# kongzhecn/OMG

Hardware: AMD Instinct MI355X
Metric: images/sec @ SDXL 1024^2 50-step, 2-concept mask fusion (higher is better)
Workload: dtype fp16 (storage and MFMA operands; fp32 accumulate; = the reference's own torch_dtype, inference_lora.py:153-159).  Measured tolerance per UNet forward at full size vs the fp32 oracle: rms 1.09e-3, max 4.9e-3 of O(1) outputs — the reference's own fp16 eager execution, emulated op by op in the oracle

## Files before the change

### include/omg_hip.h

```cpp
#ifndef OMG_HIP_H
#define OMG_HIP_H

#include <stdint.h>

#ifdef __cplusplus
extern "C" {
#endif

#define OMG_ABI_VERSION 6

enum { OMG_F16 = 0, OMG_BF16 = 1, OMG_F32 = 2  };

enum {
  OMG_OK = 0,
  OMG_EINVAL = -1,
  OMG_EDTYPE = -2,
  OMG_ELAUNCH = -3
};

enum {
  OMG_ACT_NONE = 0,
  OMG_ACT_SILU = 1,
  OMG_ACT_GEGLU = 2
};

int omg_abi_version(void);
const char* omg_last_error(void);

typedef struct {
  int32_t dtype;
  int32_t M, N, K;
  const void* A;  int64_t lda;
  const void* W;  int64_t ldw;
  const void* A2; int64_t lda2;
  const void* W2; int64_t ldw2;
  int32_t K2;
  int32_t a2_col_block;
  int32_t groups;
  int32_t rows_per_group;
  const int32_t* group_adapter;
  int64_t w_adapter_stride;
  int64_t w2_adapter_stride;
  const void* bias;
  const void* group_bias; int64_t ldgb;
  const void* residual; int64_t ldr;
  int32_t act;
  float out_scale;
  void* C; int64_t ldc;
} omg_gemm_args;

int omg_gemm(const omg_gemm_args* a, void* stream);

int omg_quant_mx8(int32_t dtype, const void* x, int64_t ldx, int32_t M, int32_t K,
                  void* q, int64_t ldq, void* scales, int32_t s_ld, void* stream);

typedef struct {
  int32_t dtype;
  int32_t M, N, K;
  const void* A; int64_t lda;
  const void* a_scale; int32_t sa_ld;
  const void* W; int64_t ldw;
  const void* w_scale; int32_t sw_ld;
  int32_t groups, rows_per_group;
  const int32_t* group_adapter;
  int64_t w_adapter_stride;
  int64_t sw_adapter_stride;
  const void* bias;
  const void* residual; int64_t ldr;
  int32_t act;
  float out_scale;
  void* C; int64_t ldc;
  void* c_scale; int32_t sc_ld;
} omg_gemm_mx8_args;

int omg_gemm_mx8(const omg_gemm_mx8_args* a, void* stream);

typedef struct {
  int32_t dtype;
  int32_t B, H, W, Cin, Cout;
  const void* X; const void* x_scale;
  const void* Wq; const void* w_scale;
  int32_t sw_ld, act;
  const void* bias;
  const void* group_bias; int64_t ldgb;
  const void* residual;
  float out_scale;
  void* Y;
} omg_conv2d_mx8_args;
int omg_conv2d_mx8(const omg_conv2d_mx8_args* a, void* stream);

typedef struct {
  int32_t dtype;
  int32_t B, Hin, Win;
  int32_t C1, C2;
  int32_t Hout, Wout, Cout;
  int32_t ksize;
  int32_t stride;
  int32_t upsample;
  const void* X1; const void* X2;
  const void* W;
  const void* bias;
  const void* group_bias; int64_t ldgb;
  const void* residual;
  float out_scale;
  void* Y;
  int32_t act;
} omg_conv2d_args;

int omg_conv2d(const omg_conv2d_args* a, void* stream);

typedef struct {
  int32_t dtype;
  int32_t B, heads, Nq, Nkv;
  const void* Q; int64_t ldq; int64_t q_bstride;
  const void* K; int64_t ldk; int64_t k_bstride;
  const void* Vt;
  int32_t Nkv_pad;
  const int32_t* qk_src;
  float scale;
  int32_t accumulate;
  float out_scale;
  void* O; int64_t ldo; int64_t o_bstride;
  const void* V; int64_t ldv; int64_t v_bstride;
} omg_attn_args;

int omg_attn_fwd(const omg_attn_args* a, void* stream);

int omg_transpose_v(int dtype, const void* V, int64_t ldv, int64_t v_bstride,
                    int B, int heads, int Nkv, int Nkv_pad, void* Vt, int mfma_key_order, void* stream);

int64_t omg_groupnorm_ws_floats(int B, int groups, int HW);
int omg_groupnorm(int dtype, const void* X1, int C1, const void* X2, int C2,
                  int B, int HW, int groups, float eps,
                  const void* gamma, const void* beta, int silu,
                  float* workspace, void* Y, void* stream);
int omg_layernorm(int dtype, const void* X, int64_t ldx, int M, int C, float eps,
                  const void* gamma, const void* beta, void* Y, int64_t ldy, void* stream);
int omg_layernorm_mx8(int dtype, const void* X, int64_t ldx, int M, int C, float eps,
                      const void* gamma, const void* beta, void* Q, int64_t ldq,
                      void* scales, int s_ld, void* stream);

int omg_groupnorm_mx8(int dtype, const void* X1, int C1, const void* X2, int C2,
                      int B, int HW, int groups, float eps,
                      const void* gamma, const void* beta, int silu,
                      float* workspace, void* Q, void* scales, void* stream);

typedef struct {
  int32_t B, Hin, Win, Cin;
  int32_t Hout, Wout, Cout;
  int32_t ksize, upsample;
  const void* X; const void* W; const void* bias; const void* residual;
  void* Y;
} omg_conv2d_f32_args;

int omg_conv2d_f32(const omg_conv2d_f32_args* a, void* stream);

typedef struct {
  int32_t B, Hin, Win, Cin;
  int32_t Hout, Wout, Cout;
  int32_t upsample;
  const void* X; const void* U; const void* bias; const void* residual;
  void* Y;
} omg_conv2d_f32_wino_args;

int64_t omg_conv2d_f32_wino_weight_floats(int Cout, int Cin);
int omg_conv2d_f32_wino(const omg_conv2d_f32_wino_args* a, void* stream);
int omg_cast_f32(int dtype, const void* X, float* Y, int64_t n, void* stream);

int omg_conv_in(int dtype, const void* X_nchw, int x_is_f32, int B, int Cin, int H, int W,
                const void* Wt , const void* bias, int Cout,
                void* workspace ,
                void* Y_nhwc, void* stream);
int omg_conv_out(int dtype, const void* X_nhwc, int B, int H, int W, int Cin,
                 const void* Wt , const void* bias, int Cout,
                 float* Y_nchw, void* stream);

int omg_timestep_embedding(int dtype, const float* t, int n, int dim, void* out, int64_t ldo, void* stream);
int omg_silu(int dtype, const void* x, void* y, int64_t n, void* stream);
int omg_add_inplace(int dtype, void* y, const void* a, int64_t n, void* stream);
int omg_softmax_rows(int dtype, void* X, int64_t rows, int64_t cols, int64_t ld, float scale, void* stream);
int omg_channel_mix(const float* X, const float* Wm, const float* bias, int B, int Cin, int Cout, int64_t HW,
                    float* Y, void* stream);
int omg_copy2d(int dtype, const void* src, int64_t lds, void* dst, int64_t ldd, int64_t rows, int64_t cols, void* stream);

#define OMG_MAX_CONCEPTS 8
typedef struct {
  int32_t C, H, W;
  int32_t Hm, Wm;
  int32_t n_concepts;
  int32_t fuse;
  float guidance_scale;
  const float* noise_pred;
  const float* region_pred[OMG_MAX_CONCEPTS];
  const float* masks[OMG_MAX_CONCEPTS];
  const float* coef;
  int32_t* step_idx;
  int32_t advance;
  float* latents;
  int32_t out_dtype;
  void* model_input_next;
  float* fused_noise_out;
// ... 27 lines not shown
```

### omg_amd/_lib.py

```python
from __future__ import annotations

import ctypes as C
import os

_HERE = os.path.dirname(os.path.abspath(__file__))
LIB_PATH = os.environ.get("OMG_HIP_LIB") or os.path.join(_HERE, "csrc", "libomg_hip.so")

OMG_F16, OMG_BF16, OMG_F32 = 0, 1, 2
ACT_NONE, ACT_SILU, ACT_GEGLU = 0, 1, 2
MAX_CONCEPTS = 8

c_i32, c_i64, c_f32, c_vp = C.c_int32, C.c_int64, C.c_float, C.c_void_p


class GemmArgs(C.Structure):
    _fields_ = [
        ("dtype", c_i32), ("M", c_i32), ("N", c_i32), ("K", c_i32),
        ("A", c_vp), ("lda", c_i64), ("W", c_vp), ("ldw", c_i64),
        ("A2", c_vp), ("lda2", c_i64), ("W2", c_vp), ("ldw2", c_i64),
        ("K2", c_i32), ("a2_col_block", c_i32),
        ("groups", c_i32), ("rows_per_group", c_i32),
        ("group_adapter", c_vp), ("w_adapter_stride", c_i64), ("w2_adapter_stride", c_i64),
        ("bias", c_vp), ("group_bias", c_vp), ("ldgb", c_i64),
        ("residual", c_vp), ("ldr", c_i64),
        ("act", c_i32), ("out_scale", c_f32),
        ("C", c_vp), ("ldc", c_i64),
    ]


class GemmMx8Args(C.Structure):
    _fields_ = [
        ("dtype", c_i32), ("M", c_i32), ("N", c_i32), ("K", c_i32),
        ("A", c_vp), ("lda", c_i64), ("a_scale", c_vp), ("sa_ld", c_i32),
        ("W", c_vp), ("ldw", c_i64), ("w_scale", c_vp), ("sw_ld", c_i32),
        ("groups", c_i32), ("rows_per_group", c_i32), ("group_adapter", c_vp),
        ("w_adapter_stride", c_i64), ("sw_adapter_stride", c_i64),
        ("bias", c_vp), ("residual", c_vp), ("ldr", c_i64),
        ("act", c_i32), ("out_scale", c_f32),
        ("C", c_vp), ("ldc", c_i64),
        ("c_scale", c_vp), ("sc_ld", c_i32),
    ]


class Conv2dMx8Args(C.Structure):
    _fields_ = [
        ("dtype", c_i32), ("B", c_i32), ("H", c_i32), ("W", c_i32), ("Cin", c_i32), ("Cout", c_i32),
        ("X", c_vp), ("x_scale", c_vp), ("Wq", c_vp), ("w_scale", c_vp),
        ("sw_ld", c_i32), ("act", c_i32),
        ("bias", c_vp), ("group_bias", c_vp), ("ldgb", c_i64), ("residual", c_vp),
        ("out_scale", c_f32), ("Y", c_vp),
    ]


class Conv2dArgs(C.Structure):
    _fields_ = [
        ("dtype", c_i32), ("B", c_i32), ("Hin", c_i32), ("Win", c_i32),
        ("C1", c_i32), ("C2", c_i32), ("Hout", c_i32), ("Wout", c_i32), ("Cout", c_i32),
        ("ksize", c_i32), ("stride", c_i32), ("upsample", c_i32),
        ("X1", c_vp), ("X2", c_vp), ("W", c_vp), ("bias", c_vp),
        ("group_bias", c_vp), ("ldgb", c_i64), ("residual", c_vp),
        ("out_scale", c_f32), ("Y", c_vp), ("act", c_i32),
    ]


class Conv2dF32Args(C.Structure):
    _fields_ = [
        ("B", c_i32), ("Hin", c_i32), ("Win", c_i32), ("Cin", c_i32),
        ("Hout", c_i32), ("Wout", c_i32), ("Cout", c_i32), ("ksize", c_i32), ("upsample", c_i32),
        ("X", c_vp), ("W", c_vp), ("bias", c_vp), ("residual", c_vp), ("Y", c_vp),
    ]


class Conv2dF32WinoArgs(C.Structure):
    _fields_ = [
        ("B", c_i32), ("Hin", c_i32), ("Win", c_i32), ("Cin", c_i32),
        ("Hout", c_i32), ("Wout", c_i32), ("Cout", c_i32), ("upsample", c_i32),
        ("X", c_vp), ("U", c_vp), ("bias", c_vp), ("residual", c_vp), ("Y", c_vp),
    ]


class AttnArgs(C.Structure):
    _fields_ = [
        ("dtype", c_i32), ("B", c_i32), ("heads", c_i32), ("Nq", c_i32), ("Nkv", c_i32),
        ("Q", c_vp), ("ldq", c_i64), ("q_bstride", c_i64),
        ("K", c_vp), ("ldk", c_i64), ("k_bstride", c_i64),
        ("Vt", c_vp), ("Nkv_pad", c_i32),
        ("qk_src", c_vp), ("scale", c_f32), ("accumulate", c_i32), ("out_scale", c_f32),
        ("O", c_vp), ("ldo", c_i64), ("o_bstride", c_i64),
        ("V", c_vp), ("ldv", c_i64), ("v_bstride", c_i64),
    ]


class StepArgs(C.Structure):
    _fields_ = [
        ("C", c_i32), ("H", c_i32), ("W", c_i32), ("Hm", c_i32), ("Wm", c_i32),
        ("n_concepts", c_i32), ("fuse", c_i32), ("guidance_scale", c_f32),
        ("noise_pred", c_vp), ("region_pred", c_vp * MAX_CONCEPTS), ("masks", c_vp * MAX_CONCEPTS),
        ("coef", c_vp), ("step_idx", c_vp), ("advance", c_i32),
        ("latents", c_vp), ("out_dtype", c_i32), ("model_input_next", c_vp), ("fused_noise_out", c_vp),
    ]


SYMBOLS = {
    "omg_abi_version": (c_i32, []),
    "omg_last_error": (C.c_char_p, []),
    "omg_gemm": (c_i32, [C.POINTER(GemmArgs), c_vp]),
    "omg_quant_mx8": (c_i32, [c_i32, c_vp, c_i64, c_i32, c_i32, c_vp, c_i64, c_vp, c_i32, c_vp]),
    "omg_gemm_mx8": (c_i32, [C.POINTER(GemmMx8Args), c_vp]),
    "omg_conv2d_mx8": (c_i32, [C.POINTER(Conv2dMx8Args), c_vp]),
    "omg_groupnorm_mx8": (c_i32, [c_i32, c_vp, c_i32, c_vp, c_i32, c_i32, c_i32, c_i32, c_f32, c_vp, c_vp, c_i32, c_vp, c_vp, c_vp, c_vp]),
    "omg_conv2d": (c_i32, [C.POINTER(Conv2dArgs), c_vp]),
    "omg_conv2d_f32": (c_i32, [C.POINTER(Conv2dF32Args), c_vp]),
    "omg_conv2d_f32_wino_weight_floats": (c_i64, [c_i32, c_i32]),
    "omg_conv2d_f32_wino": (c_i32, [C.POINTER(Conv2dF32WinoArgs), c_vp]),
    "omg_cast_f32": (c_i32, [c_i32, c_vp, c_vp, c_i64, c_vp]),
    "omg_attn_fwd": (c_i32, [C.POINTER(AttnArgs), c_vp]),
    "omg_transpose_v": (c_i32, [c_i32, c_vp, c_i64, c_i64, c_i32, c_i32, c_i32, c_i32, c_vp, c_i32, c_vp]),
    "omg_groupnorm_ws_floats": (c_i64, [c_i32, c_i32, c_i32]),
    "omg_groupnorm": (c_i32, [c_i32, c_vp, c_i32, c_vp, c_i32, c_i32, c_i32, c_i32, c_f32, c_vp, c_vp, c_i32, c_vp, c_vp, c_vp]),
    "omg_layernorm": (c_i32, [c_i32, c_vp, c_i64, c_i32, c_i32, c_f32, c_vp, c_vp, c_vp, c_i64, c_vp]),
    "omg_layernorm_mx8": (c_i32, [c_i32, c_vp, c_i64, c_i32, c_i32, c_f32, c_vp, c_vp, c_vp, c_i64, c_vp, c_i32, c_vp]),
    "omg_conv_in": (c_i32, [c_i32, c_vp, c_i32, c_i32, c_i32, c_i32, c_i32, c_vp, c_vp, c_i32, c_vp, c_vp, c_vp]),
    "omg_conv_out": (c_i32, [c_i32, c_vp, c_i32, c_i32, c_i32, c_i32, c_vp, c_vp, c_i32, c_vp, c_vp]),
    "omg_timestep_embedding": (c_i32, [c_i32, c_vp, c_i32, c_i32, c_vp, c_i64, c_vp]),
    "omg_silu": (c_i32, [c_i32, c_vp, c_vp, c_i64, c_vp]),
    "omg_softmax_rows": (c_i32, [c_i32, c_vp, c_i64, c_i64, c_i64, C.c_float, c_vp]),
    "omg_channel_mix": (c_i32, [c_vp, c_vp, c_vp, c_i32, c_i32, c_i32, c_i64, c_vp, c_vp]),
    "omg_add_inplace": (c_i32, [c_i32, c_vp, c_vp, c_i64, c_vp]),
    "omg_copy2d": (c_i32, [c_i32, c_vp, c_i64, c_vp, c_i64, c_i64, c_i64, c_vp]),
    "omg_fuse_cfg_step": (c_i32, [C.POINTER(StepArgs), c_vp]),
    "omg_fuse_cfg_step_ms": (c_i32, [C.POINTER(StepArgs), c_vp, c_vp, c_vp]),
    "omg_fuse_cfg_step_noise": (c_i32, [C.POINTER(StepArgs), c_vp, c_i64, c_vp]),
    "omg_scale_model_input": (c_i32, [c_i32, c_vp, c_vp, c_i32, c_vp, c_vp]),
    "omg_gather_step": (c_i32, [c_i32, c_vp, c_vp, c_vp, c_i64, c_vp]),
    "omg_attn_probs": (c_i32, [C.POINTER(AttnArgs), c_vp, c_vp]),
    "omg_attn_apply_probs": (c_i32, [c_i32, c_vp, c_vp, c_i64, c_i64, c_i32, c_i32, c_i32, c_i32, c_vp, c_i64, c_i64, c_vp]),
    "omg_dwconv2d": (c_i32, [c_i32, c_vp, c_i64, c_i32, c_i32, c_i32, c_i32, c_i32, c_vp, c_vp, c_vp, c_i64, c_vp]),
    "omg_relu_linear_att_ws_floats": (c_i64, [c_i32, c_i32, c_i32, c_i32]),
    "omg_relu_linear_att": (c_i32, [c_i32, c_vp, c_i64, c_i32, c_i32, c_i32, c_i32, c_f32, c_vp, c_vp, c_i64, c_vp]),
    "omg_debug_set_glds": (None, [c_i32]),
    "omg_debug_set_gemm_variant": (None, [c_i32]),
    "omg_debug_choose_variant": (c_i32, [c_i32, c_i32, c_i32, c_i32]),
    "omg_debug_set_mx8_split": (None, [c_i32]),
    "omg_debug_set_attn_variant": (None, [c_i32]),
}

_lib = None


class OmgHipError(RuntimeError):
    pass


def lib() -> C.CDLL:
    global _lib
    if _lib is not None:
        return _lib
    if not os.path.exists(LIB_PATH):
        raise OmgHipError(
            f"{LIB_PATH} not found: the HIP extension has not been built. "
            "Run `python -c 'import __graft_entry__ as g; g.build()'` (needs hipcc). "
            "omg_amd has no CPU fallback."
        )
    import torch

    l = C.CDLL(LIB_PATH)
    for name, (res, args) in SYMBOLS.items():
        fn = getattr(l, name)
        fn.restype = res
        fn.argtypes = args
    if l.omg_abi_version() != 6:
        raise OmgHipError("libomg_hip.so ABI version mismatch; rebuild")
    v = os.environ.get("OMG_GEMM_VARIANT")
    if v:
        l.omg_debug_set_gemm_variant(int(v))
    v = os.environ.get("OMG_ATTN_VARIANT")
    if v:
        l.omg_debug_set_attn_variant(int(v, 0))
    v = os.environ.get("OMG_MX8_SPLIT")
# ... 11 lines not shown
```

### omg_amd/attention.py

```python
from __future__ import annotations

from typing import Optional

import torch
from torch import nn

from . import _lib as L
from . import ops
from .modules import Dropout, Linear, LoraState, bump_pointer_epoch, pointer_epoch


class Attention(nn.Module):

    def __init__(self, query_dim: int, cross_attention_dim: Optional[int], heads: int, dim_head: int = 64,
                 dtype=torch.float16, device=None):
        super().__init__()
        if dim_head != 64:
            raise L.OmgHipError("the gfx950 attention kernel is specialised for head_dim 64 (all SDXL layers)")
        inner = heads * dim_head
        self.heads, self.scale, self.inner_dim = heads, dim_head ** -0.5, inner
        self.is_cross = cross_attention_dim is not None
        kv_dim = cross_attention_dim if self.is_cross else query_dim
        self.to_q = Linear(query_dim, inner, bias=False, dtype=dtype, device=device)
        self.to_k = Linear(kv_dim, inner, bias=False, dtype=dtype, device=device)
        self.to_v = Linear(kv_dim, inner, bias=False, dtype=dtype, device=device)
        self.to_out = nn.ModuleList([Linear(inner, query_dim, bias=True, dtype=dtype, device=device), Dropout()])
        self.spatial_norm = None
        self.group_norm = None
        self.norm_cross = None
        self.residual_connection = False
        self.rescale_output_factor = 1.0
        self.processor = FusedAttnProcessor()
        self._qkv = None
        self._kv = None
        self._qkv_slots = None
        self._kv_slots = None
        self._kv_cache = {}
        self.ip_kv_weight: Optional[torch.Tensor] = None
        self.ip_scale, self.ip_tokens = 1.0, 16
        self._ip_cache = None
        self._mx8 = {}

    def set_processor(self, processor) -> None:
        self.processor = processor

    def get_processor(self):
        return self.processor

    def forward(self, hidden_states, encoder_hidden_states=None, attention_mask=None, **cross_attention_kwargs):
        return self.processor(self, hidden_states, encoder_hidden_states=encoder_hidden_states,
                              attention_mask=attention_mask, **cross_attention_kwargs)

    def prepare_attention_mask(self, attention_mask, target_length, batch_size, out_dim=3):
        if attention_mask is not None:
            raise L.OmgHipError("attention masks are not used on OMG's path (always None) and are not supported")
        return None

    def head_to_batch_dim(self, t: torch.Tensor) -> torch.Tensor:
        B, N, _ = t.shape
        return t.reshape(B, N, self.heads, 64).permute(0, 2, 1, 3).reshape(B * self.heads, N, 64)

    def batch_to_head_dim(self, t: torch.Tensor) -> torch.Tensor:
        BH, N, d = t.shape
        return t.reshape(BH // self.heads, self.heads, N, d).permute(0, 2, 1, 3).reshape(BH // self.heads, N, self.heads * d)

    def get_attention_scores(self, query: torch.Tensor, key: torch.Tensor, attention_mask=None) -> torch.Tensor:
        if attention_mask is not None:
            raise L.OmgHipError("attention masks are not supported")
        q, k = query.contiguous(), key.contiguous()
        return ops.attn_probs(q, k, 1, self.scale)

    def _apply(self, fn, *a, **k):
        self.invalidate_packed()
        return super()._apply(fn, *a, **k)

    def invalidate_packed(self):
        self._qkv = self._kv = self._qkv_slots = self._kv_slots = None
        self._kv_cache = {}
        self._mx8 = {}
        self._ip_cache = None
        bump_pointer_epoch()

    def qkv_weight(self) -> torch.Tensor:
        if self._qkv is None:
            self._qkv = torch.cat([self.to_q.weight.data, self.to_k.weight.data, self.to_v.weight.data], dim=0).contiguous()
        return self._qkv

    def kv_weight(self) -> torch.Tensor:
        if self._kv is None:
            self._kv = torch.cat([self.to_k.weight.data, self.to_v.weight.data], dim=0).contiguous()
        return self._kv

    def _has_lora(self) -> bool:
        st = self.to_q.lora_state
        return st is not None and not st.merged and any(l.lora_down is not None for l in (self.to_q, self.to_k, self.to_v))

    def _merged(self) -> Optional[LoraState]:
        st = self.to_q.lora_state
        if st is None or not st.merged:
            return None
        have = [l.w_slots is not None for l in (self.to_q, self.to_k, self.to_v)]
        if any(have) and not all(have):
            raise L.OmgHipError("merged LoRA slots cover only part of to_q/to_k/to_v; rebuild the LoraBank")
        return st if all(have) else None

    def qkv_slots(self) -> torch.Tensor:
        if self._qkv_slots is None:
            self._qkv_slots = torch.cat([self.to_q.w_slots, self.to_k.w_slots, self.to_v.w_slots], dim=1).contiguous()
        return self._qkv_slots

    def kv_slots(self) -> torch.Tensor:
        if self._kv_slots is None:
            self._kv_slots = torch.cat([self.to_k.w_slots, self.to_v.w_slots], dim=1).contiguous()
        return self._kv_slots

    def project_self(self, x):
        B, N, C = x.shape
        inner = self.inner_dim
        if isinstance(x, ops.Mx8Tensor) or (self.to_q.mx8 and C % 128 == 0 and not self._has_lora()):
            if self._has_lora():
                raise L.OmgHipError("MX-fp8 activations cannot feed a segment-mode LoRA projection")
            xq = x if isinstance(x, ops.Mx8Tensor) else ops.quant_mx8(x)
            st = self._merged()
            if st is not None:
                if "qkv_slots" not in self._mx8:
                    self._mx8["qkv_slots"] = ops.quant_mx8(self.qkv_slots().reshape(-1, C))
                qkv = ops.gemm_mx8(xq, self._mx8["qkv_slots"], out_dtype=self.to_q.weight.dtype, groups=st.groups,
                                   w_group_adapter=st.group_adapter, n_per_adapter=3 * inner)
            else:
                if "qkv" not in self._mx8:
                    self._mx8["qkv"] = ops.quant_mx8(self.qkv_weight())
                qkv = ops.gemm_mx8(xq, self._mx8["qkv"], out_dtype=self.to_q.weight.dtype)
            qkv = qkv.view(B, N, 3 * inner)
            return qkv[:, :, :inner], qkv[:, :, inner:2 * inner], ops.value_operand(qkv[:, :, 2 * inner:], self.heads)
        if self._has_lora():
            q = self.to_q(x); k = self.to_k(x); v = self.to_v(x)
        else:
            st = self._merged()
            if st is not None:
                qkv = ops.gemm(x.reshape(B * N, C), self.qkv_slots(), groups=st.groups, w_group_adapter=st.group_adapter)
            else:
                qkv = ops.gemm(x.reshape(B * N, C), self.qkv_weight())
            qkv = qkv.view(B, N, 3 * inner)
            q, k, v = qkv[:, :, :inner], qkv[:, :, inner:2 * inner], qkv[:, :, 2 * inner:]
        return q, k, ops.value_operand(v, self.heads)

    def project_cross(self, ctx: torch.Tensor):
        st = self.to_k.lora_state
        skey = (tuple(ctx.shape), None if st is None else (st.group_adapter.data_ptr(), st.merged))
        stamp = (ctx.data_ptr(), ctx._version)
        hit = self._kv_cache.get(skey)
        if hit is not None:
            self._kv_cache[skey] = self._kv_cache.pop(skey)
        if hit is not None and hit[0] == stamp:
            return hit[1], hit[2]
        B, Nk, Cx = ctx.shape
        inner = self.inner_dim
        kv_out = hit[4] if hit is not None else None
        vt_out = hit[2] if hit is not None else None
        if self._has_lora():
            k = self.to_k(ctx); v = self.to_v(ctx)
            kv_out = None
        else:
            ms = self._merged()
            x2 = ctx.reshape(B * Nk, Cx)
            if ms is not None:
                kv = ops.gemm(x2, self.kv_slots(), groups=ms.groups, w_group_adapter=ms.group_adapter, out=kv_out)
            else:
                kv = ops.gemm(x2, self.kv_weight(), out=kv_out)
            kv_out = kv
            kv = kv.view(B, Nk, 2 * inner)
            k, v = kv[:, :, :inner], kv[:, :, inner:]
        vt = ops.transpose_v(v, self.heads, out=vt_out)
        if hit is None and len(self._kv_cache) >= 4:
            self._kv_cache.pop(next(iter(self._kv_cache)))
            bump_pointer_epoch()
        self._kv_cache[skey] = (stamp, k, vt, ctx, kv_out)
        return k, vt


def _ip_kv(attn: Attention, ip_ctx: torch.Tensor):
    shape = tuple(ip_ctx.shape)
    stamp = (ip_ctx.data_ptr(), ip_ctx._version)
    cache = attn._ip_cache
    if cache is None:
        cache = attn._ip_cache = {}
    c = cache.get(shape)
    if c is not None:
        cache[shape] = cache.pop(shape)
    if c is None or c[0] != stamp:
        Bc, Ni, Cx = shape
        kv_out = c[3] if c is not None else None
        vt_out = c[2] if c is not None else None
        kv = ops.gemm(ip_ctx.reshape(Bc * Ni, Cx), attn.ip_kv_weight, out=kv_out)
        kv3 = kv.view(Bc, Ni, 2 * attn.inner_dim)
        vt = ops.transpose_v(kv3[:, :, attn.inner_dim:], attn.heads, out=vt_out)
        if c is None and len(cache) >= 4:
            cache.pop(next(iter(cache)))
            bump_pointer_epoch()
        c = (stamp, kv3[:, :, :attn.inner_dim], vt, kv, shape, ip_ctx)
        cache[shape] = c
    return c


def _ip_branch(attn: Attention, q: torch.Tensor, o: torch.Tensor, ip_ctx: torch.Tensor, row0: int) -> None:
    c = _ip_kv(attn, ip_ctx)
    ops.attention(q[row0:], c[1], c[2], attn.heads, attn.scale, out=o[row0:], accumulate=True, out_scale=attn.ip_scale)


def _to_tokens(attn, hidden_states):
    if isinstance(hidden_states, ops.Mx8Tensor):
        return hidden_states
    if hidden_states.dim() == 4:
        raise L.OmgHipError("4-D (NCHW) hidden_states are not produced by the SDXL transformer blocks; pass (B, N, C)")
    return hidden_states


class FusedAttnProcessor:

    supports_fused_residual = True

    def _qk_src(self, attn, is_cross: bool, n_tokens: int, batch: int, device, main_batch=None, images=1):
        return None

    def _skip_layer(self) -> None:
        return None

    def __call__(self, attn: Attention, hidden_states, encoder_hidden_states=None, attention_mask=None, temb=None,
                 scale: float = 1.0, residual: Optional[torch.Tensor] = None, **cross_attention_kwargs):
        if attention_mask is not None:
            raise L.OmgHipError("attention_mask is not supported")
        x = _to_tokens(attn, hidden_states)
        B, N, _ = x.shape
        is_cross = encoder_hidden_states is not None
        if is_cross:
            q = attn.to_q(x)
            k, vt = attn.project_cross(encoder_hidden_states)
        else:
            q, k, vt = attn.project_self(x)
        bypass = cross_attention_kwargs.pop("omg_bypass_controller", False)
        main_b = cross_attention_kwargs.pop("omg_main_batch", None)
        n_img = cross_attention_kwargs.pop("omg_images", 1)
        twin = cross_attention_kwargs.pop("omg_twin", False)
        if twin and not bypass:
            self._skip_layer()
        src = None if (bypass or twin) else self._qk_src(attn, is_cross, N, B, x.device, main_b, n_img)
        ip_ctx = cross_attention_kwargs.pop("omg_ip_tokens", None)
        ip_row0 = cross_attention_kwargs.pop("omg_ip_rows", 0)
        o = ops.attention(q, k, vt, attn.heads, attn.scale, qk_src=src)
        if is_cross and ip_ctx is not None and attn.ip_kv_weight is not None:
            _ip_branch(attn, q, o, ip_ctx, ip_row0)
        out = attn.to_out[0](o, residual=residual)
        return out


class RegionControlNet_AttnProcessor(FusedAttnProcessor):

    def __init__(self, attention_op=None, controller=None, place_in_unet=None):
        self.attention_op = attention_op
        self.controller = controller
        self.place_in_unet = place_in_unet

    def _fusable(self) -> bool:
        return self.controller is None or getattr(self.controller, "is_pure_replacement", False)

    def _qk_src(self, attn, is_cross, n_tokens, batch, device, main_batch=None, images=1):
        if self.controller is None:
            return None
        return self.controller.fused_qk_src(is_cross, n_tokens, main_batch or batch, self.place_in_unet, device=device,
                                            total_batch=batch, images=images)

    def _skip_layer(self) -> None:
        if self.controller is not None:
            self.controller.skip_layer()

    def __call__(self, attn: Attention, hidden_states, encoder_hidden_states=None, attention_mask=None, temb=None,
                 scale: float = 1.0, residual: Optional[torch.Tensor] = None, **cross_attention_kwargs):
        if self._fusable() or cross_attention_kwargs.get("omg_bypass_controller", False):
            return super().__call__(attn, hidden_states, encoder_hidden_states, attention_mask, temb, scale,
                                    residual=residual, **cross_attention_kwargs)
        if cross_attention_kwargs.get("omg_images", 1) != 1:
            raise L.OmgHipError("protocol mode (non-identity mapper) runs one request at a time")
        x = _to_tokens(attn, hidden_states)
        is_cross = encoder_hidden_states is not None
        src = encoder_hidden_states if is_cross else x
        query = attn.head_to_batch_dim(attn.to_q(x))
        key = attn.head_to_batch_dim(attn.to_k(src))
        value = attn.to_v(src)
        probs = attn.get_attention_scores(query, key, None)
        probs = self.controller(probs, is_cross, self.place_in_unet)
        o = ops.attn_apply_probs(probs.contiguous(), value, attn.heads)
        return attn.to_out[0](o, residual=residual)


class IPAttnProcessor2_0(nn.Module):

    supports_fused_residual = True

    def __init__(self, hidden_size: int, cross_attention_dim: Optional[int] = None, scale: float = 1.0, num_tokens: int = 4,
                 dtype=torch.float16, device=None):
        super().__init__()
        self.hidden_size, self.cross_attention_dim, self.scale, self.num_tokens = hidden_size, cross_attention_dim, scale, num_tokens
        self.to_k_ip = Linear(cross_attention_dim or hidden_size, hidden_size, bias=False, dtype=dtype, device=device)
        self.to_v_ip = Linear(cross_attention_dim or hidden_size, hidden_size, bias=False, dtype=dtype, device=device)

    def __call__(self, attn: Attention, hidden_states, encoder_hidden_states=None, attention_mask=None, temb=None,
                 residual: Optional[torch.Tensor] = None, **kw):
        if attention_mask is not None:
            raise L.OmgHipError("attention_mask is not supported")
        x = _to_tokens(attn, hidden_states)
        if encoder_hidden_states is None:
            q, k, vt = attn.project_self(x)
            o = ops.attention(q, k, vt, attn.heads, attn.scale)
            return attn.to_out[0](o, residual=residual)
        end = encoder_hidden_states.shape[1] - self.num_tokens
        text, ip = encoder_hidden_states[:, :end], encoder_hidden_states[:, end:]
        q = attn.to_q(x)
        B, Nt, Cx = text.shape
        k = attn.to_k(text.reshape(B * Nt, Cx)).view(B, Nt, -1)
        v = attn.to_v(text.reshape(B * Nt, Cx)).view(B, Nt, -1)
        o = ops.attention(q, k, ops.transpose_v(v, attn.heads), attn.heads, attn.scale)
        Ni = ip.shape[1]
        ipc = ip.reshape(B * Ni, Cx)
        k_ip = self.to_k_ip(ipc).view(B, Ni, -1)
        v_ip = self.to_v_ip(ipc).view(B, Ni, -1)
        ops.attention(q, k_ip, ops.transpose_v(v_ip, attn.heads), attn.heads, attn.scale, out=o, accumulate=True,
                      out_scale=self.scale)
        return attn.to_out[0](o, residual=residual)
```

### omg_amd/controller.py

```python
from __future__ import annotations

from typing import Dict, List, Optional, Sequence, Tuple

import numpy as np
import torch

MAX_NUM_WORDS = 77


def _word_of_token(text: str, tokenizer) -> Tuple[List[str], np.ndarray]:
    words = text.split(" ")
    pieces = [tokenizer.decode([tok]).strip("#") for tok in tokenizer.encode(text)][1:-1]
    cum = np.cumsum([len(pc_) for pc_ in pieces], dtype=np.int64) if pieces else np.zeros(0, np.int64)
    owner = np.full(len(pieces), len(words), dtype=np.int64)
    first, base = 0, 0
    for k, word in enumerate(words):
        if first >= len(pieces):
            break
        last = int(np.searchsorted(cum, base + len(word), side="left"))
        last = max(last, first)
        last = min(last, len(pieces) - 1)
        owner[first:last + 1] = k
        first, base = last + 1, int(cum[last])
    return words, owner


def get_word_inds(text: str, word_place, tokenizer) -> np.ndarray:
    words = text.split(" ")
    if isinstance(word_place, str):
        wanted = [i for i, w in enumerate(words) if w == word_place]
    elif isinstance(word_place, int):
        wanted = [word_place]
    else:
        wanted = list(word_place)
    if not wanted:
        return np.array([])
    _, owner = _word_of_token(text, tokenizer)
    return np.flatnonzero(np.isin(owner, wanted)) + 1


def _alignment_matrix(src_spans: Sequence[np.ndarray], tgt_spans: Sequence[np.ndarray], max_len: int) -> np.ndarray:
    m = np.zeros((max_len, max_len))
    i = j = 0
    for s, t in zip(src_spans, tgt_spans):
        s, t = np.asarray(s, dtype=np.int64), np.asarray(t, dtype=np.int64)
        run = min(int(s[0]) - i, max_len - i, max_len - j)
        if run < int(s[0]) - i:
            r = np.arange(max(run, 0))
            m[i + r, j + r] = 1
            return m
        r = np.arange(run)
        m[i + r, j + r] = 1
        i, j = i + run, j + run
        if i >= max_len or j >= max_len:
            return m
        if len(s) == len(t):
            m[s, t] = 1
        else:
            m[np.ix_(s, t)] = 1.0 / len(t)
        i, j = i + len(s), j + len(t)
    tail = np.arange(max(0, min(max_len - i, max_len - j)))
    if src_spans:
        m[j + tail, j + tail] = 1
    else:
        m[i + tail, j + tail] = 1
    return m


def get_replacement_mapper(prompts: Sequence[str], tokenizer, max_len: int = MAX_NUM_WORDS) -> torch.Tensor:
    out = []
    words0 = prompts[0].split(" ")
    for other in prompts[1:]:
        words = other.split(" ")
        if len(words0) != len(words):
            raise ValueError("attention replacement edit can only be applied on prompts with the same length"
                             f" but prompt A has {len(words0)} words and prompt B has {len(words)} words.")
        changed = [k for k, (a, b) in enumerate(zip(words0, words)) if a != b]
        if not changed:
            out.append(torch.eye(max_len, dtype=torch.float32))
            continue
        if tokenizer is None:
            raise ValueError("a tokenizer is required to align prompts that differ")
        _, own0 = _word_of_token(prompts[0], tokenizer)
        _, own1 = _word_of_token(other, tokenizer)
        src = [np.flatnonzero(own0 == k) + 1 for k in changed]
        tgt = [np.flatnonzero(own1 == k) + 1 for k in changed]
        out.append(torch.from_numpy(_alignment_matrix(src, tgt, max_len)).float())
    return torch.stack(out)


def get_time_words_attention_alpha(prompts, num_steps, cross_replace_steps, tokenizer, max_num_words=MAX_NUM_WORDS):
    spec = dict(cross_replace_steps) if isinstance(cross_replace_steps, dict) else {"default_": cross_replace_steps}
    spec.setdefault("default_", (0.0, 1.0))
    if isinstance(cross_replace_steps, dict):
        cross_replace_steps.setdefault("default_", (0.0, 1.0))
    n_rows, n_edit = num_steps + 1, len(prompts) - 1
    steps = torch.arange(n_rows).view(n_rows, 1)

    def inside(bounds) -> torch.Tensor:
        lo, hi = (0, bounds) if isinstance(bounds, float) else bounds
        return ((steps >= int(lo * n_rows)) & (steps < int(hi * n_rows))).to(torch.float32)

    alpha = inside(spec["default_"]).view(n_rows, 1, 1).repeat(1, n_edit, max_num_words)
    for word, bounds in spec.items():
        if word == "default_":
            continue
        col = inside(bounds)
        for k in range(n_edit):
            pos = get_word_inds(prompts[k + 1], word, tokenizer)
            if len(pos) > 0:
                alpha[:, k, torch.as_tensor(pos, dtype=torch.long)] = col
    return alpha.reshape(n_rows, n_edit, 1, 1, max_num_words)


class AttentionReplace:
    def __init__(self, prompts, num_steps: int, cross_replace_steps, self_replace_steps, width, height,
                 local_blend=None, tokenizer=None, device=None, dtype=None):
        self.low_resource = False
        self.width, self.height = width, height
        self.batch_size = len(prompts)
        self.local_blend = local_blend
        self.device, self.dtype = device, dtype
        self.cross_replace_alpha = get_time_words_attention_alpha(prompts, num_steps, cross_replace_steps, tokenizer).to(device)
        if isinstance(self_replace_steps, float):
            self_replace_steps = (0, self_replace_steps)
        self.num_self_replace = (int(num_steps * self_replace_steps[0]), int(num_steps * self_replace_steps[1]))
        self.mapper = get_replacement_mapper(prompts, tokenizer).to(dtype=dtype, device=device)
        self.num_att_layers = -1
        self.cur_step = 0
        self.cur_att_layer = 0
        eye = torch.eye(MAX_NUM_WORDS)
        self._identity_mapper = all(torch.equal(m.float().cpu(), eye) for m in self.mapper)
        self.is_pure_replacement = bool(local_blend is None and self._identity_mapper and bool((self.cross_replace_alpha == 1).all()))
        self._src_cache: Dict[Tuple, torch.Tensor] = {}

    @property
    def num_uncond_att_layers(self):
        return 0

    def reset(self):
        self.cur_step = 0
        self.cur_att_layer = 0

    def between_steps(self):
        return

    def step_callback(self, x_t):
        return x_t

    def _tick(self):
        self.cur_att_layer += 1
        if self.cur_att_layer == self.num_att_layers + self.num_uncond_att_layers:
            self.cur_att_layer = 0
            self.cur_step += 1
            self.between_steps()

    def _self_window(self) -> bool:
        return self.num_self_replace[0] <= self.cur_step < self.num_self_replace[1]

    def forward(self, attn, is_cross: bool, place_in_unet: str):
        if not (is_cross or self._self_window()):
            return attn
        v = attn.reshape(self.batch_size, attn.shape[0] // self.batch_size, *attn.shape[1:])
        base, edits = v[0], v[1:]
        if is_cross:
            a = self.cross_replace_alpha[self.cur_step].to(device=v.device, dtype=v.dtype)
            mapped = base.unsqueeze(0).expand(edits.shape[0], *base.shape) if self._identity_mapper \
                else torch.matmul(base.unsqueeze(0), self.mapper.to(device=v.device, dtype=v.dtype).unsqueeze(1))
            edits.copy_(mapped * a + (1 - a) * edits)
        elif edits.shape[2] <= self.width * self.height:
            edits.copy_(base.unsqueeze(0).expand_as(edits))
        return v.reshape(attn.shape)

    def __call__(self, attn, is_cross: bool, place_in_unet: str):
        cond = attn[attn.shape[0] // 2:]
        out = self.forward(cond, is_cross, place_in_unet)
        if out.data_ptr() != cond.data_ptr():
            cond.copy_(out)
        self._tick()
        return attn

    def replaces(self, is_cross: bool, n_tokens: int) -> bool:
        if is_cross:
            return True
        return self._self_window() and n_tokens <= self.width * self.height

    def qk_src_vector(self, batch: int, device, total_batch: Optional[int] = None, images: int = 1) -> torch.Tensor:
        total = total_batch or batch * images
        key = (batch, total, images, str(device))
        t = self._src_cache.get(key)
        if t is None:
            n = batch // 2
            v = []
            for j in range(images):
                v += [j * batch + i for i in range(n)] + [j * batch + n] * (batch - n)
            v += list(range(batch * images, total))
            t = torch.tensor(v, dtype=torch.int32, device=device)
            self._src_cache[key] = t
        return t

    def skip_layer(self) -> None:
        if not self.is_pure_replacement:
            raise RuntimeError("skip_layer needs a pure-replacement controller")
        self._tick()

    def fused_qk_src(self, is_cross: bool, n_tokens: int, batch: int, place_in_unet: str = "",
                     device=None, total_batch: Optional[int] = None, images: int = 1) -> Optional[torch.Tensor]:
        if not self.is_pure_replacement:
            raise RuntimeError("fused_qk_src needs a pure-replacement controller (identity mapper, alpha == 1)")
        if batch not in (2 * self.batch_size, 2 * self.batch_size - 1):
            raise ValueError(f"controller built for {self.batch_size} prompts expects a batch of {2 * self.batch_size} "
                             f"([unc..., cond...]), got {batch}")
        src = self.qk_src_vector(batch, device or self.device or "cuda", total_batch, images) if self.replaces(is_cross, n_tokens) else None
        self._tick()
        return src
```

### omg_amd/csrc/gemm.hip

```cpp
#include "common.h"
#include "gemm_epilogue.h"

__device__ __attribute__((aligned(256))) unsigned char omg_zero_page[256];

__device__ long long omg_dbg_ts[8192][6];

namespace {

constexpr int BM = 128, BN = 128, BK = 64;
constexpr int TILE_BYTES = BM * BK * 2;
constexpr int STAGE_LD = 68;
constexpr int LDS_BYTES_MAIN = 4 * TILE_BYTES;
constexpr int LDS_BYTES_EPI = 4 * 64 * STAGE_LD * 4;
constexpr int LDS_BYTES = LDS_BYTES_EPI > LDS_BYTES_MAIN ? LDS_BYTES_EPI : LDS_BYTES_MAIN;


template <bool GLDS>
OMG_DEV void stage16(const char* src, char* lds_wave_base, int lane, u32x4& hold) {
  if constexpr (GLDS) {
    __builtin_amdgcn_global_load_lds((gbl_ptr_t)src, (lds_ptr_t)lds_wave_base, 16, 0, 0);
  } else {
    hold = *(const u32x4*)src;
  }
}

template <typename T, int MT, int NT>
OMG_DEV void acc_init_cols(const GemmP& p, f32x16 (&acc)[MT][NT], int l31, int col0, int m0) {
  const bool fold = fold_group_bias(p);
  const long grow = fold ? (long)(m0 / p.rows_per_group) * p.ldgb : 0;
#pragma unroll
  for (int j = 0; j < NT; ++j) {
    const int c = col0 + j * 32 + l31;
    float b = 0.f;
    if (c < p.N) {
      float g = 0.f;
      if (p.bias) b = (float)((const T*)p.bias)[c];
      if (fold) g = (float)((const T*)p.group_bias)[grow + c];
      b = b + g;
    }
#pragma unroll
    for (int i = 0; i < MT; ++i)
#pragma unroll
      for (int r = 0; r < 16; ++r) acc[i][j][r] = b;
  }
}

template <typename T>
OMG_DEV void gemm_epilogue(const GemmP& p, f32x16 (&acc)[2][2], char* smem, int w, int lane, int m0, int n0, int m_end) {
  const int hi = lane >> 5, l31 = lane & 31;
  const int wm = w >> 1, wn = w & 1;
  __syncthreads();
  float* stage = (float*)smem + w * (64 * STAGE_LD);
#pragma unroll
  for (int i = 0; i < 2; ++i)
#pragma unroll
    for (int j = 0; j < 2; ++j)
#pragma unroll
      for (int r = 0; r < 16; ++r) {
        const int row = i * 32 + (r & 3) + 8 * (r >> 2) + 4 * hi;
        stage[row * STAGE_LD + j * 32 + l31] = acc[i][j][r];
      }
  __syncthreads();

  const int wm0 = m0 + wm * 64;
  const int wn0 = n0 + wn * 64;
  if (p.act == OMG_ACT_GEGLU) {
    const int ocol0 = (wn0 >> 1);
    const int sub = lane & 3, rsub = lane >> 2;
#pragma unroll
    for (int it = 0; it < 4; ++it) {
      const int row = it * 16 + rsub;
      const int gm = wm0 + row;
      const int gc = wn0 + sub * 8;
      if (gm < m_end && gc < p.N) {
        float v[8], g[8];
        const float* sp = stage + row * STAGE_LD + sub * 8;
#pragma unroll
        for (int e = 0; e < 8; ++e) { v[e] = sp[e]; g[e] = sp[32 + e]; }
        float o[8];
#pragma unroll
        for (int e = 0; e < 8; ++e) o[e] = v[e] * gelu_f(g[e]) * p.out_scale;
        *(u32x4*)(p.C + ((long)gm * p.ldc + ocol0 + sub * 8) * 2) = pack8<T>(o);
      }
    }
    return;
  }
  {
    const int sub = lane & 7, rsub = lane >> 3;
    const int gc = wn0 + sub * 8;
    const bool gb_rows = p.group_bias != nullptr && !fold_group_bias(p);
#pragma unroll
    for (int it = 0; it < 8; ++it) {
      const int row = it * 8 + rsub;
      const int gm = wm0 + row;
      if (gm < m_end && gc < p.N) {
        float v[8];
        const float* sp = stage + row * STAGE_LD + sub * 8;
#pragma unroll
        for (int e = 0; e < 8; ++e) v[e] = sp[e];
        if (gb_rows) {
          float gb[8];
          const int g = gm / p.rows_per_group;
          unpack8<T>(*(const u32x4*)(p.group_bias + ((long)g * p.ldgb + gc) * 2), gb);
#pragma unroll
          for (int e = 0; e < 8; ++e) v[e] += gb[e];
        }
        if (p.act == OMG_ACT_SILU) {
#pragma unroll
          for (int e = 0; e < 8; ++e) v[e] = silu_fast(v[e]);
        }
        if (p.residual) {
          float rv[8];
          unpack8<T>(*(const u32x4*)(p.residual + ((long)gm * p.ldr + gc) * 2), rv);
#pragma unroll
          for (int e = 0; e < 8; ++e) v[e] = __builtin_fmaf(v[e], p.out_scale, rv[e]);
        } else {
#pragma unroll
          for (int e = 0; e < 8; ++e) v[e] *= p.out_scale;
        }
        *(u32x4*)(p.C + ((long)gm * p.ldc + gc) * 2) = pack8<T>(v);
      }
    }
  }
}

template <typename T, bool CONV, bool GLDS>
__global__ __launch_bounds__(256, 2) void gemm_kernel(GemmP p) {
  extern __shared__ __attribute__((aligned(16))) char smem[];
  const int tid = threadIdx.x;
  const int lane = tid & 63;
  const int w = __builtin_amdgcn_readfirstlane(tid >> 6);
  const int hi = lane >> 5;
  const int l31 = lane & 31;

  const int nwg = gridDim.x;
  int bid = blockIdx.x;
  {
    const int q = nwg >> 3, r = nwg & 7, xcd = bid & 7, idx = bid >> 3;
    bid = (xcd < r ? xcd * (q + 1) : r * (q + 1) + (xcd - r) * q) + idx;
  }
  const int tiles_per_group = p.tiles_m * p.tiles_n;
  const int grp = bid / tiles_per_group;
  const int t_in = bid - grp * tiles_per_group;
  int tm, tn;
  {
    const int per_group = 8 * p.tiles_n;
    const int gid = t_in / per_group;
    const int first_m = gid * 8;
    const int gsz = (p.tiles_m - first_m) < 8 ? (p.tiles_m - first_m) : 8;
    const int r = t_in - gid * per_group;
    tm = first_m + (r % gsz);
    tn = r / gsz;
  }
  const int m_base = (p.tile_groups > 1) ? grp * p.rows_per_group : 0;
  const int m_end = (p.tile_groups > 1) ? m_base + p.rows_per_group : p.M;
  const int m0 = m_base + tm * BM;
  const int n0 = tn * BN;

  int adapter = 0;
  if (p.group_adapter != nullptr) adapter = p.group_adapter[grp];
  const bool seg2 = (p.K2 > 0) && (adapter >= 0);
  if (p.w_adapter_stride != 0 && adapter < 0) return;
  const char* Wp = p.W + (p.w_adapter_stride != 0 ? (long)adapter * p.w_adapter_stride * 2 : 0);
  const char* W2p = p.W2 + (seg2 ? (long)adapter * p.w2_adapter_stride * 2 : 0);
  const int a2off = (p.a2_col_block > 0) ? (n0 / p.a2_col_block) * p.K2 : 0;

  const int nk1 = (p.K + BK - 1) / BK;
  const int nk2 = seg2 ? (p.K2 + BK - 1) / BK : 0;
  const int nk = nk1 + nk2;

  const int prow = lane >> 3;
  const int ppos = lane & 7;
  int arow[4];
  int wrow[4];
  int cb[4], cy[4], cx[4];
#pragma unroll
  for (int i = 0; i < 4; ++i) {
    const int r = w * 32 + i * 8 + prow;
    int gm = m0 + r; if (gm > m_end - 1) gm = m_end - 1;
    int gn = n0 + r; if (gn > p.N - 1) gn = p.N - 1;
    arow[i] = gm; wrow[i] = gn;
    if constexpr (CONV) {
      const int hw = p.Hout * p.Wout;
      const int b = gm / hw; const int rem = gm - b * hw;
      cb[i] = b; cy[i] = rem / p.Wout; cx[i] = rem - cy[i] * p.Wout;
    }
  }
  const int Ctot = p.C1 + p.C2;
  const int cpt = CONV ? Ctot / BK : 1;
  const int pad = CONV ? (p.ksize == 3 ? 1 : 0) : 0;
  const char* zero = (const char*)omg_zero_page;

  u32x4 hold[8];
  char* ldsA = smem;
  char* ldsB = smem + 2 * TILE_BYTES;

  auto issue = [&](int kt, int buf) {
    const bool s2 = kt >= nk1;
    const int k0 = (s2 ? kt - nk1 : kt) * BK;
    const int Kseg = s2 ? p.K2 : p.K;
    int dy = 0, dx = 0, c0 = k0;
    const char* xsrc = p.A; int xC = p.C1;
    if constexpr (CONV) {
      const int tap = kt / cpt; const int cc = kt - tap * cpt;
      dy = tap / p.ksize; dx = tap - dy * p.ksize;
      c0 = cc * BK;
      if (c0 >= p.C1) { xsrc = p.X2; xC = p.C2; c0 -= p.C1; }
    }
#pragma unroll
    for (int i = 0; i < 4; ++i) {
      const int r = w * 32 + i * 8 + prow;
      const int c = ppos ^ ((r >> 1) & 7);
      const bool kvalid = (k0 + c * 8) < Kseg;
      const char* asrc;
      if constexpr (CONV) {
        int iy = cy[i] * p.stride + dy - pad;
        int ix = cx[i] * p.stride + dx - pad;
        const int Hl = p.upsample ? p.Hin * 2 : p.Hin;
        const int Wl = p.upsample ? p.Win * 2 : p.Win;
        const bool ok = (iy >= 0) && (iy < Hl) && (ix >= 0) && (ix < Wl);
        if (p.upsample) { iy >>= 1; ix >>= 1; }
        const long pix = ((long)cb[i] * p.Hin + iy) * p.Win + ix;
        asrc = ok ? xsrc + (pix * xC + c0 + c * 8) * 2 : zero;
      } else {
        if (!s2) asrc = kvalid ? p.A + ((long)arow[i] * p.lda + k0 + c * 8) * 2 : zero;
        else     asrc = kvalid ? p.A2 + ((long)arow[i] * p.lda2 + a2off + k0 + c * 8) * 2 : zero;
      }
      stage16<GLDS>(asrc, ldsA + buf * TILE_BYTES + (w * 32 + i * 8) * 128, lane, hold[i]);
      const char* wsrc;
      if (!s2) wsrc = kvalid ? Wp + ((long)wrow[i] * p.ldw + (CONV ? kt * BK : k0) + c * 8) * 2 : zero;
      else     wsrc = kvalid ? W2p + ((long)wrow[i] * p.ldw2 + k0 + c * 8) * 2 : zero;
      stage16<GLDS>(wsrc, ldsB + buf * TILE_BYTES + (w * 32 + i * 8) * 128, lane, hold[4 + i]);
    }
  };
  auto commit = [&](int buf) {
    if constexpr (!GLDS) {
#pragma unroll
      for (int i = 0; i < 4; ++i) {
        const int off = (w * 32 + i * 8) * 128 + lane * 16;
        *(u32x4*)(ldsA + buf * TILE_BYTES + off) = hold[i];
        *(u32x4*)(ldsB + buf * TILE_BYTES + off) = hold[4 + i];
      }
    }
  };

  const int wm = w >> 1, wn = w & 1;
  f32x16 acc[2][2];
  acc_init_cols<T, 2, 2>(p, acc, lane & 31, n0 + wn * 64, m0);

  using V8 = typename Vec<T>::v8;

  issue(0, 0);
  commit(0);
  for (int kt = 0; kt < nk; ++kt) {
    const int buf = kt & 1;
    asm volatile("s_waitcnt vmcnt(0)" ::: "memory");
    __syncthreads();
    if (kt + 1 < nk) issue(kt + 1, buf ^ 1);
    const char* a_base = ldsA + buf * TILE_BYTES;
    const char* b_base = ldsB + buf * TILE_BYTES;
#pragma unroll
    for (int ks = 0; ks < 4; ++ks) {
      V8 af[2], bf[2];
      const int kc = ks * 2 + hi;
#pragma unroll
      for (int i = 0; i < 2; ++i) {
        const int ra = wm * 64 + i * 32 + l31;
        af[i] = *(const V8*)(a_base + ra * 128 + ((kc ^ ((ra >> 1) & 7)) << 4));
        const int rb = wn * 64 + i * 32 + l31;
        bf[i] = *(const V8*)(b_base + rb * 128 + ((kc ^ ((rb >> 1) & 7)) << 4));
      }
#pragma unroll
      for (int i = 0; i < 2; ++i)
#pragma unroll
        for (int j = 0; j < 2; ++j) acc[i][j] = Vec<T>::mfma32(af[i], bf[j], acc[i][j]);
    }
    if constexpr (!GLDS) { if (kt + 1 < nk) commit(buf ^ 1); }
  }

  gemm_epilogue<T>(p, acc, smem, w, lane, m0, n0, m_end);
}


OMG_DEV int conv_voff(int b, int oy, int ox, int ch_bytes, int stride, int dy, int dx, int Hl, int Wl, int ups, int Hin, int Win,
                      int pix_bytes, int c0_bytes) {
  int iy = oy * stride + dy, ix = ox * stride + dx;
  const bool ok = ((unsigned)iy < (unsigned)Hl) & ((unsigned)ix < (unsigned)Wl);
  iy >>= ups; ix >>= ups;
  const int pix = (b * Hin + iy) * Win + ix;
  const int off = pix * pix_bytes + c0_bytes + ch_bytes;
  return ok ? off : 0x7ffffff0;
}

template <typename T, bool CONV, int MT>
__global__ __launch_bounds__(512, 2) void gemm_kernel_v6(GemmP p) {
  constexpr int BM_ = 256, BN_ = MT == 4 ? 256 : 128, BKc = 64, NW = 8, NT = 2;
  constexpr int WN_ = MT == 4 ? 4 : 2;
  constexpr int BI = BN_ / 8 / NW;
  constexpr int ND = 4 + BI;
  constexpr int HB = ND / 2;
  constexpr int A_BYTES = BM_ * BKc * 2;
  constexpr int STAGE_BYTES = (BM_ + BN_) * BKc * 2;

  extern __shared__ __attribute__((aligned(16))) char smem[];
  const int tid = threadIdx.x;
  const int lane = tid & 63;
  const int w = __builtin_amdgcn_readfirstlane(tid >> 6);
  const int hi = lane >> 5;
  const int l31 = lane & 31;

  const int nwg = gridDim.x;
  int bid = blockIdx.x;
  {
    const int q = nwg >> 3, r = nwg & 7, xcd = bid & 7, idx = bid >> 3;
    bid = (xcd < r ? xcd * (q + 1) : r * (q + 1) + (xcd - r) * q) + idx;
  }
  const int tiles_per_group = p.tiles_m * p.tiles_n;
  const int grp = bid / tiles_per_group;
  const int t_in = bid - grp * tiles_per_group;
  int tm, tn;
  {
    const int per_group = 8 * p.tiles_n;
    const int gid = t_in / per_group;
    const int first_m = gid * 8;
    const int gsz = (p.tiles_m - first_m) < 8 ? (p.tiles_m - first_m) : 8;
    const int r = t_in - gid * per_group;
    tm = first_m + (r % gsz);
    tn = r / gsz;
  }
  const int m_base = (p.tile_groups > 1) ? grp * p.rows_per_group : 0;
  const int m_end = (p.tile_groups > 1) ? m_base + p.rows_per_group : p.M;
  const int m0 = m_base + tm * BM_;
  const int n0 = tn * BN_;
  int adapter = 0;
  if (p.group_adapter != nullptr) adapter = p.group_adapter[grp];
  if (p.w_adapter_stride != 0 && adapter < 0) return;
  const char* Wp = p.W + (p.w_adapter_stride != 0 ? (long)adapter * p.w_adapter_stride * 2 : 0);
  const int nk = (p.K + BKc - 1) / BKc;

  const int Ctot = p.C1 + p.C2;
  const long a_bytes = CONV ? (long)p.M / (p.Hout * p.Wout) * p.Hin * p.Win * p.C1 * 2 : ((long)(p.M - 1) * p.lda + p.K) * 2;
  const __amdgpu_buffer_rsrc_t rsA = __builtin_amdgcn_make_buffer_rsrc((void*)p.A, 0, (int)(a_bytes < 0x7fffff00 ? a_bytes : 0x7fffff00), 0x00020000);
  const __amdgpu_buffer_rsrc_t rsA2 = __builtin_amdgcn_make_buffer_rsrc((void*)(CONV && p.X2 ? p.X2 : p.A), 0,
      CONV ? (int)((long)p.M / (p.Hout * p.Wout) * p.Hin * p.Win * p.C2 * 2) : 0, 0x00020000);
  const long w_bytes = ((long)(p.N - 1) * p.ldw + p.K) * 2;
  const __amdgpu_buffer_rsrc_t rsW = __builtin_amdgcn_make_buffer_rsrc((void*)Wp, 0, (int)w_bytes, 0x00020000);

  const int prow = lane >> 3, ppos = lane & 7;
  int voffA[4], voffW[BI], ldoA[4], ldoW[BI];
  int cb[4], cy[4], cx[4], cch[4];
#pragma unroll
  for (int i = 0; i < 4; ++i) {
    const int r = (w + i * NW) * 8 + prow;
    const int c = ppos ^ ((r >> 1) & 7);
    int gm = m0 + r; if (gm > m_end - 1) gm = m_end - 1;
    ldoA[i] = (w + i * NW) * 1024;
    if constexpr (CONV) {
      const int hw = p.Hout * p.Wout;
      const int b = gm / hw; const int rem = gm - b * hw;
      cb[i] = b; cy[i] = rem / p.Wout; cx[i] = rem - cy[i] * p.Wout; cch[i] = c * 16;
      voffA[i] = 0;
    } else {
      voffA[i] = (int)(((long)gm * p.lda + c * 8) * 2);
    }
  }
#pragma unroll
  for (int i = 0; i < BI; ++i) {
    const int r = (w + i * NW) * 8 + prow;
    const int c = ppos ^ ((r >> 1) & 7);
    int gn = n0 + r; if (gn > p.N - 1) gn = p.N - 1;
    voffW[i] = (int)(((long)gn * p.ldw + c * 8) * 2);
    ldoW[i] = A_BYTES + (w + i * NW) * 1024;
  }

  const int wm = w / WN_, wn = w % WN_;
  f32x16 acc[MT][NT];
  const bool gb_epi = acc_init_bias<T, MT, NT>(p, acc, lane, m0, n0 + wn * 64);
  using V8 = typename Vec<T>::v8;
  int aro[MT][4], bro[NT][4];
#pragma unroll
  for (int ks = 0; ks < 4; ++ks) {
    const int kc = ks * 2 + hi;
#pragma unroll
    for (int i = 0; i < MT; ++i) {
      const int ra = wm * (MT * 32) + i * 32 + l31;
      aro[i][ks] = ra * 128 + ((kc ^ ((ra >> 1) & 7)) << 4);
    }
#pragma unroll
    for (int j = 0; j < NT; ++j) {
      const int rb = wn * 64 + j * 32 + l31;
      bro[j][ks] = A_BYTES + rb * 128 + ((kc ^ ((rb >> 1) & 7)) << 4);
    }
  }

  int koff = 0;
  int tap_dy = 0, tap_dx = 0, c0b = 0, xCb = 0;
  bool x2 = false;
  const int cpt = CONV ? Ctot / BKc : 1;
  const int pad = CONV ? (p.ksize == 3 ? 1 : 0) : 0;
  const int Hl = CONV ? (p.upsample ? p.Hin * 2 : p.Hin) : 0;
  const int Wl = CONV ? (p.upsample ? p.Win * 2 : p.Win) : 0;
#define OMG_PREP(kt_)                                                                                      \
  do {                                                                                                     \
    koff = (kt_) * (BKc * 2);                                                                              \
    if constexpr (CONV) {                                                                                  \
      const int tap = (kt_) / cpt; const int cc = (kt_) - tap * cpt;                                       \
      tap_dy = tap / p.ksize - pad; tap_dx = tap - (tap / p.ksize) * p.ksize - pad;                        \
      int c0 = cc * BKc;                                                                                   \
      x2 = c0 >= p.C1;                                                                                     \
      if (x2) c0 -= p.C1;                                                                                  \
      c0b = c0 * 2; xCb = (x2 ? p.C2 : p.C1) * 2;                                                          \
    }                                                                                                      \
  } while (0)
#define OMG_AVO(i_) (CONV ? conv_voff(cb[i_], cy[i_], cx[i_], cch[i_], p.stride, tap_dy, tap_dx, Hl, Wl, p.upsample, p.Hin, p.Win, xCb, c0b) : voffA[i_])

  const bool late = w >= 4;
  V8 af[2][MT], bf[2][NT];
#define OMG_ISA(d_) ((d_) < 4)
#define OMG_AI(d_) ((d_) < 4 ? (d_) : 0)
#define OMG_WI(d_) ((d_) >= 4 ? (d_) - 4 : 0)
#define OMG_VO(d_) (OMG_ISA(d_) ? OMG_AVO(OMG_AI(d_)) : voffW[OMG_WI(d_)])
#define OMG_LO(d_) (OMG_ISA(d_) ? ldoA[OMG_AI(d_)] : ldoW[OMG_WI(d_)])
#define OMG_RS(d_) (OMG_ISA(d_) ? ((CONV && x2) ? rsA2 : rsA) : rsW)
#define OMG_SO(d_) ((OMG_ISA(d_) && CONV) ? 0 : koff)
#define OMG_DMA(d_, nb_)                                                                                     \
  dma16(OMG_RS(d_), (nb_) + OMG_LO(d_), OMG_VO(d_), OMG_SO(d_))
#define OMG_DMA2(q_, nb_)                                                                                    \
  dma16(late ? OMG_RS(HB + (q_)) : OMG_RS(q_), (nb_) + (late ? OMG_LO(HB + (q_)) : OMG_LO(q_)),              \
        late ? OMG_VO(HB + (q_)) : OMG_VO(q_), late ? OMG_SO(HB + (q_)) : OMG_SO(q_))
#define OMG_Q(q_)                                                                                            \
  do {                                                                                                       \
    if constexpr (MT == 4) {                                                                                 \
      _Pragma("unroll") for (int i = ((q_) & 1) * 2; i < ((q_) & 1) * 2 + 2; ++i)                            \
        _Pragma("unroll") for (int j = 0; j < NT; ++j)                                                       \
          acc[i][j] = Vec<T>::mfma32(bf[(q_) >> 1][j], af[(q_) >> 1][i], acc[i][j]);                         \
    } else {                                                                                                 \
      _Pragma("unroll") for (int j = 0; j < NT; ++j)                                                         \
        acc[(q_) & 1][j] = Vec<T>::mfma32(bf[(q_) >> 1][j], af[(q_) >> 1][(q_) & 1], acc[(q_) & 1][j]);      \
    }                                                                                                        \
  } while (0)
#define OMG_RD(sb_, half_)                                                                                   \
  do {                                                                                                       \
    _Pragma("unroll") for (int ks = 0; ks < 2; ++ks) {                                                       \
      _Pragma("unroll") for (int j = 0; j < NT; ++j) bf[ks][j] = *(const V8*)((sb_) + bro[j][(half_) * 2 + ks]); \
      _Pragma("unroll") for (int i = 0; i < MT; ++i) af[ks][i] = *(const V8*)((sb_) + aro[i][(half_) * 2 + ks]); \
    }                                                                                                        \
  } while (0)

  OMG_PREP(0);
  OMG_DMA(0, smem); OMG_DMA(1, smem); OMG_DMA(2, smem); OMG_DMA(3, smem);
  OMG_DMA(4, smem); OMG_DMA(5, smem);
  if constexpr (ND == 8) { OMG_DMA(6, smem); OMG_DMA(7, smem); }

  for (int kt = 0; kt < nk; ++kt) {
    wait_vmcnt<0>();
    __builtin_amdgcn_s_barrier();
    const char* sb = smem + (kt & 1) * STAGE_BYTES;
    char* nb = smem + ((kt + 1) & 1) * STAGE_BYTES;
    const bool nxt = kt + 1 < nk;
    OMG_PREP(kt + 1);
    if (late) {
      if (kt > 0) {
        OMG_Q(0); if (nxt) OMG_DMA(0, nb);
        OMG_Q(1); if (nxt) OMG_DMA(1, nb);
        OMG_Q(2); if (nxt) OMG_DMA(2, nb);
        OMG_Q(3); if constexpr (HB == 4) { if (nxt) OMG_DMA(3, nb); }
      } else if (nxt) {
        OMG_DMA(0, nb); OMG_DMA(1, nb); OMG_DMA(2, nb);
        if constexpr (HB == 4) OMG_DMA(3, nb);
      }
    }
    OMG_RD(sb, 0);
    OMG_Q(0); if (nxt) OMG_DMA2(0, nb);
    OMG_Q(1); if (nxt) OMG_DMA2(1, nb);
    OMG_Q(2); if (nxt) OMG_DMA2(2, nb);
    OMG_Q(3); if constexpr (HB == 4) { if (nxt) OMG_DMA2(3, nb); }
    OMG_RD(sb, 1);
    if (!late) {
      OMG_Q(0); if (nxt) OMG_DMA(HB + 0, nb);
      OMG_Q(1); if (nxt) OMG_DMA(HB + 1, nb);
      OMG_Q(2); if (nxt) OMG_DMA(HB + 2, nb);
      OMG_Q(3); if constexpr (HB == 4) { if (nxt) OMG_DMA(HB + 3, nb); }
    }
  }
  if (late) { OMG_Q(0); OMG_Q(1); OMG_Q(2); OMG_Q(3); }
#undef OMG_DMA
#undef OMG_DMA2
#undef OMG_Q
#undef OMG_RD
#undef OMG_ISA
#undef OMG_AI
#undef OMG_WI
#undef OMG_VO
#undef OMG_LO
#undef OMG_RS
#undef OMG_SO
#undef OMG_PREP
#undef OMG_AVO
  if (p.dbg & 32) {
    float sacc = 0.f;
#pragma unroll
    for (int i = 0; i < MT; ++i)
#pragma unroll
      for (int j = 0; j < NT; ++j)
#pragma unroll
        for (int r = 0; r < 16; ++r) sacc += acc[i][j][r];
    if (sacc == 1.2345e-30f) p.C[0] = 1;
    return;
  }
  epilogue_direct<T, MT, NT>(p, acc, lane, m0 + wm * (MT * 32), n0 + wn * 64, m_end, gb_epi);
}

template <typename T, bool CONV, int ABL = 0, int MT = 4, int NT = 4, bool XE = false, int EF = 0>
__global__ __launch_bounds__(256, 1) void gemm_kernel_v7(GemmP p) {
  constexpr int BM_ = MT * 64, BN_ = NT * 64, BKc = 64;
  constexpr int AB = MT * 2, WB = NT * 2;
  constexpr int NMM = MT * NT;
  constexpr int SLOTS = NMM / 2;
  constexpr int NRD = MT + NT;
  static_assert(NMM % 2 == 0, "even number of MFMAs per k-step");
  constexpr int A_BYTES = BM_ * BKc * 2;
  constexpr int STAGE_BYTES = (BM_ + BN_) * BKc * 2;

  const bool ts_on = (p.dbg & 16) && blockIdx.x < 8192 && threadIdx.x == 0;
  long long ts0 = 0, ts1 = 0, ts2 = 0;
  if (((p.dbg >> 16) & 0xff) != 0 && blockIdx.x < 256) {
    const long long wait = (long long)((blockIdx.x * 97) & 255) * ((p.dbg >> 16) & 0xff) * 25 / 256;
    const long long t_end = __builtin_amdgcn_s_memrealtime() + wait;
    while (__builtin_amdgcn_s_memrealtime() < t_end) __builtin_amdgcn_s_sleep(2);
  }
  if (p.dbg & 16) ts0 = __builtin_amdgcn_s_memrealtime();
  extern __shared__ __attribute__((aligned(16))) char smem[];
  const int tid = threadIdx.x;
  const int lane = tid & 63;
  const int w = __builtin_amdgcn_readfirstlane(tid >> 6);
  const int hi = lane >> 5;
  const int l31 = lane & 31;

  const int nwg = gridDim.x;
  int bid = blockIdx.x;
  {
    const int q = nwg >> 3, r = nwg & 7, xcd = bid & 7, idx = bid >> 3;
    bid = (xcd < r ? xcd * (q + 1) : r * (q + 1) + (xcd - r) * q) + idx;
  }
  const int tiles_per_group = p.tiles_m * p.tiles_n;
  const int grp = bid / tiles_per_group;
  const int t_in = bid - grp * tiles_per_group;
  int tm, tn;
  {
    const int per_group = 8 * p.tiles_n;
    const int gid = t_in / per_group;
    const int first_m = gid * 8;
    const int gsz = (p.tiles_m - first_m) < 8 ? (p.tiles_m - first_m) : 8;
    const int r = t_in - gid * per_group;
    tm = first_m + (r % gsz);
    tn = r / gsz;
  }
  const int m_base = (p.tile_groups > 1) ? grp * p.rows_per_group : 0;
  const int m_end = (p.tile_groups > 1) ? m_base + p.rows_per_group : p.M;
  const int m0 = m_base + tm * BM_;
  const int n0 = tn * BN_;
  int adapter = 0;
  if (p.group_adapter != nullptr) adapter = p.group_adapter[grp];
  if (p.w_adapter_stride != 0 && adapter < 0) return;
  const char* Wp = p.W + (p.w_adapter_stride != 0 ? (long)adapter * p.w_adapter_stride * 2 : 0);
  const int nk = (p.K + BKc - 1) / BKc;

  const int Ctot = p.C1 + p.C2;
  const long a_bytes = CONV ? (long)p.M / (p.Hout * p.Wout) * p.Hin * p.Win * p.C1 * 2 : ((long)(p.M - 1) * p.lda + p.K) * 2;
  const __amdgpu_buffer_rsrc_t rsA = __builtin_amdgcn_make_buffer_rsrc((void*)p.A, 0, (int)(a_bytes < 0x7fffff00 ? a_bytes : 0x7fffff00), 0x00020000);
  const __amdgpu_buffer_rsrc_t rsA2 = __builtin_amdgcn_make_buffer_rsrc((void*)(CONV && p.X2 ? p.X2 : p.A), 0,
      CONV ? (int)((long)p.M / (p.Hout * p.Wout) * p.Hin * p.Win * p.C2 * 2) : 0, 0x00020000);
  const long w_bytes = ((long)(p.N - 1) * p.ldw + p.K) * 2;
  const __amdgpu_buffer_rsrc_t rsW = __builtin_amdgcn_make_buffer_rsrc((void*)Wp, 0, (int)w_bytes, 0x00020000);

  const int prow = lane >> 3, ppos = lane & 7;
  int voffA[AB], voffW[WB];
  int cb[AB], cy[AB], cx[AB];
  const int dchunk = (ppos ^ ((w & 1) * 4 + (prow >> 1))) * 16;
#pragma unroll
  for (int i = 0; i < AB; ++i) {
    const int r = (w + i * 4) * 8 + prow;
    int gm = m0 + r; if (gm > m_end - 1) gm = m_end - 1;
    if constexpr (CONV) {
      const int hw = p.Hout * p.Wout;
      const int b = gm / hw; const int rem = gm - b * hw;
      cb[i] = b; cy[i] = rem / p.Wout; cx[i] = rem - cy[i] * p.Wout;
      voffA[i] = 0;
    } else {
      cb[i] = cy[i] = cx[i] = 0;
      voffA[i] = (int)((long)gm * p.lda * 2) + dchunk;
    }
  }
#pragma unroll
  for (int i = 0; i < WB; ++i) {
    const int r = (w + i * 4) * 8 + prow;
    int gn = n0 + r; if (gn > p.N - 1) gn = p.N - 1;
    voffW[i] = (int)((long)gn * p.ldw * 2) + dchunk;
  }
  const int ldo = w * 1024;

  const int wm = w >> 1, wn = w & 1;
  f32x16 acc[MT][NT];
  using V8 = typename Vec<T>::v8;
  int aoff[4], boff[4];
#pragma unroll
  for (int ks = 0; ks < 4; ++ks) {
    const int sw = ((ks * 2 + hi) ^ ((l31 >> 1) & 7)) << 4;
    aoff[ks] = (wm * (MT * 32) + l31) * 128 + sw;
    boff[ks] = A_BYTES + (wn * (NT * 32) + l31) * 128 + sw;
  }

  int koff = 0;
  int tap_dy = 0, tap_dx = 0, c0b = 0, xCb = 0;
  bool x2 = false;
  const int cpt = CONV ? Ctot / BKc : 1;
  const int pad = CONV ? (p.ksize == 3 ? 1 : 0) : 0;
  const int Hl = CONV ? (p.upsample ? p.Hin * 2 : p.Hin) : 0;
  const int Wl = CONV ? (p.upsample ? p.Win * 2 : p.Win) : 0;
#define OMG_PREP(kt_)                                                                                      \
  do {                                                                                                     \
    koff = (kt_) * (BKc * 2);                                                                              \
    if constexpr (CONV) {                                                                                  \
      const int tap = (kt_) / cpt; const int cc = (kt_) - tap * cpt;                                       \
      tap_dy = tap / p.ksize - pad; tap_dx = tap - (tap / p.ksize) * p.ksize - pad;                        \
      int c0 = cc * BKc;                                                                                   \
      x2 = c0 >= p.C1;                                                                                     \
      if (x2) c0 -= p.C1;                                                                                  \
      c0b = c0 * 2; xCb = (x2 ? p.C2 : p.C1) * 2;                                                          \
    }                                                                                                      \
  } while (0)
#define OMG_DMA(d_, nb_)                                                                                   \
  do {                                                                                                     \
    if ((d_) < AB) {                                                                                       \
      const int i_ = (d_) < AB ? (d_) : 0;                                                                 \
      if (CONV) dma16(x2 ? rsA2 : rsA, (nb_) + ldo + i_ * 4096,                                            \
                      conv_voff(cb[i_], cy[i_], cx[i_], dchunk, p.stride, tap_dy, tap_dx, Hl, Wl, p.upsample, p.Hin, p.Win, xCb, c0b), 0); \
      else dma16(rsA, (nb_) + ldo + i_ * 4096, voffA[i_], koff);                                           \
    } else {                                                                                               \
      const int i_ = (d_) - AB < WB ? (d_) - AB : 0;                                                       \
      dma16(rsW, (nb_) + A_BYTES + ldo + i_ * 4096, voffW[i_], koff);                                      \
    }                                                                                                      \
  } while (0)
#define OMG_DMAN(first_, n_, nb_)                                                                          \
  do { _Pragma("unroll") for (int d_ = 0; d_ < (n_); ++d_) OMG_DMA((first_) + d_, nb_); } while (0)
#define OMG_RD(f_, sb_, ks_)                                                                               \
  do {                                                                                                     \
    _Pragma("unroll") for (int j = 0; j < NT; ++j) bf[f_][j] = *(const V8*)((sb_) + boff[ks_] + j * 4096); \
    _Pragma("unroll") for (int i = 0; i < MT; ++i) af[f_][i] = *(const V8*)((sb_) + aoff[ks_] + i * 4096); \
  } while (0)
#define OMG_MM(f_)                                                                                         \
  do {                                                                                                     \
    _Pragma("unroll") for (int i = 0; i < MT; ++i)                                                         \
      _Pragma("unroll") for (int j = 0; j < NT; ++j)                                                       \
        acc[i][j] = Vec<T>::mfma32(af[f_][i], bf[f_][j], acc[i][j]);                                       \
  } while (0)
#define OMG_RD1(f_, sb_, ks_, r_)                                                                          \
  do {                                                                                                     \
     \
    const bool isA_ = (r_) == 1 || (r_) > NT;                                                              \
    const int idx_ = (r_) <= 1 ? 0 : (r_) <= NT ? (r_) - 1 : (r_) - NT;                                    \
    if (!isA_) bf[f_][idx_] = *(const V8*)((sb_) + boff[ks_] + idx_ * 4096);                               \
    else af[f_][idx_] = *(const V8*)((sb_) + aoff[ks_] + idx_ * 4096);                                     \
  } while (0)
#define OMG_MM1(f_, n_) acc[(n_) / NT][(n_) % NT] = Vec<T>::mfma32(bf[f_][(n_) % NT], af[f_][(n_) / NT], acc[(n_) / NT][(n_) % NT])
#define OMG_KSTEP(f_, RD_, rb_, rks_, DMA_, d0_, dn_, db_)                                                 \
  do {                                                                                                     \
    constexpr int RPS_ = (RD_) == 2 ? 2 : (NRD + SLOTS - 1) / SLOTS;                                       \
    constexpr int DPS_ = ((dn_) + SLOTS - 1) / SLOTS;                                                      \
    _Pragma("unroll") for (int s_ = 0; s_ < SLOTS; ++s_) {                                                 \
      OMG_MM1(f_, 2 * s_);                                                                                 \
      __builtin_amdgcn_sched_barrier(0);                                                                   \
      if ((RD_) != 0 && !(ABL & 2)) {                                                                      \
        _Pragma("unroll") for (int q_ = 0; q_ < RPS_; ++q_)                                                \
          if (s_ * RPS_ + q_ < NRD) OMG_RD1(1 - (f_), rb_, rks_, s_ * RPS_ + q_);                          \
      }                                                                                                    \
      __builtin_amdgcn_sched_barrier(0);                                                                   \
      OMG_MM1(f_, 2 * s_ + 1);                                                                             \
      __builtin_amdgcn_sched_barrier(0);                                                                   \
      if ((DMA_) && !(ABL & 1)) {                                                                          \
        _Pragma("unroll") for (int q_ = 0; q_ < DPS_; ++q_)                                                \
          if (s_ * DPS_ + q_ < (dn_)) OMG_DMA((d0_) + s_ * DPS_ + q_, db_);                                \
      }                                                                                                    \
      __builtin_amdgcn_sched_barrier(0);                                                                   \
    }                                                                                                      \
  } while (0)

  V8 af[2][MT], bf[2][NT];
  OMG_PREP(0);
  OMG_DMAN(0, AB + WB, smem);
  const bool gb_epi = acc_init_bias<T, MT, NT>(p, acc, lane, m0, n0 + wn * (NT * 32));
  wait_vmcnt<0>();
  __builtin_amdgcn_s_barrier();
  if (p.dbg & 16) ts1 = __builtin_amdgcn_s_memrealtime();
  OMG_PREP(1);
  if (nk > 1) OMG_DMAN(0, AB, smem + STAGE_BYTES);
  OMG_RD(0, smem, 0);

#define OMG_STAGE(HAS1_, HAS2_)                                                                            \
  do {                                                                                                     \
    const char* cur = smem + (kt & 1) * STAGE_BYTES;                                                       \
    char* nxt = smem + ((kt + 1) & 1) * STAGE_BYTES;                                                       \
                                                  \
    OMG_KSTEP(0, 1, cur, 1, HAS1_, AB, WB, nxt);                                                            \
    OMG_KSTEP(1, 1, cur, 2, false, 0, 0, nxt);                                                             \
    OMG_KSTEP(0, 1, cur, 3, false, 0, 0, nxt);                                                             \
     \
    if (!(ABL & 4)) { asm volatile("s_waitcnt vmcnt(0) lgkmcnt(0)" ::: "memory"); __builtin_amdgcn_s_barrier(); } \
                                                                                                      \
     \
    if (HAS2_) OMG_PREP(kt + 2);                                                                           \
    OMG_KSTEP(1, (HAS1_) ? 2 : 0, nxt, 0, HAS2_, 0, AB, (char*)cur);                                                     \
  } while (0)
  int kt = 0;
// ... 49 lines not shown
  if (!attr) {
    attr = true;
    (void)hipFuncSetAttribute((const void*)gemm_kernel_v6<T, CONV, MT>, hipFuncAttributeMaxDynamicSharedMemorySize, lds);
  }
  p.tiles_m = (mrows + 255) / 256;
  p.tiles_n = (p.N + BN_ - 1) / BN_;
  p.dbg = g_dbg;
  const int grid = p.tile_groups * p.tiles_m * p.tiles_n;
  if (grid <= 0) return OMG_OK;
  OMG_LAUNCH((gemm_kernel_v6<T, CONV, MT>), dim3(grid), dim3(512), lds, s, p);
  return omg_check_launch("gemm_v6");
}

template <typename T, bool CONV, int ABL = 0, int MT = 4, int NT = 4, bool XE = false, int EF = 0>
int launch_v7(GemmP p, hipStream_t s, int mrows) {
  constexpr int BM_ = MT * 64, BN_ = NT * 64;
  constexpr int lds = 2 * (BM_ + BN_) * 64 * 2 + (XE ? 4 * 8192 : 0);
  static bool attr = false;
  if (!attr) {
    attr = true;
    (void)hipFuncSetAttribute((const void*)gemm_kernel_v7<T, CONV, ABL, MT, NT, XE, EF>, hipFuncAttributeMaxDynamicSharedMemorySize, lds);
  }
  p.tiles_m = (mrows + BM_ - 1) / BM_;
  p.tiles_n = (p.N + BN_ - 1) / BN_;
  p.dbg = g_dbg;
  const int grid = p.tile_groups * p.tiles_m * p.tiles_n;
  if (grid <= 0) return OMG_OK;
  OMG_LAUNCH((gemm_kernel_v7<T, CONV, ABL, MT, NT, XE, EF>), dim3(grid), dim3(256), lds, s, p);
  return omg_check_launch("gemm_v7");
}

int num_cus();
#include "gemm_v12.h"
#include "gemm_v13.h"

int num_cus() {
  static int n = 0;
  if (n == 0) {
    int dev = 0;
    (void)hipGetDevice(&dev);
    if (hipDeviceGetAttribute(&n, hipDeviceAttributeMultiprocessorCount, dev) != hipSuccess || n <= 0) n = 256;
  }
  return n;
}

int choose_variant(int mrows, int groups, int N, bool conv, bool geglu = false) {
  if (g_variant != 0) return g_variant;
  const long t256 = (long)groups * ((mrows + 255) / 256) * ((N + 255) / 256);
  const long t256x128 = (long)groups * ((mrows + 255) / 256) * ((N + 127) / 128);
  const long t128x320 = (long)groups * ((mrows + 127) / 128) * ((N + 319) / 320);
  const long t256x320 = (long)groups * ((mrows + 255) / 256) * ((N + 319) / 320);
  const double c256 = (N > 128 && t256 >= 120) ? (double)((t256 + 255) / 256) : 1e30;
  const double c128 = t256x128 >= 120 ? (double)((t256x128 + 255) / 256) * 0.58 * 1.06 : 1e30;
  const double c320 = (conv && !geglu && N % 320 == 0 && t128x320 >= 120) ? (double)((t128x320 + 255) / 256) * 0.70 : 1e30;
  const double c13 = (!geglu && N % 320 == 0 && t256x320 >= 120) ? (double)((t256x320 + 255) / 256) * (conv ? 1.20 : 1.28) : 1e30;
  if (c13 < c256 && c13 < c128 && c13 < c320) return 28;
  if (c320 < c256 && c320 < c128) return 24;
  if (c256 <= c128) return c256 < 1e30 ? 25 : 1;
  return 14;
}

template <typename T, bool CONV>
int launch(const GemmP& p, hipStream_t s) {
  const int mrows = p.tile_groups > 1 ? p.rows_per_group : p.M;
  if (g_use_glds) {
    int v = choose_variant(mrows, p.tile_groups, p.N, CONV, p.act == OMG_ACT_GEGLU);
    const long lim = 0x7fff0000L;
    const long a_sz = CONV ? (long)p.M / (p.Hout * p.Wout) * p.Hin * p.Win * (p.C1 > p.C2 ? p.C1 : p.C2) * 2 : (long)p.M * p.lda * 2;
    const long c_sz = (long)p.M * (p.ldc > p.ldr ? p.ldc : p.ldr) * 2;
    const bool v6ok = p.K2 == 0 && p.A2 == nullptr && p.K % 64 == 0 && a_sz < lim && (long)p.N * p.ldw * 2 < lim && c_sz < lim &&
                      (p.group_bias == nullptr || (long)(p.M / (p.rows_per_group > 0 ? p.rows_per_group : 1) + 1) * p.ldgb * 2 < lim);
    if ((v == 24 || v == 28) && p.act == OMG_ACT_GEGLU) v = 25;
    if (v == 24 && v6ok) return launch_v7<T, CONV, 0, 2, 5>(p, s, mrows);
    if (v == 15 && v6ok) return launch_v7<T, CONV>(p, s, mrows);
    if (v == 25 && v6ok) return launch_v12_form<T, CONV>(p, s, mrows);
    if (v == 28 && v6ok) return launch_v13_form<T, CONV>(p, s, mrows);
#ifdef OMG_ABLATION_BUILDS
    if constexpr (!CONV && sizeof(T) == 2 && Vec<T>::is_f16) {
      if (v >= 17 && v <= 23 && v6ok) {
        switch (v - 16) {
          case 1: return launch_v7<T, CONV, 1>(p, s, mrows);
          case 2: return launch_v7<T, CONV, 2>(p, s, mrows);
          case 3: return launch_v7<T, CONV, 3>(p, s, mrows);
          case 4: return launch_v7<T, CONV, 4>(p, s, mrows);
          case 5: return launch_v7<T, CONV, 5>(p, s, mrows);
          case 6: return launch_v7<T, CONV, 6>(p, s, mrows);
          default: return launch_v7<T, CONV, 7>(p, s, mrows);
        }
      }
    }
#endif
    if ((v == 13 || v == 14) && v6ok) return v == 13 ? launch_v6<T, CONV, 4>(p, s, mrows) : launch_v6<T, CONV, 2>(p, s, mrows);
  }
  const int grid = p.tile_groups * p.tiles_m * p.tiles_n;
  if (grid <= 0) return OMG_OK;
  if (g_use_glds) {
    OMG_LAUNCH((gemm_kernel<T, CONV, true>), dim3(grid), dim3(256), LDS_BYTES, s, p);
  } else {
    OMG_LAUNCH((gemm_kernel<T, CONV, false>), dim3(grid), dim3(256), LDS_BYTES, s, p);
  }
  return omg_check_launch("gemm");
}

bool g_attr_set = false;
void ensure_attrs() {
  if (g_attr_set) return;
  g_attr_set = true;
  (void)hipFuncSetAttribute((const void*)gemm_kernel<f16, false, true>, hipFuncAttributeMaxDynamicSharedMemorySize, LDS_BYTES);
  (void)hipFuncSetAttribute((const void*)gemm_kernel<f16, false, false>, hipFuncAttributeMaxDynamicSharedMemorySize, LDS_BYTES);
  (void)hipFuncSetAttribute((const void*)gemm_kernel<f16, true, true>, hipFuncAttributeMaxDynamicSharedMemorySize, LDS_BYTES);
  (void)hipFuncSetAttribute((const void*)gemm_kernel<f16, true, false>, hipFuncAttributeMaxDynamicSharedMemorySize, LDS_BYTES);
#ifndef OMG_DEV_F16_ONLY
  (void)hipFuncSetAttribute((const void*)gemm_kernel<bf16, false, true>, hipFuncAttributeMaxDynamicSharedMemorySize, LDS_BYTES);
  (void)hipFuncSetAttribute((const void*)gemm_kernel<bf16, false, false>, hipFuncAttributeMaxDynamicSharedMemorySize, LDS_BYTES);
  (void)hipFuncSetAttribute((const void*)gemm_kernel<bf16, true, true>, hipFuncAttributeMaxDynamicSharedMemorySize, LDS_BYTES);
  (void)hipFuncSetAttribute((const void*)gemm_kernel<bf16, true, false>, hipFuncAttributeMaxDynamicSharedMemorySize, LDS_BYTES);
#endif
}

}

extern "C" int omg_debug_read_ts(long long* out, int blocks) {
  return (int)hipMemcpyFromSymbol(out, HIP_SYMBOL(omg_dbg_ts), sizeof(long long) * 6 * (blocks < 8192 ? blocks : 8192));
}
extern "C" void omg_debug_set_glds(int on) { g_use_glds = on != 0; }
extern "C" void omg_debug_set_gemm_variant(int v) { g_variant = v & 0xff; g_dbg = v >> 8; }
extern "C" int omg_debug_choose_variant(int mrows, int groups, int N, int conv) {
  const int saved = g_variant;
  g_variant = 0;
  const int v = choose_variant(mrows, groups, N, (conv & 1) != 0, (conv & 2) != 0);
  g_variant = saved;
  return v;
}

extern "C" int omg_gemm(const omg_gemm_args* a, void* stream) {
  OMG_REQUIRE(a != nullptr, "omg_gemm: null args");
  OMG_REQUIRE(a->dtype == OMG_F16 || a->dtype == OMG_BF16, "omg_gemm: dtype");
  OMG_REQUIRE(a->M >= 0 && a->N > 0 && a->K > 0, "omg_gemm: shape");
  if (a->M == 0) return OMG_OK;
  OMG_REQUIRE(a->K % 8 == 0 && a->N % 8 == 0 && a->K2 % 8 == 0, "omg_gemm: K, K2, N must be multiples of 8");
  OMG_REQUIRE(a->lda % 8 == 0 && a->ldw % 8 == 0 && a->ldc % 8 == 0, "omg_gemm: leading dims must be multiples of 8");
  OMG_REQUIRE(a->A && a->W && a->C, "omg_gemm: null operand");
  OMG_REQUIRE(a->groups >= 1 && (long)a->groups * a->rows_per_group == a->M, "omg_gemm: M != groups*rows_per_group");
  if (a->K2 > 0) OMG_REQUIRE(a->A2 && a->W2 && a->lda2 % 8 == 0 && a->ldw2 % 8 == 0, "omg_gemm: LoRA segment operands");
  if (a->act == OMG_ACT_GEGLU) OMG_REQUIRE(a->N % 64 == 0 && !a->residual && !a->group_bias, "omg_gemm: GEGLU needs N % 64 == 0, no residual");
  if (a->residual) OMG_REQUIRE(a->ldr % 8 == 0, "omg_gemm: ldr");
  if (a->group_bias) OMG_REQUIRE(a->ldgb % 8 == 0, "omg_gemm: ldgb");
  ensure_attrs();
  GemmP p{};
  p.M = a->M; p.N = a->N; p.K = a->K;
  p.A = (const char*)a->A; p.lda = a->lda; p.W = (const char*)a->W; p.ldw = a->ldw;
  p.A2 = (const char*)a->A2; p.lda2 = a->lda2; p.W2 = (const char*)a->W2; p.ldw2 = a->ldw2;
  p.K2 = a->K2; p.a2_col_block = a->a2_col_block;
  const bool per_group = (a->group_adapter != nullptr) && a->groups > 1;
  p.tile_groups = per_group ? a->groups : 1;
  p.rows_per_group = a->rows_per_group;
  p.group_adapter = a->group_adapter;
  p.w_adapter_stride = a->w_adapter_stride; p.w2_adapter_stride = a->w2_adapter_stride;
  p.bias = (const char*)a->bias; p.group_bias = (const char*)a->group_bias; p.ldgb = a->ldgb;
  p.residual = (const char*)a->residual; p.ldr = a->ldr;
  p.act = a->act; p.out_scale = a->out_scale; p.C = (char*)a->C; p.ldc = a->ldc;
  const int mrows = per_group ? a->rows_per_group : a->M;
  p.tiles_m = (mrows + BM - 1) / BM;
  p.tiles_n = (a->N + BN - 1) / BN;
  hipStream_t s = (hipStream_t)stream;
#ifdef OMG_DEV_F16_ONLY
  OMG_REQUIRE(a->dtype == OMG_F16, "omg_gemm: this is a DEV=1 build (fp16 kernels only)");
  return launch<f16, false>(p, s);
#else
  return a->dtype == OMG_F16 ? launch<f16, false>(p, s) : launch<bf16, false>(p, s);
#endif
}

extern "C" int omg_conv2d(const omg_conv2d_args* a, void* stream) {
  OMG_REQUIRE(a != nullptr, "omg_conv2d: null args");
  OMG_REQUIRE(a->dtype == OMG_F16 || a->dtype == OMG_BF16, "omg_conv2d: dtype");
  OMG_REQUIRE(a->ksize == 1 || a->ksize == 3, "omg_conv2d: ksize must be 1 or 3");
  OMG_REQUIRE(a->stride == 1 || a->stride == 2, "omg_conv2d: stride must be 1 or 2");
  OMG_REQUIRE(a->C1 > 0 && a->C1 % 64 == 0 && a->C2 % 64 == 0 && a->C2 >= 0, "omg_conv2d: channels must be multiples of 64");
  OMG_REQUIRE(a->Cout % 8 == 0, "omg_conv2d: Cout % 8");
  OMG_REQUIRE(a->X1 && a->W && a->Y && (a->C2 == 0 || a->X2), "omg_conv2d: null operand");
  OMG_REQUIRE(!(a->upsample && a->stride != 1), "omg_conv2d: upsample with stride");
  const int Hl = a->upsample ? 2 * a->Hin : a->Hin, Wl = a->upsample ? 2 * a->Win : a->Win;
  const int pad = a->ksize == 3 ? 1 : 0;
  OMG_REQUIRE(a->Hout == (Hl + 2 * pad - a->ksize) / a->stride + 1 && a->Wout == (Wl + 2 * pad - a->ksize) / a->stride + 1,
              "omg_conv2d: output size mismatch");
  ensure_attrs();
  GemmP p{};
  const int Ctot = a->C1 + a->C2;
  p.M = a->B * a->Hout * a->Wout; p.N = a->Cout; p.K = a->ksize * a->ksize * Ctot;
  if (p.M == 0) return OMG_OK;
  p.A = (const char*)a->X1; p.X2 = (const char*)a->X2;
  p.W = (const char*)a->W; p.ldw = p.K;
  p.K2 = 0; p.tile_groups = 1; p.rows_per_group = a->Hout * a->Wout;
  p.bias = (const char*)a->bias; p.group_bias = (const char*)a->group_bias; p.ldgb = a->ldgb;
  p.residual = (const char*)a->residual; p.ldr = a->Cout;
  OMG_REQUIRE(a->act == OMG_ACT_NONE || a->act == OMG_ACT_SILU, "omg_conv2d: act");
  p.act = a->act; p.out_scale = a->out_scale; p.C = (char*)a->Y; p.ldc = a->Cout;
  p.Hin = a->Hin; p.Win = a->Win; p.C1 = a->C1; p.C2 = a->C2; p.Hout = a->Hout; p.Wout = a->Wout;
  p.ksize = a->ksize; p.stride = a->stride; p.upsample = a->upsample;
  p.tiles_m = (p.M + BM - 1) / BM; p.tiles_n = (p.N + BN - 1) / BN;
  if (a->group_bias) OMG_REQUIRE(a->ldgb % 8 == 0, "omg_conv2d: ldgb");
  hipStream_t s = (hipStream_t)stream;
#ifdef OMG_DEV_F16_ONLY
  OMG_REQUIRE(a->dtype == OMG_F16, "omg_conv2d: this is a DEV=1 build (fp16 kernels only)");
  return launch<f16, true>(p, s);
#else
  return a->dtype == OMG_F16 ? launch<f16, true>(p, s) : launch<bf16, true>(p, s);
#endif
}
```

### omg_amd/csrc/gemm_epilogue.h

```cpp
#pragma once
#include "common.h"

namespace {

struct GemmP {
  int M, N, K;
  const char* A; long lda;
  const char* W; long ldw;
  const char* A2; long lda2;
  const char* W2; long ldw2;
  int K2, a2_col_block;
  int tile_groups, rows_per_group;
  const int* group_adapter;
  long w_adapter_stride, w2_adapter_stride;
  const char* bias;
  const char* group_bias; long ldgb;
  const char* residual; long ldr;
  int act; float out_scale;
  char* C; long ldc;
  int Hin, Win, C1, C2, Hout, Wout, ksize, stride, upsample;
  const char* X2;
  int tiles_m, tiles_n;
  int dbg;
  const char* SA; const char* SW;
  int sa_ld, sw_ld;
  long sw_adapter_stride;
  char* QS; int qs_ld;
};

typedef __attribute__((address_space(3))) void* lds_ptr_t;
typedef const __attribute__((address_space(1))) void* gbl_ptr_t;
OMG_DEV bool fold_group_bias(const GemmP& p) { return p.group_bias != nullptr && p.rows_per_group % 256 == 0; }

template <int N> OMG_DEV void wait_vmcnt() {
  static_assert(N >= 0 && N <= 63, "vmcnt range");
  asm volatile("s_waitcnt vmcnt(%0)" ::"n"(N) : "memory");
}


template <typename T>
OMG_DEV void swap_runs(unsigned (&q)[4]) {
  asm volatile("s_nop 4\n\tv_permlane32_swap_b32 %0, %2\n\tv_permlane32_swap_b32 %1, %3\n\ts_nop 4"
               : "+v"(q[0]), "+v"(q[1]), "+v"(q[2]), "+v"(q[3]));
}
constexpr int EPI_OOB = 0x7f000000;
OMG_DEV __amdgpu_buffer_rsrc_t epi_rsrc(const char* base, long bytes) {
  const unsigned long long a = (unsigned long long)base;
  const unsigned lo = __builtin_amdgcn_readfirstlane((unsigned)a), hi = __builtin_amdgcn_readfirstlane((unsigned)(a >> 32));
  const int n = __builtin_amdgcn_readfirstlane(base != nullptr ? (int)(bytes < 0x7effff00L ? bytes : 0x7effff00L) : 0);
  return __builtin_amdgcn_make_buffer_rsrc((void*)(((unsigned long long)hi << 32) | lo), 0, n, 0x00020000);
}
template <typename T>
OMG_DEV void decode_runs(const u32x4 raw, float (&f)[8]) {
  unsigned q[4] = {raw[0], raw[1], raw[2], raw[3]};
  swap_runs<T>(q);
  u32x4 sw = {q[0], q[1], q[2], q[3]};
  unpack8<T>(sw, f);
}
template <typename T>
OMG_DEV void load_runs(__amdgpu_buffer_rsrc_t rs, int off, int soff, float (&f)[8]) {
  decode_runs<T>(__builtin_amdgcn_raw_buffer_load_b128(rs, off, soff, 0), f);
}
template <typename T>
OMG_DEV void store_runs(__amdgpu_buffer_rsrc_t rs, int off, int soff, const float (&f)[8]) {
  u32x4 pk = pack8<T>(f);
  unsigned q[4] = {pk[0], pk[1], pk[2], pk[3]};
  swap_runs<T>(q);
  u32x4 sw = {q[0], q[1], q[2], q[3]};
  __builtin_amdgcn_raw_buffer_store_b128(sw, rs, off + soff, 0, 0);
}
template <typename T>
OMG_DEV void store_runs_dbg(__amdgpu_buffer_rsrc_t rs, int off, const float (&f)[8], bool nt, int pol) {
  u32x4 pk = pack8<T>(f);
  switch (pol) {
    case 1: __builtin_amdgcn_raw_buffer_store_b128(pk, rs, off, 0, 1); break;
    case 2: __builtin_amdgcn_raw_buffer_store_b128(pk, rs, off, 0, 16); break;
    case 3: __builtin_amdgcn_raw_buffer_store_b128(pk, rs, off, 0, 17); break;
    case 4: __builtin_amdgcn_raw_buffer_store_b128(pk, rs, off, 0, 3); break;
    case 5: __builtin_amdgcn_raw_buffer_store_b128(pk, rs, off, 0, 18); break;
    case 6: __builtin_amdgcn_raw_buffer_store_b128(pk, rs, off, 0, 19); break;
    default:
      if (nt) __builtin_amdgcn_raw_buffer_store_b128(pk, rs, off, 0, 2);
      else __builtin_amdgcn_raw_buffer_store_b128(pk, rs, off, 0, 0);
  }
}

template <typename T, int MT, int NT>
OMG_DEV bool acc_init_bias(const GemmP& p, f32x16 (&acc)[MT][NT], int lane, int m0, int wn0) {
  const int hi = lane >> 5;
  const bool fold_gb = fold_group_bias(p);
  const __amdgpu_buffer_rsrc_t rsB = epi_rsrc(p.bias, (long)p.N * 2);
  const __amdgpu_buffer_rsrc_t rsG = epi_rsrc(fold_gb ? p.group_bias + (long)(m0 / p.rows_per_group) * p.ldgb * 2 : nullptr, (long)p.N * 2);
  u32x4 rb[NT][2], rg[NT][2];
#pragma unroll
  for (int j = 0; j < NT; ++j)
#pragma unroll
    for (int pr = 0; pr < 2; ++pr) {
      const int c = wn0 + j * 32 + pr * 16 + hi * 8;
      rb[j][pr] = __builtin_amdgcn_raw_buffer_load_b128(rsB, c * 2, 0, 0);
      rg[j][pr] = __builtin_amdgcn_raw_buffer_load_b128(rsG, c * 2, 0, 0);
    }
#pragma unroll
  for (int j = 0; j < NT; ++j)
#pragma unroll
    for (int pr = 0; pr < 2; ++pr) {
      float f[8], g[8];
      decode_runs<T>(rb[j][pr], f);
      decode_runs<T>(rg[j][pr], g);
#pragma unroll
      for (int i = 0; i < MT; ++i)
#pragma unroll
        for (int e = 0; e < 8; ++e) acc[i][j][pr * 8 + e] = f[e] + g[e];
    }
  return p.group_bias != nullptr && !fold_gb;
}

template <int NT>
struct EpiCtx {
  __amdgpu_buffer_rsrc_t rsC, rsR, rsG;
  int hi, l31, wm0, m_end;
  int lane_col;
  int wn0, n_out;
  char* xl;
  const char* rl;
  int voob[NT][2];
};


template <typename T, int ROWB>
OMG_DEV void xe_put(const EpiCtx<4>& cx, int piece, const float (&v)[8]) {
  const u32x4 pk = pack8<T>(v);
  const int sw = ROWB == 256 ? (cx.l31 & 15) : ((cx.l31 >> 1) & 7);
  char* b = cx.xl + cx.l31 * ROWB + ((cx.hi ^ (cx.l31 >> 4)) << 3);
  const int c0 = piece ^ sw;
  const u32x2 r0 = {pk[0], pk[1]}, r1 = {pk[2], pk[3]};
  *(u32x2*)(b + (c0 << 4)) = r0;
  *(u32x2*)(b + ((c0 ^ 1) << 4)) = r1;
}
template <typename T, int ROWB>
OMG_DEV void xe_flush(const GemmP& p, const EpiCtx<4>& cx, int i, int col0) {
  constexpr int LPR = ROWB / 16;
  constexpr int RPI = 64 / LPR;
  constexpr int NU = 32 / RPI;
  asm volatile("s_waitcnt lgkmcnt(0)" ::: "memory");
  const int lane = cx.hi * 32 + cx.l31;
  const int rq = lane / LPR, c = lane % LPR;
  const bool col_ok = col0 + 8 * c < cx.n_out && !(p.dbg & 1024);
  const int colb = (col0 + 8 * c) * 2;
  u32x4 d[NU];
#pragma unroll
  for (int u = 0; u < NU; ++u) {
    const int rr = u * RPI + rq;
    const int sw = ROWB == 256 ? (rr & 15) : ((rr >> 1) & 7);
    const u32x4 x = *(const u32x4*)(cx.xl + rr * ROWB + ((c ^ sw) << 4));
    if (u * RPI >= 16) d[u] = u32x4{x[2], x[3], x[0], x[1]}; else d[u] = x;
  }
  if constexpr (ROWB == 128) {
    if (p.QS != nullptr) {
      const __amdgpu_buffer_rsrc_t rsQ = epi_rsrc(p.QS, (long)(cx.n_out >> 7) * p.qs_ld * 4);
      const int sbase = ((col0 >> 7) * p.qs_ld) * 4 + ((col0 >> 5) & 3);
#pragma unroll
      for (int u = 0; u < NU; ++u) {
        const int gm = cx.wm0 + i * 32 + u * RPI + rq;
        float f[8];
        unpack8<T>(d[u], f);
        float amax = 0.f;
#pragma unroll
        for (int e = 0; e < 8; ++e) amax = __builtin_fmaxf(amax, __builtin_fabsf(f[e]));
        amax = __builtin_fmaxf(amax, __shfl_xor(amax, 1));
        amax = __builtin_fmaxf(amax, __shfl_xor(amax, 2));
        const unsigned be = mx8_scale_exp(amax);
        const float inv = mx8_inv_scale(be);
        const u32x2 o = {mx8_pack4(f[0] * inv, f[1] * inv, f[2] * inv, f[3] * inv), mx8_pack4(f[4] * inv, f[5] * inv, f[6] * inv, f[7] * inv)};
        const bool ok = gm < cx.m_end && col_ok;
        __builtin_amdgcn_raw_buffer_store_b64(o, cx.rsC, ok ? gm * (int)p.ldc + col0 + 8 * c : EPI_OOB, 0, 0);
        const unsigned both = be | (__shfl_down(be, 4) << 8);
        __builtin_amdgcn_raw_buffer_store_b16((unsigned short)both, rsQ, (ok && c == 0) ? sbase + gm * 4 : EPI_OOB, 0, 0);
      }
      asm volatile("" ::: "memory");
      return;
    }
  }
#pragma unroll
  for (int u = 0; u < NU; ++u) {
// ... 168 lines not shown
```

### omg_amd/csrc/gemm_v12.h

```cpp
#include "gemm_v12_sched.inc"

template <typename T, int NT>
OMG_DEV void bias_issue(const GemmP& p, int lane, int m0, int wn0, u32x4 (&rb)[NT][2], u32x4 (&rg)[NT][2]) {
  const int hi = lane >> 5;
  const bool fold_gb = fold_group_bias(p);
  const __amdgpu_buffer_rsrc_t rsB = epi_rsrc(p.bias, (long)p.N * 2);
  const __amdgpu_buffer_rsrc_t rsG = epi_rsrc(fold_gb ? p.group_bias + (long)(m0 / p.rows_per_group) * p.ldgb * 2 : nullptr, (long)p.N * 2);
#pragma unroll
  for (int j = 0; j < NT; ++j)
#pragma unroll
    for (int pr = 0; pr < 2; ++pr) {
      const int c = wn0 + j * 32 + pr * 16 + hi * 8;
      rb[j][pr] = __builtin_amdgcn_raw_buffer_load_b128(rsB, c * 2, 0, 0);
      rg[j][pr] = __builtin_amdgcn_raw_buffer_load_b128(rsG, c * 2, 0, 0);
    }
}
template <typename T, int MT, int NT>
OMG_DEV void bias_apply(const u32x4 (&rb)[NT][2], const u32x4 (&rg)[NT][2], f32x16 (&acc)[MT][NT]) {
#pragma unroll
  for (int j = 0; j < NT; ++j)
#pragma unroll
    for (int pr = 0; pr < 2; ++pr) {
      float f[8], g[8];
      decode_runs<T>(rb[j][pr], f);
      decode_runs<T>(rg[j][pr], g);
#pragma unroll
      for (int i = 0; i < MT; ++i)
#pragma unroll
        for (int e = 0; e < 8; ++e) acc[i][j][pr * 8 + e] = f[e] + g[e];
    }
}

constexpr bool omg_is_next(unsigned tag) { return tag == 1u; }
OMG_DEV int fresh_lane() {
  int l = (int)__builtin_amdgcn_mbcnt_hi(~0u, __builtin_amdgcn_mbcnt_lo(~0u, 0u));
  asm volatile("" : "+v"(l));
  return l;
}
struct TileV12 { int m0, n0, m_end, grp; };
OMG_DEV TileV12 decode_tile_v12(const GemmP& p, int vb, int ntiles) {
  int bid = vb;
  {
    const int q = ntiles >> 3, r = ntiles & 7, xcd = bid & 7, idx = bid >> 3;
    bid = (xcd < r ? xcd * (q + 1) : r * (q + 1) + (xcd - r) * q) + idx;
  }
  const int tiles_per_group = p.tiles_m * p.tiles_n;
  const int grp = bid / tiles_per_group;
  const int t_in = bid - grp * tiles_per_group;
  constexpr int G = 8;
  const int per_group = G * p.tiles_n;
  const int gid = t_in / per_group;
  const int first_m = gid * G;
  const int gsz = (p.tiles_m - first_m) < G ? (p.tiles_m - first_m) : G;
  const int r = t_in - gid * per_group;
  const int tm = first_m + (r % gsz);
  const int tn = r / gsz;
  const int m_base = (p.tile_groups > 1) ? grp * p.rows_per_group : 0;
  TileV12 t;
  t.m_end = (p.tile_groups > 1) ? m_base + p.rows_per_group : p.M;
  t.m0 = m_base + tm * 256;
  t.n0 = tn * 256;
  t.grp = grp;
  return t;
}
OMG_DEV int next_tile_v12(const GemmP& p, int vb, int step, int ntiles) {
  if (p.w_adapter_stride == 0 || p.group_adapter == nullptr) return vb;
  while (vb < ntiles) {
    const TileV12 t = decode_tile_v12(p, vb, ntiles);
    if (p.group_adapter[t.grp] >= 0) break;
    vb += step;
  }
  return vb;
}

template <typename T, bool CONV, int EF>
__global__ __launch_bounds__(256, 1) void gemm_kernel_v12(GemmP p) {
  constexpr int MT = 4, NT = 4;
  constexpr bool XE = true;
  constexpr int BM_ = MT * 64, BN_ = NT * 64, BKc = 64;
  constexpr int AB = MT * 2, WB = NT * 2;
  constexpr int A_BYTES = BM_ * BKc * 2;
  constexpr int STAGE_BYTES = (BM_ + BN_) * BKc * 2;
  constexpr int HALF = 32768;
  static_assert(A_BYTES == HALF && STAGE_BYTES == 2 * HALF, "the ring's canonical roles are the two-stage layout");
  constexpr bool EARLY_RES = EF == 2;
  constexpr bool PERSIST = EF != 2;
  constexpr bool PREFETCH = PERSIST;
  static_assert(OMG_KS_LAST_TAILS >= 32, "32 prefetch DMAs / 32 residual DMAs");

  extern __shared__ __attribute__((aligned(16))) char smem[];
  const int tid = threadIdx.x;
  const int lane = tid & 63;
  const int w = __builtin_amdgcn_readfirstlane(tid >> 6);
  const int ntiles = p.tile_groups * p.tiles_m * p.tiles_n;
  const int step = PERSIST ? (int)gridDim.x : ntiles;
  const int nk = (p.K + BKc - 1) / BKc;

  const int Ctot = p.C1 + p.C2;
  const long a_bytes = CONV ? (long)p.M / (p.Hout * p.Wout) * p.Hin * p.Win * p.C1 * 2 : ((long)(p.M - 1) * p.lda + p.K) * 2;
  const __amdgpu_buffer_rsrc_t rsA = __builtin_amdgcn_make_buffer_rsrc((void*)p.A, 0, (int)(a_bytes < 0x7fffff00 ? a_bytes : 0x7fffff00), 0x00020000);
  const __amdgpu_buffer_rsrc_t rsA2 = __builtin_amdgcn_make_buffer_rsrc((void*)(CONV && p.X2 ? p.X2 : p.A), 0,
      CONV ? (int)((long)p.M / (p.Hout * p.Wout) * p.Hin * p.Win * p.C2 * 2) : 0, 0x00020000);
  const long w_bytes = ((long)(p.N - 1) * p.ldw + p.K) * 2;
  __amdgpu_buffer_rsrc_t rsW;

  const int prow = lane >> 3, ppos = lane & 7;
  int voffA[AB], voffW[WB];
  int cb[AB], cy[AB], cx[AB];
  const int dchunk = (ppos ^ ((w & 1) * 4 + (prow >> 1))) * 16;
  const int ldo = w * 1024;
  const int wm = w >> 1, wn = w & 1;
  f32x16 acc[MT][NT];
  using V8 = typename Vec<T>::v8;

  int vb = next_tile_v12(p, (int)blockIdx.x, step, ntiles);
  if (vb >= ntiles) return;
  int m0, n0, m_end;
#define OMG_TILE_SCALARS(t_)                                                                               \
  do {                                                                                                     \
    m0 = (t_).m0; n0 = (t_).n0; m_end = (t_).m_end;                                                        \
    int adapter_ = 0;                                                                                      \
    if (p.group_adapter != nullptr) adapter_ = p.group_adapter[(t_).grp];                                  \
    const char* Wp_ = p.W + (p.w_adapter_stride != 0 ? (long)adapter_ * p.w_adapter_stride * 2 : 0);       \
    rsW = __builtin_amdgcn_make_buffer_rsrc((void*)Wp_, 0, (int)w_bytes, 0x00020000);                      \
  } while (0)
#define OMG_ADDR_A(i_)                                                                                     \
  do {                                                                                                     \
    const int r_ = (w + (i_) * 4) * 8 + prow;                                                              \
    int gm_ = m0 + r_; if (gm_ > m_end - 1) gm_ = m_end - 1;                                               \
    if constexpr (CONV) {                                                                                  \
      const int hw_ = p.Hout * p.Wout;                                                                     \
      const int b_ = gm_ / hw_; const int rem_ = gm_ - b_ * hw_;                                           \
      cb[i_] = b_; cy[i_] = rem_ / p.Wout; cx[i_] = rem_ - cy[i_] * p.Wout;                                \
      voffA[i_] = 0;                                                                                       \
    } else {                                                                                               \
      cb[i_] = cy[i_] = cx[i_] = 0;                                                                        \
      voffA[i_] = (int)((long)gm_ * p.lda * 2) + dchunk;                                                   \
    }                                                                                                      \
  } while (0)
#define OMG_ADDR_W(i_)                                                                                     \
  do {                                                                                                     \
    const int r_ = (w + (i_) * 4) * 8 + prow;                                                              \
    int gn_ = n0 + r_; if (gn_ > p.N - 1) gn_ = p.N - 1;                                                   \
    voffW[i_] = (int)((long)gn_ * p.ldw * 2) + dchunk;                                                     \
  } while (0)
  {
    const TileV12 t = decode_tile_v12(p, vb, ntiles);
    OMG_TILE_SCALARS(t);
  }
#pragma unroll
  for (int i = 0; i < AB; ++i) OMG_ADDR_A(i);
#pragma unroll
  for (int i = 0; i < WB; ++i) OMG_ADDR_W(i);

  int koff = 0;
  int tap_dy = 0, tap_dx = 0, c0b = 0, xCb = 0;
  bool x2 = false;
  const int cpt = CONV ? Ctot / BKc : 1;
  const int pad = CONV ? (p.ksize == 3 ? 1 : 0) : 0;
  const int Hl = CONV ? (p.upsample ? p.Hin * 2 : p.Hin) : 0;
  const int Wl = CONV ? (p.upsample ? p.Win * 2 : p.Win) : 0;
#define OMG_PREP(kt_)                                                                                      \
  do {                                                                                                     \
    koff = (kt_) * (BKc * 2);                                                                              \
    if constexpr (CONV) {                                                                                  \
      const int tap = (kt_) / cpt; const int cc = (kt_) - tap * cpt;                                       \
      tap_dy = tap / p.ksize - pad; tap_dx = tap - (tap / p.ksize) * p.ksize - pad;                        \
      int c0 = cc * BKc;                                                                                   \
      x2 = c0 >= p.C1;                                                                                     \
      if (x2) c0 -= p.C1;                                                                                  \
      c0b = c0 * 2; xCb = (x2 ? p.C2 : p.C1) * 2;                                                          \
    }                                                                                                      \
  } while (0)
#define OMG_DMA(d_, nb_)                                                                                   \
  do {                                                                                                     \
    if ((d_) < AB) {                                                                                       \
      const int i_ = (d_) < AB ? (d_) : 0;                                                                 \
      if (CONV) dma16(x2 ? rsA2 : rsA, (nb_) + ldo + i_ * 4096,                                            \
                      conv_voff(cb[i_], cy[i_], cx[i_], dchunk, p.stride, tap_dy, tap_dx, Hl, Wl, p.upsample, p.Hin, p.Win, xCb, c0b), 0); \
      else dma16(rsA, (nb_) + ldo + i_ * 4096, voffA[i_], koff);                                           \
    } else {                                                                                               \
      const int i_ = (d_) >= AB ? (d_) - AB : 0;                                                           \
      dma16(rsW, (nb_) + A_BYTES + ldo + i_ * 4096, voffW[i_], koff);                                      \
    }                                                                                                      \
  } while (0)
#define OMG_DMAN(first_, n_, nb_)                                                                          \
  do { _Pragma("unroll") for (int d_ = 0; d_ < (n_); ++d_) OMG_DMA((first_) + d_, nb_); } while (0)
  V8 fw[4][NT], fa[4][MT];
  unsigned la[4], lw[4];
#define OMG_LA_LW(lane_)                                                                                   \
  do {                                                                                                     \
    const unsigned lds0_ = (unsigned)(unsigned long)(lds_ptr_t)smem;                                       \
    const int hi_ = (lane_) >> 5, l31_ = (lane_) & 31;                                                     \
    _Pragma("unroll") for (int ks = 0; ks < 4; ++ks) {                                                     \
      const unsigned sw_ = (unsigned)(((ks * 2 + hi_) ^ ((l31_ >> 1) & 7)) << 4);                          \
      la[ks] = lds0_ + (unsigned)((wm * (MT * 32) + l31_) * 128) + sw_;                                    \
      lw[ks] = lds0_ + (unsigned)((wn * (NT * 32) + l31_) * 128) + sw_;                                    \
    }                                                                                                      \
  } while (0)
  OMG_LA_LW(lane);
  int sa_cur, sw_cur, sa_nxt, sw_nxt, s_sp;
#define OMG_DMAR(d_)                                                                                       \
  do {                                                                                                     \
    if ((d_) < AB) {                                                                                       \
      const int i_ = (d_) < AB ? (d_) : 0;                                                                 \
      if (CONV) dma16(x2 ? rsA2 : rsA, smem + s_sp + ldo + i_ * 4096,                                      \
                      conv_voff(cb[i_], cy[i_], cx[i_], dchunk, p.stride, tap_dy, tap_dx, Hl, Wl, p.upsample, p.Hin, p.Win, xCb, c0b), 0); \
      else dma16(rsA, smem + s_sp + ldo + i_ * 4096, voffA[i_], koff);                                     \
    } else {                                                                                               \
      const int i_ = (d_) >= AB ? (d_) - AB : 0;                                                           \
      dma16(rsW, smem + sw_cur + ldo + i_ * 4096, voffW[i_], koff);                                        \
    }                                                                                                      \
  } while (0)
#define OMG_SB __builtin_amdgcn_sched_barrier(0)
#define OMG_XRD1(ks_, r_, tog_)                                                                            \
  do {                                                                                                     \
    constexpr bool isA_ = (r_) == 1 || (r_) > NT;                                                          \
    constexpr int idx_ = (r_) <= 1 ? 0 : (r_) <= NT ? (r_) - 1 : (r_) - NT;                                \
    const unsigned ad_ = (isA_ ? la[ks_] : lw[ks_]) + (unsigned)(omg_is_next(tog_) ? (isA_ ? sa_nxt : sw_nxt) : (isA_ ? sa_cur : sw_cur)); \
    if constexpr (isA_) asm volatile("ds_read_b128 %0, %1 offset:%2" : "=v"(fa[ks_][idx_]) : "v"(ad_), "n"(idx_ * 4096)); \
    else asm volatile("ds_read_b128 %0, %1 offset:%2" : "=v"(fw[ks_][idx_]) : "v"(ad_), "n"(idx_ * 4096));  \
  } while (0)
#define OMG_XMM1(ks_, n_) acc[(n_) / NT][(n_) % NT] = Vec<T>::mfma32(fw[ks_][(n_) % NT], fa[ks_][(n_) / NT], acc[(n_) / NT][(n_) % NT])
#define OMG_XMML(ks_, n_) do { OMG_XMM1(ks_, n_); asm volatile("" : "+a"(acc[(n_) / NT][(n_) % NT])); } while (0)
#define OMG_XWAIT(ks_, left_)                                                                              \
  asm volatile("s_waitcnt lgkmcnt(" #left_ ")"                                                             \
               : "+v"(fw[ks_][0]), "+v"(fw[ks_][1]), "+v"(fw[ks_][2]), "+v"(fw[ks_][3]),                   \
                 "+v"(fa[ks_][0]), "+v"(fa[ks_][1]), "+v"(fa[ks_][2]), "+v"(fa[ks_][3]))

  int e_m0 = 0, e_n0 = 0, e_mend = 0;
  int vbn = 0;
  int lane_l = 0; (void)lane_l;
  bool has_next = false;
  u32x4 rb[NT][2], rg[NT][2];
#define OMG_HEAD(n_)                                                                                       \
  do {                                                                                                     \
    if constexpr (PREFETCH) {       \
      if constexpr ((n_) == 0) {              \
        const TileV12 t_ = decode_tile_v12(p, has_next ? vbn : vb, ntiles);                                \
        OMG_TILE_SCALARS(t_);                                                                              \
      } else if constexpr ((n_) >= 1 && (n_) <= AB) {                                                      \
        OMG_ADDR_A((n_) >= 1 && (n_) <= AB ? (n_) - 1 : 0);                                                \
      } else if constexpr ((n_) > AB && (n_) <= AB + WB) {                                                 \
        OMG_ADDR_W((n_) > AB && (n_) <= AB + WB ? (n_) - 1 - AB : 0);                                      \
      }                                                                                                    \
    }                                                                                                      \
  } while (0)
#define OMG_TAIL(n_)                                                                                       \
  do {                                                                                                     \
    if constexpr (EARLY_RES) {                                                                             \
      if constexpr ((n_) == 0) lane_l = fresh_lane();                                 \
      if constexpr ((n_) < 32) {                                                      \
        constexpr int i_ = (n_) >> 3, u_ = (n_) & 7;                                                       \
        const int rr_ = u_ * 4 + (lane_l >> 4);                                                            \
        const int gm_ = e_m0 + wm * 128 + i_ * 32 + rr_;                                                   \
        const int col_ = e_n0 + wn * 128 + (((lane_l & 15) ^ (rr_ & 15)) << 3);                            \
        const int off_ = (gm_ < e_mend && col_ < p.N) ? (gm_ * (int)p.ldr + col_) * 2 : EPI_OOB;           \
        __builtin_amdgcn_raw_ptr_buffer_load_lds(rsRes, (lds_ptr_t)(smem + w * 32768 + i_ * 8192 + u_ * 1024), 16, off_, 0, 0, 0); \
      }                                                                                                    \
    }                                                                                                      \
    if constexpr (PREFETCH) {                                                                              \
      if constexpr ((n_) == 0) OMG_PREP(0);                                                                \
      if constexpr ((n_) == AB + WB) OMG_PREP(1);                                                          \
      if constexpr ((n_) < AB + WB) {                                                                      \
        if (has_next) OMG_DMA((n_) < AB + WB ? (n_) : 0, smem);                                            \
      } else if constexpr ((n_) < 2 * (AB + WB)) {                                                         \
        if (has_next && nk > 1) OMG_DMA((n_) >= AB + WB && (n_) < 2 * (AB + WB) ? (n_) - (AB + WB) : 0, smem + STAGE_BYTES); \
      }                                                                                                    \
    }                                                                                                      \
  } while (0)
  const __amdgpu_buffer_rsrc_t rsRes = epi_rsrc(EARLY_RES ? p.residual : nullptr, ((long)(p.M - 1) * p.ldr + p.N) * 2);
  const bool fold_gb = fold_group_bias(p);
  const bool gb_epi = p.group_bias != nullptr && !fold_gb;
  (void)rsRes;

  OMG_PREP(0);
  OMG_DMAN(0, AB + WB, smem);
  bias_issue<T, NT>(p, lane, m0, n0 + wn * (NT * 32), rb, rg);
  bias_apply<T, MT, NT>(rb, rg, acc);
  bool first = true;
  for (;;) {
    wait_vmcnt<0>();
    __builtin_amdgcn_s_barrier();
    if (!PREFETCH || first) {
      OMG_PREP(1);
      if (nk > 1) OMG_DMAN(0, AB + WB, smem + STAGE_BYTES);
    }
    sa_cur = 0; sw_cur = HALF; sa_nxt = 2 * HALF; sw_nxt = 3 * HALF; s_sp = 4 * HALF;
    { const unsigned tnxt = 1u; (void)tnxt; OMG_KS_PROLOGUE_5(); }
    e_m0 = m0; e_n0 = n0; e_mend = m_end;
    if constexpr (PERSIST) { vbn = next_tile_v12(p, vb + step, step, ntiles); has_next = vbn < ntiles; }

    int kt = 0;
#define OMG_KS_VARS const unsigned tcur = 0u; const unsigned tnxt = 1u; (void)tnxt; (void)tcur
#define OMG_KS_ROT do { const int t_ = sa_cur; sa_cur = sa_nxt; sa_nxt = s_sp; s_sp = t_; const int u_ = sw_cur; sw_cur = sw_nxt; sw_nxt = u_; } while (0)
    for (; kt < nk - 2; ++kt) { OMG_KS_VARS; OMG_KS_STAGE_5(true, true); OMG_KS_ROT; }
    if (kt < nk - 1) { OMG_KS_VARS; OMG_KS_STAGE_5(true, false); OMG_KS_ROT; ++kt; }
    { OMG_KS_VARS; OMG_KS_LAST_5(); }

    const int lane_e = PERSIST ? fresh_lane() : lane;
    if constexpr (EF == 2) {
      if constexpr (!EARLY_RES) res_stage_dma(p, smem + w * 32768, lane_e, e_m0 + wm * 128, e_n0 + wn * 128, e_mend);
      epilogue_direct<T, MT, NT, XE, EF>(p, acc, lane_e, e_m0 + wm * (MT * 32), e_n0 + wn * (NT * 32), e_mend, gb_epi, smem + 2 * STAGE_BYTES + w * 8192,
                                         smem + w * 32768);
    } else
    epilogue_direct<T, MT, NT, XE, EF>(p, acc, lane_e, e_m0 + wm * (MT * 32), e_n0 + wn * (NT * 32), e_mend, gb_epi, smem + 2 * STAGE_BYTES + w * 8192);
    if (!PERSIST || !has_next) break;
    vb = vbn;
    first = false;
    { const int lane_n = fresh_lane(); OMG_LA_LW(lane_n); }
    if constexpr (!PREFETCH) {
      const TileV12 t = decode_tile_v12(p, vb, ntiles);
      OMG_TILE_SCALARS(t);
#pragma unroll
      for (int i = 0; i < AB; ++i) OMG_ADDR_A(i);
#pragma unroll
      for (int i = 0; i < WB; ++i) OMG_ADDR_W(i);
      OMG_PREP(0);
      OMG_DMAN(0, AB + WB, smem);
    }
    bias_issue<T, NT>(p, lane, m0, n0 + wn * (NT * 32), rb, rg);
    bias_apply<T, MT, NT>(rb, rg, acc);
  }
#undef OMG_KS_VARS
#undef OMG_KS_ROT
#undef OMG_HEAD
#undef OMG_TAIL
#undef OMG_DMAR
#undef OMG_XWAIT
#undef OMG_XMM1
#undef OMG_XMML
#undef OMG_XRD1
#undef OMG_SB
#undef OMG_PREP
#undef OMG_DMA
#undef OMG_DMAN
#undef OMG_ADDR_A
#undef OMG_LA_LW
#undef OMG_ADDR_W
#undef OMG_TILE_SCALARS
}

template <typename T, bool CONV, int EF>
int launch_v12(GemmP p, hipStream_t s, int mrows) {
  constexpr int lds = 2 * (256 + 256) * 64 * 2 + 4 * 8192;
  static bool attr = false;
  if (!attr) {
    attr = true;
    (void)hipFuncSetAttribute((const void*)gemm_kernel_v12<T, CONV, EF>, hipFuncAttributeMaxDynamicSharedMemorySize, lds);
  }
  p.tiles_m = (mrows + 255) / 256;
  p.tiles_n = (p.N + 255) / 256;
  p.dbg = g_dbg;
  const int ntiles = p.tile_groups * p.tiles_m * p.tiles_n;
  if (ntiles <= 0) return OMG_OK;
  int grid = ntiles;
  if (EF != 2) {
    int cus = num_cus() & ~7;
    if (g_dbg & 0x10000) cus = 8;
    if (grid > cus && cus > 0) grid = cus;
  }
  OMG_LAUNCH((gemm_kernel_v12<T, CONV, EF>), dim3(grid), dim3(256), lds, s, p);
  return omg_check_launch("gemm_v12");
}
template <typename T, bool CONV>
int launch_v12_form(const GemmP& p, hipStream_t s, int mrows) {
  const bool gb_rows = p.group_bias != nullptr && p.rows_per_group % 256 != 0;
  if (p.act == OMG_ACT_GEGLU) return launch_v12<T, CONV, 3>(p, s, mrows);
  if (gb_rows || p.act == OMG_ACT_SILU) return launch_v12<T, CONV, 4>(p, s, mrows);
  if (p.residual != nullptr) return launch_v12<T, CONV, 2>(p, s, mrows);
  return launch_v12<T, CONV, 1>(p, s, mrows);
}
```

### omg_amd/csrc/gemm_v13.h

```cpp

template <typename T> struct MfmaAsm;
template <> struct MfmaAsm<f16> {
  static OMG_DEV void a(f32x16& c, f16x8 x, f16x8 y) { asm volatile("v_mfma_f32_32x32x16_f16 %0, %1, %2, %0" : "+a"(c) : "v"(x), "v"(y)); }
  static OMG_DEV void v(f32x16& c, f16x8 x, f16x8 y) { asm volatile("v_mfma_f32_32x32x16_f16 %0, %1, %2, %0" : "+v"(c) : "v"(x), "v"(y)); }
};
template <> struct MfmaAsm<bf16> {
  static OMG_DEV void a(f32x16& c, bf16x8 x, bf16x8 y) { asm volatile("v_mfma_f32_32x32x16_bf16 %0, %1, %2, %0" : "+a"(c) : "v"(x), "v"(y)); }
  static OMG_DEV void v(f32x16& c, bf16x8 x, bf16x8 y) { asm volatile("v_mfma_f32_32x32x16_bf16 %0, %1, %2, %0" : "+v"(c) : "v"(x), "v"(y)); }
};
OMG_DEV void acc_fence(f32x16 (&acc)[4][5]) {
  asm volatile("s_nop 15\n\ts_nop 15" : "+a"(acc[0][0]), "+a"(acc[0][1]), "+a"(acc[0][2]), "+a"(acc[0][3]), "+v"(acc[0][4]));
  asm volatile("" : "+a"(acc[1][0]), "+a"(acc[1][1]), "+a"(acc[1][2]), "+a"(acc[1][3]), "+v"(acc[1][4]));
  asm volatile("" : "+a"(acc[2][0]), "+a"(acc[2][1]), "+a"(acc[2][2]), "+a"(acc[2][3]), "+v"(acc[2][4]));
  asm volatile("" : "+a"(acc[3][0]), "+a"(acc[3][1]), "+a"(acc[3][2]), "+a"(acc[3][3]), "+v"(acc[3][4]));
}

#define OMG_V13_COL(j_, wn0_, wn4_) ((j_) < 4 ? (wn0_) + (j_) * 32 : (wn4_))

template <typename T>
OMG_DEV bool acc_init_bias13(const GemmP& p, f32x16 (&acc)[4][5], int lane, int m0, int wn0, int wn4) {
  const int hi = lane >> 5;
  const bool fold_gb = fold_group_bias(p);
  const __amdgpu_buffer_rsrc_t rsB = epi_rsrc(p.bias, (long)p.N * 2);
  const __amdgpu_buffer_rsrc_t rsG = epi_rsrc(fold_gb ? p.group_bias + (long)(m0 / p.rows_per_group) * p.ldgb * 2 : nullptr, (long)p.N * 2);
// ... 9 lines not shown
#pragma unroll
  for (int j = 0; j < 5; ++j)
#pragma unroll
    for (int pr = 0; pr < 2; ++pr) {
      float f[8], g[8];
      decode_runs<T>(rb[j][pr], f);
      decode_runs<T>(rg[j][pr], g);
#pragma unroll
      for (int i = 0; i < 4; ++i)
#pragma unroll
        for (int e = 0; e < 8; ++e) acc[i][j][pr * 8 + e] = f[e] + g[e];
    }
  return p.group_bias != nullptr && !fold_gb;
}

template <typename T, bool RS, bool GENERIC>
OMG_DEV void epilogue_rows13(const GemmP& p, f32x16 (&acc)[4][5], const EpiCtx<5>& cx, const EpiCtx<4>& cx4, int lane_col4, bool has_gb) {
  const float osc = p.out_scale;
  const bool has_rs = GENERIC ? p.residual != nullptr : RS;
  u32x4 rraw[2][5][2];
#define OMG_V13_LCOL(j_) ((j_) < 4 ? cx.lane_col : lane_col4)
#define OMG_V13_SOFF(j_, pr_) ((((j_) < 4 ? (j_) * 32 : 0) + (pr_) * 16) * 2)
#define OMG_FETCH_RES13(i_, buf_)                                                                          \
  do {                                                                                                     \
    const int gm_ = cx.wm0 + (i_) * 32 + cx.l31;                                                           \
    const int rrow_ = gm_ < cx.m_end ? gm_ * (int)p.ldr * 2 : EPI_OOB;                                     \
    _Pragma("unroll") for (int j = 0; j < 5; ++j)                                                          \
      _Pragma("unroll") for (int pr = 0; pr < 2; ++pr)                                                     \
        rraw[buf_][j][pr] = __builtin_amdgcn_raw_buffer_load_b128(cx.rsR, (rrow_ + OMG_V13_LCOL(j)) | cx.voob[j][pr], OMG_V13_SOFF(j, pr), 0); \
  } while (0)
  if (has_rs) OMG_FETCH_RES13(0, 0);
#pragma unroll
  for (int i = 0; i < 4; ++i) {
    const int gm = cx.wm0 + i * 32 + cx.l31;
    const bool row_ok = gm < cx.m_end;
    if (has_rs && i + 1 < 4) OMG_FETCH_RES13(i + 1, (i + 1) & 1);
    const int crow = row_ok ? gm * (int)p.ldc * 2 : EPI_OOB;
    const int grow = GENERIC && has_gb && row_ok ? ((gm / p.rows_per_group) * (int)p.ldgb) * 2 : EPI_OOB;
#pragma unroll
    for (int j = 0; j < 5; ++j)
#pragma unroll
      for (int pr = 0; pr < 2; ++pr) {
        float v[8];
#pragma unroll
        for (int e = 0; e < 8; ++e) v[e] = acc[i][j][pr * 8 + e];
        if constexpr (GENERIC) {
          if (has_gb) {
            float f[8];
            load_runs<T>(cx.rsG, (grow + OMG_V13_LCOL(j)) | cx.voob[j][pr], OMG_V13_SOFF(j, pr), f);
#pragma unroll
            for (int e = 0; e < 8; ++e) v[e] += f[e];
          }
          if (p.act == OMG_ACT_SILU) {
#pragma unroll
            for (int e = 0; e < 8; ++e) v[e] = silu_fast(v[e]);
          }
        }
        if (has_rs) {
          const u32x4 rr = rraw[i & 1][j][pr];
          unsigned q[4] = {rr[0], rr[1], rr[2], rr[3]};
          swap_runs<T>(q);
          u32x4 sw = {q[0], q[1], q[2], q[3]};
          float rf[8];
          unpack8<T>(sw, rf);
#pragma unroll
          for (int e = 0; e < 8; ++e) v[e] = __builtin_fmaf(v[e], osc, rf[e]);
        } else {
#pragma unroll
          for (int e = 0; e < 8; ++e) v[e] *= osc;
        }
        if (j < 4) xe_put<T, 256>(cx4, 4 * j + 2 * pr, v);
        else store_runs<T>(cx.rsC, (crow + OMG_V13_LCOL(j)) | cx.voob[j][pr], OMG_V13_SOFF(j, pr), v);
        __builtin_amdgcn_sched_barrier(0);
      }
    xe_flush<T, 256>(p, cx4, i, cx4.wn0);
  }
#undef OMG_FETCH_RES13
#undef OMG_V13_SOFF
#undef OMG_V13_LCOL
}

template <typename T, int EF>
OMG_DEV void epilogue13(const GemmP& p, f32x16 (&acc)[4][5], int lane, int wm0, int wn0, int wn4, int m_end, bool has_gb, char* xl) {
  static_assert(EF == 1 || EF == 4 || EF == 5, "forms of the 256 x 320 tile: bias only, generic, residual");
  EpiCtx<5> cx;
  cx.hi = lane >> 5; cx.l31 = lane & 31; cx.wm0 = wm0; cx.m_end = m_end;
  cx.rsC = epi_rsrc(p.C, ((long)(p.M - 1) * p.ldc + p.N) * 2);
  cx.rsR = epi_rsrc(p.residual, ((long)(p.M - 1) * p.ldr + p.N) * 2);
  cx.rsG = epi_rsrc(has_gb ? p.group_bias : nullptr, 0x7effff00L);
#pragma unroll
  for (int j = 0; j < 5; ++j)
#pragma unroll
    for (int pr = 0; pr < 2; ++pr) cx.voob[j][pr] = (OMG_V13_COL(j, wn0, wn4) + pr * 16 + cx.hi * 8 < p.N && !(p.dbg & 1024)) ? 0 : EPI_OOB;
  cx.lane_col = (wn0 + cx.hi * 8) * 2;
  cx.wn0 = wn0; cx.n_out = p.N; cx.xl = xl; cx.rl = nullptr;
  const int lane_col4 = (wn4 + cx.hi * 8) * 2;
  EpiCtx<4> cx4;
  cx4.rsC = cx.rsC; cx4.rsR = cx.rsR; cx4.rsG = cx.rsG;
  cx4.hi = cx.hi; cx4.l31 = cx.l31; cx4.wm0 = wm0; cx4.m_end = m_end; cx4.lane_col = cx.lane_col; cx4.wn0 = wn0; cx4.n_out = p.N; cx4.xl = xl; cx4.rl = nullptr;
#pragma unroll
  for (int j = 0; j < 4; ++j)
#pragma unroll
    for (int pr = 0; pr < 2; ++pr) cx4.voob[j][pr] = cx.voob[j][pr];
  if constexpr (EF == 1) epilogue_rows13<T, false, false>(p, acc, cx, cx4, lane_col4, false);
  else if constexpr (EF == 5) epilogue_rows13<T, true, false>(p, acc, cx, cx4, lane_col4, false);
  else epilogue_rows13<T, false, true>(p, acc, cx, cx4, lane_col4, has_gb);
}

template <typename T, bool CONV, int EF>
__global__ __launch_bounds__(256, 1) void gemm_kernel_v13(GemmP p) {
  constexpr int MT = 4, NT = 5;
  constexpr int BM_ = MT * 64, BN_ = NT * 64, BKc = 64;
  constexpr int AB = MT * 2, WB = NT * 2;
  constexpr int NMM = MT * NT;
  constexpr int SLOTS = NMM / 2;
  constexpr int NRD = MT + NT;
  constexpr int A_BYTES = BM_ * BKc * 2;
  constexpr int STAGE_BYTES = (BM_ + BN_) * BKc * 2;
  static_assert(2 * STAGE_BYTES <= 160 * 1024, "two stages in LDS");

  const bool ts_on = (p.dbg & 16) && blockIdx.x < 8192 && threadIdx.x == 0;
  long long ts0 = 0, ts1 = 0, ts2 = 0;
  if (p.dbg & 16) ts0 = __builtin_amdgcn_s_memrealtime();
  extern __shared__ __attribute__((aligned(16))) char smem[];
  const int tid = threadIdx.x;
  const int lane = tid & 63;
  const int w = __builtin_amdgcn_readfirstlane(tid >> 6);
  const int hi = lane >> 5;
  const int l31 = lane & 31;

  const int nwg = gridDim.x;
  int bid = blockIdx.x;
  {
    const int q = nwg >> 3, r = nwg & 7, xcd = bid & 7, idx = bid >> 3;
    bid = (xcd < r ? xcd * (q + 1) : r * (q + 1) + (xcd - r) * q) + idx;
  }
  const int tiles_per_group = p.tiles_m * p.tiles_n;
  const int grp = bid / tiles_per_group;
  const int t_in = bid - grp * tiles_per_group;
  int tm, tn;
  {
    const int per_group = 8 * p.tiles_n;
    const int gid = t_in / per_group;
    const int first_m = gid * 8;
    const int gsz = (p.tiles_m - first_m) < 8 ? (p.tiles_m - first_m) : 8;
    const int r = t_in - gid * per_group;
    tm = first_m + (r % gsz);
    tn = r / gsz;
  }
  const int m_base = (p.tile_groups > 1) ? grp * p.rows_per_group : 0;
  const int m_end = (p.tile_groups > 1) ? m_base + p.rows_per_group : p.M;
  const int m0 = m_base + tm * BM_;
  const int n0 = tn * BN_;
  int adapter = 0;
  if (p.group_adapter != nullptr) adapter = p.group_adapter[grp];
  if (p.w_adapter_stride != 0 && adapter < 0) return;
  const char* Wp = p.W + (p.w_adapter_stride != 0 ? (long)adapter * p.w_adapter_stride * 2 : 0);
  const int nk = (p.K + BKc - 1) / BKc;

  const int Ctot = p.C1 + p.C2;
  const long a_bytes = CONV ? (long)p.M / (p.Hout * p.Wout) * p.Hin * p.Win * p.C1 * 2 : ((long)(p.M - 1) * p.lda + p.K) * 2;
  const __amdgpu_buffer_rsrc_t rsA = __builtin_amdgcn_make_buffer_rsrc((void*)p.A, 0, (int)(a_bytes < 0x7fffff00 ? a_bytes : 0x7fffff00), 0x00020000);
  const __amdgpu_buffer_rsrc_t rsA2 = __builtin_amdgcn_make_buffer_rsrc((void*)(CONV && p.X2 ? p.X2 : p.A), 0,
      CONV ? (int)((long)p.M / (p.Hout * p.Wout) * p.Hin * p.Win * p.C2 * 2) : 0, 0x00020000);
  const long w_bytes = ((long)(p.N - 1) * p.ldw + p.K) * 2;
  const __amdgpu_buffer_rsrc_t rsW = __builtin_amdgcn_make_buffer_rsrc((void*)Wp, 0, (int)w_bytes, 0x00020000);

  const int prow = lane >> 3, ppos = lane & 7;
  int voffA[AB], voffW[WB];
  int cb[AB], cy[AB], cx[AB];
  const int dchunk = (ppos ^ ((w & 1) * 4 + (prow >> 1))) * 16;
#pragma unroll
  for (int i = 0; i < AB; ++i) {
    const int r = (w + i * 4) * 8 + prow;
    int gm = m0 + r; if (gm > m_end - 1) gm = m_end - 1;
    if constexpr (CONV) {
      const int hw = p.Hout * p.Wout;
      const int b = gm / hw; const int rem = gm - b * hw;
      cb[i] = b; cy[i] = rem / p.Wout; cx[i] = rem - cy[i] * p.Wout;
      voffA[i] = 0;
    } else {
      cb[i] = cy[i] = cx[i] = 0;
      voffA[i] = (int)((long)gm * p.lda * 2) + dchunk;
    }
  }
#pragma unroll
  for (int i = 0; i < WB; ++i) {
    const int r = (w + i * 4) * 8 + prow;
    int gn = n0 + r; if (gn > p.N - 1) gn = p.N - 1;
    voffW[i] = (int)((long)gn * p.ldw * 2) + dchunk;
  }
  const int ldo = w * 1024;

  const int wm = w >> 1, wn = w & 1;
  const int wn0 = n0 + wn * 128, wn4 = n0 + 256 + wn * 32;
  f32x16 acc[MT][NT];
  using V8 = typename Vec<T>::v8;
  int aoff[4], boff[4], boff4[4];
#pragma unroll
  for (int ks = 0; ks < 4; ++ks) {
    const int sw = ((ks * 2 + hi) ^ ((l31 >> 1) & 7)) << 4;
    aoff[ks] = (wm * (MT * 32) + l31) * 128 + sw;
    boff[ks] = A_BYTES + (wn * 128 + l31) * 128 + sw;
    boff4[ks] = A_BYTES + (256 + wn * 32 + l31) * 128 + sw;
  }

  int koff = 0;
  int tap_dy = 0, tap_dx = 0, c0b = 0, xCb = 0;
  bool x2 = false;
  const int cpt = CONV ? Ctot / BKc : 1;
  const int pad = CONV ? (p.ksize == 3 ? 1 : 0) : 0;
  const int Hl = CONV ? (p.upsample ? p.Hin * 2 : p.Hin) : 0;
  const int Wl = CONV ? (p.upsample ? p.Win * 2 : p.Win) : 0;
#define OMG_PREP(kt_)                                                                                      \
  do {                                                                                                     \
    koff = (kt_) * (BKc * 2);                                                                              \
    if constexpr (CONV) {                                                                                  \
      const int tap = (kt_) / cpt; const int cc = (kt_) - tap * cpt;                                       \
      tap_dy = tap / p.ksize - pad; tap_dx = tap - (tap / p.ksize) * p.ksize - pad;                        \
      int c0 = cc * BKc;                                                                                   \
      x2 = c0 >= p.C1;                                                                                     \
      if (x2) c0 -= p.C1;                                                                                  \
      c0b = c0 * 2; xCb = (x2 ? p.C2 : p.C1) * 2;                                                          \
    }                                                                                                      \
  } while (0)
#define OMG_DMA(d_, nb_)                                                                                   \
  do {                                                                                                     \
    if ((d_) < AB) {                                                                                       \
      const int i_ = (d_) < AB ? (d_) : 0;                                                                 \
      if (CONV) dma16(x2 ? rsA2 : rsA, (nb_) + ldo + i_ * 4096,                                            \
                      conv_voff(cb[i_], cy[i_], cx[i_], dchunk, p.stride, tap_dy, tap_dx, Hl, Wl, p.upsample, p.Hin, p.Win, xCb, c0b), 0); \
      else dma16(rsA, (nb_) + ldo + i_ * 4096, voffA[i_], koff);                                           \
    } else {                                                                                               \
      const int i_ = (d_) - AB < WB ? (d_) - AB : 0;                                                       \
      dma16(rsW, (nb_) + A_BYTES + ldo + i_ * 4096, voffW[i_], koff);                                      \
    }                                                                                                      \
  } while (0)
#define OMG_DMAN(first_, n_, nb_)                                                                          \
  do { _Pragma("unroll") for (int d_ = 0; d_ < (n_); ++d_) OMG_DMA((first_) + d_, nb_); } while (0)
#define OMG_WFRAG(sb_, ks_, j_) (*(const V8*)((sb_) + ((j_) < 4 ? boff[ks_] + (j_) * 4096 : boff4[ks_])))
#define OMG_RD(f_, sb_, ks_)                                                                               \
  do {                                                                                                     \
    _Pragma("unroll") for (int j = 0; j < NT; ++j) bf[f_][j] = OMG_WFRAG(sb_, ks_, j);                     \
    _Pragma("unroll") for (int i = 0; i < MT; ++i) af[f_][i] = *(const V8*)((sb_) + aoff[ks_] + i * 4096); \
  } while (0)
#define OMG_RD1(f_, sb_, ks_, r_)                                                                          \
  do {                                                                                                     \
    const bool isA_ = (r_) == 1 || (r_) > NT;                                                              \
    const int idx_ = (r_) <= 1 ? 0 : (r_) <= NT ? (r_) - 1 : (r_) - NT;                                    \
    if (!isA_) bf[f_][idx_] = OMG_WFRAG(sb_, ks_, idx_);                                                   \
    else af[f_][idx_] = *(const V8*)((sb_) + aoff[ks_] + idx_ * 4096);                                     \
  } while (0)
#define OMG_MM1(f_, n_)                                                                                    \
  do {                                                                                                     \
    if ((n_) % NT == 4) MfmaAsm<T>::v(acc[(n_) / NT][4], bf[f_][4], af[f_][(n_) / NT]);                    \
    else MfmaAsm<T>::a(acc[(n_) / NT][(n_) % NT], bf[f_][(n_) % NT], af[f_][(n_) / NT]);                   \
  } while (0)
#define OMG_KSTEP(f_, RD_, rb_, rks_, DMA_, d0_, dn_, db_)                                                 \
  do {                                                                                                     \
    constexpr int RPS_ = (RD_) == 2 ? 2 : (NRD + SLOTS - 1) / SLOTS;                                       \
    constexpr int DPS_ = ((dn_) + SLOTS - 1) / SLOTS;                                                      \
    _Pragma("unroll") for (int s_ = 0; s_ < SLOTS; ++s_) {                                                 \
      OMG_MM1(f_, 2 * s_);                                                                                 \
      __builtin_amdgcn_sched_barrier(0);                                                                   \
      if ((RD_) != 0) {                                                                                    \
        _Pragma("unroll") for (int q_ = 0; q_ < RPS_; ++q_)                                                \
          if (s_ * RPS_ + q_ < NRD) OMG_RD1(1 - (f_), rb_, rks_, s_ * RPS_ + q_);                          \
      }                                                                                                    \
      __builtin_amdgcn_sched_barrier(0);                                                                   \
      OMG_MM1(f_, 2 * s_ + 1);                                                                             \
      __builtin_amdgcn_sched_barrier(0);                                                                   \
      if (DMA_) {                                                                                          \
        _Pragma("unroll") for (int q_ = 0; q_ < DPS_; ++q_)                                                \
          if (s_ * DPS_ + q_ < (dn_)) OMG_DMA((d0_) + s_ * DPS_ + q_, db_);                                \
      }                                                                                                    \
      __builtin_amdgcn_sched_barrier(0);                                                                   \
    }                                                                                                      \
  } while (0)

  V8 af[2][MT], bf[2][NT];
  OMG_PREP(0);
  OMG_DMAN(0, AB + WB, smem);
  const bool gb_epi = acc_init_bias13<T>(p, acc, lane, m0, wn0, wn4);
  wait_vmcnt<0>();
  __builtin_amdgcn_s_barrier();
  if (p.dbg & 16) ts1 = __builtin_amdgcn_s_memrealtime();
  OMG_PREP(1);
  if (nk > 1) OMG_DMAN(0, AB, smem + STAGE_BYTES);
  OMG_RD(0, smem, 0);
  acc_fence(acc);

#define OMG_STAGE(HAS1_, HAS2_)                                                                            \
  do {                                                                                                     \
    const char* cur = smem + (kt & 1) * STAGE_BYTES;                                                       \
    char* nxt = smem + ((kt + 1) & 1) * STAGE_BYTES;                                                       \
    OMG_KSTEP(0, 1, cur, 1, HAS1_, AB, WB, nxt);                                                           \
    OMG_KSTEP(1, 1, cur, 2, false, 0, 0, nxt);                                                             \
    OMG_KSTEP(0, 1, cur, 3, false, 0, 0, nxt);                                                             \
     \
    asm volatile("s_waitcnt vmcnt(0) lgkmcnt(0)" ::: "memory"); __builtin_amdgcn_s_barrier();              \
    if (HAS2_) OMG_PREP(kt + 2);                                                                           \
    OMG_KSTEP(1, (HAS1_) ? 2 : 0, nxt, 0, HAS2_, 0, AB, (char*)cur);                                       \
  } while (0)
  int kt = 0;
  for (; kt < nk - 2; ++kt) OMG_STAGE(true, true);
  if (kt < nk - 1) { OMG_STAGE(true, false); ++kt; }
// ... 57 lines not shown
```

### omg_amd/modules.py

```python
from __future__ import annotations

from typing import Optional

import torch
from torch import nn

from . import _lib as L
from . import ops


class LoraState:

    __slots__ = ("group_adapter", "groups", "merged")

    def __init__(self, group_adapter: torch.Tensor, groups: int, merged: bool = False):
        self.group_adapter = group_adapter
        self.groups = groups
        self.merged = merged


_POINTER_EPOCH = [0]


def pointer_epoch() -> int:
    return _POINTER_EPOCH[0]


def bump_weights_version(net) -> None:
    net.weights_version = getattr(net, "weights_version", 0) + 1


def bump_pointer_epoch() -> None:
    _POINTER_EPOCH[0] += 1


class _Packed(nn.Module):
    def __init__(self):
        super().__init__()
        self._packed = {}

    def invalidate_packed(self):
        if self._packed:
            bump_pointer_epoch()
        self._packed = {}

    def _load_from_state_dict(self, *a, **k):
        self.invalidate_packed()
        return super()._load_from_state_dict(*a, **k)

    def _apply(self, fn, *a, **k):
        self.invalidate_packed()
        return super()._apply(fn, *a, **k)


class Linear(_Packed):

    def __init__(self, in_features: int, out_features: int, bias: bool = True, dtype=torch.float16, device=None):
        super().__init__()
        self.in_features, self.out_features = in_features, out_features
        self.weight = nn.Parameter(torch.empty(out_features, in_features, dtype=dtype, device=device), requires_grad=False)
        self.bias = nn.Parameter(torch.empty(out_features, dtype=dtype, device=device), requires_grad=False) if bias else None
        self.lora_down: Optional[torch.Tensor] = None
        self.lora_up: Optional[torch.Tensor] = None
        self.w_slots: Optional[torch.Tensor] = None
        self.lora_state: Optional[LoraState] = None
        self.mx8 = False

    def invalidate_mx8_slots(self) -> None:
        if self._packed.pop("mx8_slots", None) is not None:
            bump_pointer_epoch()

    def _mx8_ok(self) -> bool:
        st = self.lora_state
        return self.in_features % 128 == 0 and not (st is not None and not st.merged and self.lora_down is not None)

    def _forward_mx8(self, x, residual, act):
        xq = x if isinstance(x, ops.Mx8Tensor) else ops.quant_mx8(x)
        shp = xq.shape
        r2 = residual.reshape(-1, self.out_features) if residual is not None else None
        st = self.lora_state
        dt = self.weight.dtype
        if st is not None and st.merged and self.w_slots is not None:
            if "mx8_slots" not in self._packed:
                self._packed["mx8_slots"] = ops.quant_mx8(self.w_slots.reshape(-1, self.in_features))
            y = ops.gemm_mx8(xq, self._packed["mx8_slots"], out_dtype=dt, bias=self.bias, residual=r2, act=act, groups=st.groups,
                             w_group_adapter=st.group_adapter, n_per_adapter=self.out_features)
        else:
            if "mx8_w" not in self._packed:
                self._packed["mx8_w"] = ops.quant_mx8(self.weight.data)
            y = ops.gemm_mx8(xq, self._packed["mx8_w"], out_dtype=dt, bias=self.bias, residual=r2, act=act)
        return y.view(*shp[:-1], y.shape[-1])

    def _lora(self, x2: torch.Tensor) -> Optional[ops.LoraSpec]:
        st = self.lora_state
        if st is None or st.merged or self.lora_down is None:
            return None
        t = ops.gemm(x2, self.lora_down, groups=st.groups, w_group_adapter=st.group_adapter)
        return ops.LoraSpec(t, self.lora_up, st.group_adapter)

    def forward(self, x: torch.Tensor, scale=None, *, residual: Optional[torch.Tensor] = None, act: int = L.ACT_NONE,
                group_bias: Optional[torch.Tensor] = None, groups: int = 1) -> torch.Tensor:
        if isinstance(x, ops.Mx8Tensor) or (self.mx8 and group_bias is None and self._mx8_ok()):
            if group_bias is not None or not self._mx8_ok():
                raise L.OmgHipError("an MX-fp8 activation reached a Linear layer that cannot run in MX-fp8")
            return self._forward_mx8(x, residual, act)
        shp = x.shape
        x2 = x.reshape(-1, shp[-1])
        r2 = residual.reshape(-1, self.out_features) if residual is not None else None
        st = self.lora_state
        if st is not None and st.merged and self.w_slots is not None:
            y = ops.gemm(x2, self.w_slots, bias=self.bias, residual=r2, act=act, groups=st.groups, w_group_adapter=st.group_adapter)
            return y.view(*shp[:-1], y.shape[-1])
        lora = self._lora(x2)
        if lora is not None:
            groups = self.lora_state.groups
            if x2.shape[0] % groups != 0:
                raise L.OmgHipError("LoRA groups do not divide the row count")
        y = ops.gemm(x2, self.weight, bias=self.bias, residual=r2, act=act, group_bias=group_bias, groups=groups, lora=lora)
        return y.view(*shp[:-1], y.shape[-1])


class GEGLU(_Packed):

    def __init__(self, dim_in: int, dim_out: int, dtype=torch.float16, device=None):
        super().__init__()
        self.proj = Linear(dim_in, dim_out * 2, dtype=dtype, device=device)

    def _packed_w(self):
        if "w" not in self._packed:
            perm = ops.geglu_row_perm(self.proj.out_features).to(self.proj.weight.device)
            self._packed["w"] = self.proj.weight.data[perm].contiguous()
            self._packed["b"] = self.proj.bias.data[perm].contiguous()
            if self.proj.lora_up is not None:
                self._packed["up"] = self.proj.lora_up[:, perm].contiguous()
            if self.proj.w_slots is not None:
                self._packed["w_slots"] = self.proj.w_slots[:, perm].contiguous()
        return self._packed

    def invalidate_packed(self):
        super().invalidate_packed()

    def _forward_mx8(self, x, out_mx8: bool = False):
        xq = x if isinstance(x, ops.Mx8Tensor) else ops.quant_mx8(x)
        shp = xq.shape
        pk = self._packed_w()
        st = self.proj.lora_state
        dt = self.proj.weight.dtype
        out_mx8 = out_mx8 and self.proj.out_features % 256 == 0
        if st is not None and st.merged and "w_slots" in pk:
            if "mx8_slots" not in pk:
                pk["mx8_slots"] = ops.quant_mx8(pk["w_slots"].reshape(-1, self.proj.in_features))
            y = ops.gemm_mx8(xq, pk["mx8_slots"], out_dtype=dt, bias=pk["b"], act=L.ACT_GEGLU, groups=st.groups,
                             w_group_adapter=st.group_adapter, n_per_adapter=self.proj.out_features, out_mx8=out_mx8)
        else:
            if "mx8_w" not in pk:
                pk["mx8_w"] = ops.quant_mx8(pk["w"])
            y = ops.gemm_mx8(xq, pk["mx8_w"], out_dtype=dt, bias=pk["b"], act=L.ACT_GEGLU, out_mx8=out_mx8)
        if isinstance(y, ops.Mx8Tensor):
            return y
        return y.view(*shp[:-1], y.shape[-1])

    def forward(self, x, out_mx8: bool = False):
        if isinstance(x, ops.Mx8Tensor) or (self.proj.mx8 and self.proj._mx8_ok()):
            return self._forward_mx8(x, out_mx8)
        shp = x.shape
        x2 = x.reshape(-1, shp[-1])
        pk = self._packed_w()
        lora = None
        groups = 1
        st = self.proj.lora_state
        if st is not None and st.merged and "w_slots" in pk:
            y = ops.gemm(x2, pk["w_slots"], bias=pk["b"], act=L.ACT_GEGLU, groups=st.groups, w_group_adapter=st.group_adapter)
            return y.view(*shp[:-1], y.shape[-1])
        if st is not None and not st.merged and self.proj.lora_down is not None:
            t = ops.gemm(x2, self.proj.lora_down, groups=st.groups, w_group_adapter=st.group_adapter)
            lora = ops.LoraSpec(t, pk["up"], st.group_adapter)
            groups = st.groups
        y = ops.gemm(x2, pk["w"], bias=pk["b"], act=L.ACT_GEGLU, groups=groups, lora=lora)
        return y.view(*shp[:-1], y.shape[-1])


class Conv2d(_Packed):

    def __init__(self, cin: int, cout: int, ksize: int, stride: int = 1, dtype=torch.float16, device=None):
        super().__init__()
        self.cin, self.cout, self.ksize, self.stride = cin, cout, ksize, stride
        self.weight = nn.Parameter(torch.empty(cout, cin, ksize, ksize, dtype=dtype, device=device), requires_grad=False)
        self.bias = nn.Parameter(torch.empty(cout, dtype=dtype, device=device), requires_grad=False)
        self.mx8 = False

    def packed_weight(self) -> torch.Tensor:
        if "w" not in self._packed:
            self._packed["w"] = ops.pack_conv_weight(self.weight.data)
        return self._packed["w"]

    def wino_weight(self) -> Optional[torch.Tensor]:
        if self.ksize != 3 or self.stride != 1 or self.cin % 8 != 0 or self.weight.dtype != torch.float32:
            return None
        if "wu" not in self._packed:
            self._packed["wu"] = ops.pack_conv_weight_wino(self.weight.data)
        return self._packed["wu"]

    def mx8_ok(self) -> bool:
        return self.mx8 and self.ksize == 3 and self.stride == 1 and self.cin % 32 == 0 and self.weight.dtype != torch.float32

    def mx8_weight(self) -> "ops.Mx8Tensor":
        if "wq" not in self._packed:
            w = self.packed_weight()
            cq = (self.cin + 127) // 128 * 128
            if cq != self.cin:
                wp = torch.zeros((self.cout, 9, cq), dtype=w.dtype, device=w.device)
                wp[:, :, :self.cin] = w.view(self.cout, 9, self.cin)
                w = wp.view(self.cout, 9 * cq)
            self._packed["wq"] = ops.quant_mx8(w)
        return self._packed["wq"]

    def forward(self, x: torch.Tensor, *, x2: Optional[torch.Tensor] = None, upsample: bool = False,
                group_bias: Optional[torch.Tensor] = None, residual: Optional[torch.Tensor] = None) -> torch.Tensor:
        if isinstance(x, ops.Mx8Map):
            if not self.mx8_ok() or x2 is not None or upsample:
                raise L.OmgHipError("an MX-fp8 feature map can only feed a 3x3 / stride 1 convolution in MX-fp8 mode")
            return ops.conv2d_mx8(x, self.mx8_weight(), bias=self.bias, group_bias=group_bias, residual=residual)
        if self.weight.dtype == torch.float32:
            if x2 is not None or group_bias is not None or self.stride != 1:
                raise L.OmgHipError("the fp32 convolution supports stride 1 without concat / per-sample bias (all the VAE decoder needs)")
            return ops.conv2d_f32(x, self.packed_weight(), self.ksize, upsample=upsample, bias=self.bias, residual=residual,
                                  wu=self.wino_weight())
        return ops.conv2d(x, self.packed_weight(), self.ksize, stride=self.stride, upsample=upsample, x2=x2, bias=self.bias,
                          group_bias=group_bias, residual=residual)


class GroupNorm(nn.Module):
    def __init__(self, groups: int, channels: int, eps: float, dtype=torch.float16, device=None):
        super().__init__()
        self.groups, self.eps = groups, eps
        self.weight = nn.Parameter(torch.empty(channels, dtype=dtype, device=device), requires_grad=False)
        self.bias = nn.Parameter(torch.empty(channels, dtype=dtype, device=device), requires_grad=False)

    def forward(self, x: torch.Tensor, *, x2: Optional[torch.Tensor] = None, silu: bool = False, mx8: bool = False):
        if mx8:
            return ops.groupnorm_mx8(x, self.weight, self.bias, self.groups, self.eps, silu=silu, x2=x2)
        return ops.groupnorm(x, self.weight, self.bias, self.groups, self.eps, silu=silu, x2=x2)


class LayerNorm(nn.Module):
    def __init__(self, channels: int, eps: float = 1e-5, dtype=torch.float16, device=None):
        super().__init__()
        self.eps = eps
        self.weight = nn.Parameter(torch.empty(channels, dtype=dtype, device=device), requires_grad=False)
        self.bias = nn.Parameter(torch.empty(channels, dtype=dtype, device=device), requires_grad=False)

    def forward(self, x: torch.Tensor, mx8: bool = False):
        if mx8 and x.shape[-1] % 128 == 0:
            return ops.layernorm_mx8(x, self.weight, self.bias, self.eps)
        return ops.layernorm(x, self.weight, self.bias, self.eps)


class Dropout(nn.Module):

    def forward(self, x):
        return x
```

### omg_amd/ops.py

```python
from __future__ import annotations

import ctypes as C
import os
from typing import Optional, Sequence

import torch

from . import _lib as L

_DT = {torch.float16: L.OMG_F16, torch.bfloat16: L.OMG_BF16}


def _dt(t: torch.Tensor, allow_f32: bool = False) -> int:
    if allow_f32 and t.dtype == torch.float32:
        return L.OMG_F32
    try:
        return _DT[t.dtype]
    except KeyError:
        raise L.OmgHipError(f"unsupported dtype {t.dtype}; use float16 or bfloat16") from None


def _dev(t: torch.Tensor) -> None:
    if not t.is_cuda:
        raise L.OmgHipError("omg_amd ops need tensors on the MI355X (cuda/hip device); there is no CPU fallback")


def _stream() -> int:
    return torch.cuda.current_stream().cuda_stream


def _p(t: Optional[torch.Tensor]) -> Optional[int]:
    return None if t is None else t.data_ptr()


class KernelProfiler:

    def __init__(self):
        self.records = []

    def begin(self):
        e = torch.cuda.Event(enable_timing=True)
        e.record(torch.cuda.current_stream())
        return e

    def end(self, kind: str, flops: float, start, tag=None) -> None:
        e = torch.cuda.Event(enable_timing=True)
        e.record(torch.cuda.current_stream())
        self.records.append((kind, flops, start, e, tag))

    def summary(self):
        out = {}
        for kind, fl, s, e, _ in self.records:
            d = out.setdefault(kind, dict(launches=0, ms=0.0, flops=0.0))
            d["launches"] += 1
            d["ms"] += s.elapsed_time(e)
            d["flops"] += fl
        return out

    def by_tag(self):
        out = {}
        for kind, fl, s, e, tag in self.records:
            d = out.setdefault((kind, tag), dict(launches=0, ms=0.0, flops=0.0))
            d["launches"] += 1
            d["ms"] += s.elapsed_time(e)
            d["flops"] += fl
        return sorted(out.items(), key=lambda kv: -kv[1]["ms"])


_PROF: Optional[KernelProfiler] = None


def set_profiler(p: Optional[KernelProfiler]) -> None:
    global _PROF
    _PROF = p


class LoraSpec:

    __slots__ = ("a2", "w2", "group_adapter", "a2_col_block")

    def __init__(self, a2: torch.Tensor, w2: torch.Tensor, group_adapter: Optional[torch.Tensor] = None,
                 a2_col_block: int = 0):
        self.a2, self.w2, self.group_adapter, self.a2_col_block = a2, w2, group_adapter, a2_col_block


def gemm(a: torch.Tensor, w: torch.Tensor, *, bias: Optional[torch.Tensor] = None,
         residual: Optional[torch.Tensor] = None, act: int = L.ACT_NONE, out: Optional[torch.Tensor] = None,
         out_scale: float = 1.0, group_bias: Optional[torch.Tensor] = None, groups: int = 1,
         lora: Optional[LoraSpec] = None, w_group_adapter: Optional[torch.Tensor] = None) -> torch.Tensor:
    _dev(a)
    M, K = a.shape
    assert a.stride(1) == 1
    if w.dim() == 3:
        N = w.shape[1]
        w_stride = w.stride(0)
        ldw = w.stride(1)
    else:
        N = w.shape[0]
        w_stride = 0
        ldw = w.stride(0)
    assert w.shape[-1] == K and w.stride(-1) == 1
    n_out = N // 2 if act == L.ACT_GEGLU else N
    if out is None:
        out = torch.empty((M, n_out), dtype=a.dtype, device=a.device)
    assert out.stride(1) == 1 and out.shape[0] == M and out.shape[1] == n_out
    args = L.GemmArgs()
    args.dtype = _dt(a)
    args.M, args.N, args.K = M, N, K
    args.A, args.lda = a.data_ptr(), a.stride(0)
    args.W, args.ldw = w.data_ptr(), ldw
    args.groups = groups
    args.rows_per_group = M // groups
    adapter = w_group_adapter
    if lora is not None:
        a2, w2 = lora.a2, lora.w2
        args.A2, args.lda2 = a2.data_ptr(), a2.stride(0)
        args.K2 = w2.shape[-1]
        args.W2 = w2.data_ptr()
        if w2.dim() == 3:
            args.ldw2, args.w2_adapter_stride = w2.stride(1), w2.stride(0)
        else:
            args.ldw2, args.w2_adapter_stride = w2.stride(0), 0
        args.a2_col_block = lora.a2_col_block
        if lora.group_adapter is not None:
            adapter = lora.group_adapter
    args.group_adapter = _p(adapter)
    args.w_adapter_stride = w_stride
    args.bias = _p(bias)
    if group_bias is not None:
        args.group_bias, args.ldgb = group_bias.data_ptr(), group_bias.stride(0)
    if residual is not None:
        assert residual.stride(1) == 1
        args.residual, args.ldr = residual.data_ptr(), residual.stride(0)
    args.act = act
    args.out_scale = out_scale
    args.C, args.ldc = out.data_ptr(), out.stride(0)
    if _PROF is not None:
        t0 = _PROF.begin()
        L.check(L.lib().omg_gemm(C.byref(args), _stream()), "omg_gemm")
        _PROF.end("gemm", 2.0 * M * N * (K + args.K2), t0, ("lin", M, N, K, args.K2, groups if adapter is not None else 1, act))
        return out
    L.check(L.lib().omg_gemm(C.byref(args), _stream()), "omg_gemm")
    return out


class Mx8Tensor:

    __slots__ = ("q", "scales", "rows", "K", "shape")

    def __init__(self, q: torch.Tensor, scales: torch.Tensor, shape=None):
        self.q, self.scales, self.rows, self.K = q, scales, q.shape[0], q.shape[1]
        self.shape = tuple(shape) if shape is not None else (q.shape[0], q.shape[1])

    @property
    def device(self):
        return self.q.device


def quant_mx8(x: torch.Tensor, out: Optional[Mx8Tensor] = None) -> Mx8Tensor:
    _dev(x)
    shape = x.shape
    x = x.reshape(-1, shape[-1])
    assert x.stride(1) == 1
    M, K = x.shape
    if K % 128 != 0:
        raise L.OmgHipError("MX-fp8 operands need K % 128 == 0")
    if out is None:
        s_ld = (M + 3) // 4 * 4
        out = Mx8Tensor(torch.empty((M, K), dtype=torch.uint8, device=x.device),
                        torch.zeros((K // 128, s_ld), dtype=torch.int32, device=x.device), shape)
    assert out.q.shape == (M, K) and out.q.stride(1) == 1 and out.scales.shape[0] == K // 128
    L.check(L.lib().omg_quant_mx8(_dt(x), x.data_ptr(), x.stride(0), M, K, out.q.data_ptr(), out.q.stride(0),
                                  out.scales.data_ptr(), out.scales.stride(0), _stream()), "omg_quant_mx8")
    return out


def gemm_mx8(a: Mx8Tensor, w: Mx8Tensor, *, out_dtype: torch.dtype = torch.float16, bias: Optional[torch.Tensor] = None,
             residual: Optional[torch.Tensor] = None, act: int = L.ACT_NONE, out: Optional[torch.Tensor] = None,
             out_scale: float = 1.0, groups: int = 1, w_group_adapter: Optional[torch.Tensor] = None,
             n_per_adapter: Optional[int] = None, out_mx8: bool = False):
    M, K = a.rows, a.K
    assert w.K == K
    N = n_per_adapter if w_group_adapter is not None else w.rows
    n_out = N // 2 if act == L.ACT_GEGLU else N
    oq = None
    if out_mx8:
        assert out is None and act == L.ACT_GEGLU and N % 256 == 0
        oq = Mx8Tensor(torch.empty((M, n_out), dtype=torch.uint8, device=a.q.device),
                       torch.empty((n_out // 128, (M + 3) // 4 * 4), dtype=torch.int32, device=a.q.device), tuple(a.shape[:-1]) + (n_out,))
        out = oq.q
    elif out is None:
        out = torch.empty((M, n_out), dtype=out_dtype, device=a.q.device)
    assert out.stride(1) == 1 and out.shape == (M, n_out)
    g = L.GemmMx8Args()
    g.dtype = _DT[out_dtype] if out_mx8 else _dt(out)
    g.M, g.N, g.K = M, N, K
    g.A, g.lda, g.a_scale, g.sa_ld = a.q.data_ptr(), a.q.stride(0), a.scales.data_ptr(), a.scales.stride(0)
    g.W, g.ldw, g.w_scale, g.sw_ld = w.q.data_ptr(), w.q.stride(0), w.scales.data_ptr(), w.scales.stride(0)
    g.groups, g.rows_per_group = groups, M // groups
    if w_group_adapter is not None:
        g.group_adapter = w_group_adapter.data_ptr()
        g.w_adapter_stride, g.sw_adapter_stride = N * w.q.stride(0), N
    g.bias = _p(bias)
    if residual is not None:
        assert residual.stride(1) == 1
        g.residual, g.ldr = residual.data_ptr(), residual.stride(0)
    g.act, g.out_scale = act, out_scale
    g.C, g.ldc = out.data_ptr(), out.stride(0)
    if oq is not None:
        g.c_scale, g.sc_ld = oq.scales.data_ptr(), oq.scales.stride(0)
    if _PROF is not None:
        t0 = _PROF.begin()
        L.check(L.lib().omg_gemm_mx8(C.byref(g), _stream()), "omg_gemm_mx8")
        _PROF.end("gemm_mx8", 2.0 * M * N * K, t0, ("mx8", M, N, K, 0, groups if w_group_adapter is not None else 1, act))
        return oq if oq is not None else out
    L.check(L.lib().omg_gemm_mx8(C.byref(g), _stream()), "omg_gemm_mx8")
    return oq if oq is not None else out


def conv2d(x1: torch.Tensor, w: torch.Tensor, ksize: int, *, stride: int = 1, upsample: bool = False,
           x2: Optional[torch.Tensor] = None, bias: Optional[torch.Tensor] = None,
           group_bias: Optional[torch.Tensor] = None, residual: Optional[torch.Tensor] = None,
           out_scale: float = 1.0, act: int = L.ACT_NONE) -> torch.Tensor:
    _dev(x1)
    B, Hin, Win, C1 = x1.shape
    assert x1.is_contiguous()
    C2 = 0
    if x2 is not None:
        assert x2.is_contiguous() and x2.shape[:3] == x1.shape[:3]
        C2 = x2.shape[3]
    Cout = w.shape[0]
    assert w.is_contiguous() and w.shape[1] == ksize * ksize * (C1 + C2)
    Hl, Wl = (2 * Hin, 2 * Win) if upsample else (Hin, Win)
    pad = 1 if ksize == 3 else 0
    Hout = (Hl + 2 * pad - ksize) // stride + 1
    Wout = (Wl + 2 * pad - ksize) // stride + 1
    y = torch.empty((B, Hout, Wout, Cout), dtype=x1.dtype, device=x1.device)
    a = L.Conv2dArgs()
    a.dtype = _dt(x1)
    a.B, a.Hin, a.Win, a.C1, a.C2 = B, Hin, Win, C1, C2
    a.Hout, a.Wout, a.Cout = Hout, Wout, Cout
    a.ksize, a.stride, a.upsample = ksize, stride, int(upsample)
    a.X1, a.X2, a.W, a.bias = x1.data_ptr(), _p(x2), w.data_ptr(), _p(bias)
    if group_bias is not None:
        a.group_bias, a.ldgb = group_bias.data_ptr(), group_bias.stride(0)
    if residual is not None:
        assert residual.is_contiguous() and residual.shape == y.shape
        a.residual = residual.data_ptr()
    a.out_scale = out_scale
    a.act = act
    a.Y = y.data_ptr()
    if _PROF is not None:
        t0 = _PROF.begin()
        L.check(L.lib().omg_conv2d(C.byref(a), _stream()), "omg_conv2d")
        _PROF.end("gemm", 2.0 * B * Hout * Wout * Cout * ksize * ksize * (C1 + C2), t0, ("conv", B * Hout * Wout, Cout, ksize * ksize * (C1 + C2), 0, 1, 0))
        return y
    L.check(L.lib().omg_conv2d(C.byref(a), _stream()), "omg_conv2d")
    return y


class Mx8Map:

    __slots__ = ("q", "scales", "shape", "dtype")

    def __init__(self, q: torch.Tensor, scales: torch.Tensor, dtype: torch.dtype):
        self.q, self.scales, self.shape, self.dtype = q, scales, tuple(q.shape), dtype

    @property
    def device(self):
        return self.q.device


def groupnorm_mx8(x1: torch.Tensor, gamma: torch.Tensor, beta: torch.Tensor, groups: int, eps: float, *,
                  silu: bool = False, x2: Optional[torch.Tensor] = None) -> Mx8Map:
    _dev(x1)
    assert x1.is_contiguous() and x1.dim() == 4
    B, H, W, C1 = x1.shape
    C2 = 0
    if x2 is not None:
        assert x2.is_contiguous() and x2.shape[:3] == x1.shape[:3]
        C2 = x2.shape[-1]
    Cc = C1 + C2
    if Cc % 32 != 0:
        raise L.OmgHipError("MX-fp8 feature maps need C % 32 == 0")
    Cq = (Cc + 127) // 128 * 128
    out = Mx8Map(torch.empty((B, H, W, Cq), dtype=torch.uint8, device=x1.device),
                 torch.empty((Cq // 128, B * H * W), dtype=torch.int32, device=x1.device), x1.dtype)
    ws = _gn_workspace(x1.device, B, groups, H * W)
    assert gamma.dtype == x1.dtype and beta.dtype == x1.dtype
    L.check(L.lib().omg_groupnorm_mx8(_dt(x1), x1.data_ptr(), C1, _p(x2), C2, B, H * W, groups, eps, gamma.data_ptr(), beta.data_ptr(),
                                      int(silu), ws.data_ptr(), out.q.data_ptr(), out.scales.data_ptr(), _stream()), "omg_groupnorm_mx8")
    return out

# ... 449 lines not shown
```

Measured before the change: 0.4224.

## Skip GEMM tiles for Q/K projection columns that attention never reads

For batch samples whose attention query/key rows are sourced from another sample (qk_src remap), the Q (and K for self-attention) projection columns are dead. A per-group n_begin vector is passed to the GEMM, whose kernels return early on dead N tiles, and the persistent v12 kernel gets a live-tile walk that uses a wave prefix-sum so persistent blocks only iterate over live tiles. This is meant to cut projection FLOPs in the mask-fusion path, at the cost of extra kernel variants, more decode logic per tile, and garbage in the skipped output columns.

Result: no change. 0.4250 (median of 6 runs) (+0.6%).

```diff
diff --git a/include/omg_hip.h b/include/omg_hip.h
--- a/include/omg_hip.h
+++ b/include/omg_hip.h
@@ -47,6 +47,7 @@
   int32_t act;
   float out_scale;
   void* C; int64_t ldc;
+  const int32_t* group_n_begin;
 } omg_gemm_args;
 
 int omg_gemm(const omg_gemm_args* a, void* stream);
diff --git a/omg_amd/_lib.py b/omg_amd/_lib.py
--- a/omg_amd/_lib.py
+++ b/omg_amd/_lib.py
@@ -25,6 +25,7 @@
         ("residual", c_vp), ("ldr", c_i64),
         ("act", c_i32), ("out_scale", c_f32),
         ("C", c_vp), ("ldc", c_i64),
+        ("group_n_begin", c_vp),
     ]
 
 
diff --git a/omg_amd/attention.py b/omg_amd/attention.py
--- a/omg_amd/attention.py
+++ b/omg_amd/attention.py
@@ -114,7 +114,7 @@
             self._kv_slots = torch.cat([self.to_k.w_slots, self.to_v.w_slots], dim=1).contiguous()
         return self._kv_slots
 
-    def project_self(self, x):
+    def project_self(self, x, dead_qk=None):
         B, N, C = x.shape
         inner = self.inner_dim
         if isinstance(x, ops.Mx8Tensor) or (self.to_q.mx8 and C % 128 == 0 and not self._has_lora()):
@@ -138,7 +138,10 @@
         else:
             st = self._merged()
             if st is not None:
-                qkv = ops.gemm(x.reshape(B * N, C), self.qkv_slots(), groups=st.groups, w_group_adapter=st.group_adapter)
+                qkv = ops.gemm(x.reshape(B * N, C), self.qkv_slots(), groups=st.groups, w_group_adapter=st.group_adapter,
+                               group_n_begin=dead_qk if st.groups == B else None)
+            elif dead_qk is not None:
+                qkv = ops.gemm(x.reshape(B * N, C), self.qkv_weight(), groups=B, group_n_begin=dead_qk)
             else:
                 qkv = ops.gemm(x.reshape(B * N, C), self.qkv_weight())
             qkv = qkv.view(B, N, 3 * inner)
@@ -226,6 +229,9 @@
     def _skip_layer(self) -> None:
         return None
 
+    def _dead_columns(self, src, n_dead: int, keep_from):
+        return None
+
     def __call__(self, attn: Attention, hidden_states, encoder_hidden_states=None, attention_mask=None, temb=None,
                  scale: float = 1.0, residual: Optional[torch.Tensor] = None, **cross_attention_kwargs):
         if attention_mask is not None:
@@ -233,11 +239,6 @@
         x = _to_tokens(attn, hidden_states)
         B, N, _ = x.shape
         is_cross = encoder_hidden_states is not None
-        if is_cross:
-            q = attn.to_q(x)
-            k, vt = attn.project_cross(encoder_hidden_states)
-        else:
-            q, k, vt = attn.project_self(x)
         bypass = cross_attention_kwargs.pop("omg_bypass_controller", False)
         main_b = cross_attention_kwargs.pop("omg_main_batch", None)
         n_img = cross_attention_kwargs.pop("omg_images", 1)
@@ -247,8 +248,15 @@
         src = None if (bypass or twin) else self._qk_src(attn, is_cross, N, B, x.device, main_b, n_img)
         ip_ctx = cross_attention_kwargs.pop("omg_ip_tokens", None)
         ip_row0 = cross_attention_kwargs.pop("omg_ip_rows", 0)
+        ip = is_cross and ip_ctx is not None and attn.ip_kv_weight is not None
+        dead = None if src is None else self._dead_columns(src, attn.inner_dim if is_cross else 2 * attn.inner_dim, ip_row0 if ip else None)
+        if is_cross:
+            q = attn.to_q(x, group_n_begin=dead)
+            k, vt = attn.project_cross(encoder_hidden_states)
+        else:
+            q, k, vt = attn.project_self(x, dead)
         o = ops.attention(q, k, vt, attn.heads, attn.scale, qk_src=src)
-        if is_cross and ip_ctx is not None and attn.ip_kv_weight is not None:
+        if ip:
             _ip_branch(attn, q, o, ip_ctx, ip_row0)
         out = attn.to_out[0](o, residual=residual)
         return out
@@ -269,6 +277,13 @@
             return None
         return self.controller.fused_qk_src(is_cross, n_tokens, main_batch or batch, self.place_in_unet, device=device,
                                             total_batch=batch, images=images)
+
+    skip_dead_projections = True
+
+    def _dead_columns(self, src, n_dead, keep_from):
+        if not self.skip_dead_projections or self.controller is None or not hasattr(self.controller, "dead_n_begin"):
+            return None
+        return self.controller.dead_n_begin(src, n_dead, keep_from)
 
     def _skip_layer(self) -> None:
         if self.controller is not None:
diff --git a/omg_amd/controller.py b/omg_amd/controller.py
--- a/omg_amd/controller.py
+++ b/omg_amd/controller.py
@@ -133,6 +133,8 @@
         self._identity_mapper = all(torch.equal(m.float().cpu(), eye) for m in self.mapper)
         self.is_pure_replacement = bool(local_blend is None and self._identity_mapper and bool((self.cross_replace_alpha == 1).all()))
         self._src_cache: Dict[Tuple, torch.Tensor] = {}
+        self._src_rows: Dict[int, Tuple[int, ...]] = {}
+        self._dead_cache: Dict[Tuple, object] = {}
 
     @property
     def num_uncond_att_layers(self):
@@ -197,7 +199,20 @@
             v += list(range(batch * images, total))
             t = torch.tensor(v, dtype=torch.int32, device=device)
             self._src_cache[key] = t
+            self._src_rows[id(t)] = tuple(v)
         return t
+
+    def dead_n_begin(self, src: torch.Tensor, n_dead: int, keep_from: Optional[int] = None):
+        rows = self._src_rows.get(id(src))
+        if rows is None or len(rows) > 64:
+            return None
+        key = (id(src), n_dead, keep_from)
+        hit = self._dead_cache.get(key)
+        if hit is None:
+            host = tuple(n_dead if (s != b and (keep_from is None or b < keep_from)) else 0 for b, s in enumerate(rows))
+            hit = (torch.tensor(host, dtype=torch.int32, device=src.device), host) if any(host) else False
+            self._dead_cache[key] = hit
+        return hit or None
 
     def skip_layer(self) -> None:
         if not self.is_pure_replacement:
diff --git a/omg_amd/csrc/gemm.hip b/omg_amd/csrc/gemm.hip
--- a/omg_amd/csrc/gemm.hip
+++ b/omg_amd/csrc/gemm.hip
@@ -156,6 +156,9 @@
   const int m_end = (p.tile_groups > 1) ? m_base + p.rows_per_group : p.M;
   const int m0 = m_base + tm * BM;
   const int n0 = tn * BN;
+  if constexpr (!CONV) {
+    if (p.group_n_begin != nullptr && tn < dead_tiles_n(p, p.group_n_begin[grp], BN)) return;
+  }
 
   int adapter = 0;
   if (p.group_adapter != nullptr) adapter = p.group_adapter[grp];
@@ -332,6 +335,9 @@
   const int m_end = (p.tile_groups > 1) ? m_base + p.rows_per_group : p.M;
   const int m0 = m_base + tm * BM_;
   const int n0 = tn * BN_;
+  if constexpr (!CONV) {
+    if (p.group_n_begin != nullptr && tn < dead_tiles_n(p, p.group_n_begin[grp], BN_)) return;
+  }
   int adapter = 0;
   if (p.group_adapter != nullptr) adapter = p.group_adapter[grp];
   if (p.w_adapter_stride != 0 && adapter < 0) return;
@@ -560,6 +566,9 @@
   const int m_end = (p.tile_groups > 1) ? m_base + p.rows_per_group : p.M;
   const int m0 = m_base + tm * BM_;
   const int n0 = tn * BN_;
+  if constexpr (!CONV) {
+    if (p.group_n_begin != nullptr && tn < dead_tiles_n(p, p.group_n_begin[grp], BN_)) return;
+  }
   int adapter = 0;
   if (p.group_adapter != nullptr) adapter = p.group_adapter[grp];
   if (p.w_adapter_stride != 0 && adapter < 0) return;
@@ -915,10 +924,13 @@
   p.A = (const char*)a->A; p.lda = a->lda; p.W = (const char*)a->W; p.ldw = a->ldw;
   p.A2 = (const char*)a->A2; p.lda2 = a->lda2; p.W2 = (const char*)a->W2; p.ldw2 = a->ldw2;
   p.K2 = a->K2; p.a2_col_block = a->a2_col_block;
-  const bool per_group = (a->group_adapter != nullptr) && a->groups > 1;
+  if (a->group_n_begin != nullptr)
+    OMG_REQUIRE(a->groups <= 64 && a->act != OMG_ACT_GEGLU, "omg_gemm: group_n_begin needs groups <= 64 and is not combined with GEGLU");
+  const bool per_group = (a->group_adapter != nullptr || a->group_n_begin != nullptr) && a->groups > 1;
   p.tile_groups = per_group ? a->groups : 1;
   p.rows_per_group = a->rows_per_group;
   p.group_adapter = a->group_adapter;
+  p.group_n_begin = a->group_n_begin;
   p.w_adapter_stride = a->w_adapter_stride; p.w2_adapter_stride = a->w2_adapter_stride;
   p.bias = (const char*)a->bias; p.group_bias = (const char*)a->group_bias; p.ldgb = a->ldgb;
   p.residual = (const char*)a->residual; p.ldr = a->ldr;
diff --git a/omg_amd/csrc/gemm_epilogue.h b/omg_amd/csrc/gemm_epilogue.h
--- a/omg_amd/csrc/gemm_epilogue.h
+++ b/omg_amd/csrc/gemm_epilogue.h
@@ -12,6 +12,7 @@
   int K2, a2_col_block;
   int tile_groups, rows_per_group;
   const int* group_adapter;
+  const int* group_n_begin;
   long w_adapter_stride, w2_adapter_stride;
   const char* bias;
   const char* group_bias; long ldgb;
@@ -30,6 +31,7 @@
 
 typedef __attribute__((address_space(3))) void* lds_ptr_t;
 typedef const __attribute__((address_space(1))) void* gbl_ptr_t;
+OMG_DEV int dead_tiles_n(const GemmP& p, int nb, int bn) { return nb >= p.N ? p.tiles_n : (nb > 0 ? nb / bn : 0); }
 OMG_DEV bool fold_group_bias(const GemmP& p) { return p.group_bias != nullptr && p.rows_per_group % 256 == 0; }
 
 template <int N> OMG_DEV void wait_vmcnt() {
diff --git a/omg_amd/csrc/gemm_v12.h b/omg_amd/csrc/gemm_v12.h
--- a/omg_amd/csrc/gemm_v12.h
+++ b/omg_amd/csrc/gemm_v12.h
@@ -38,23 +38,44 @@
   return l;
 }
 struct TileV12 { int m0, n0, m_end, grp; };
-OMG_DEV TileV12 decode_tile_v12(const GemmP& p, int vb, int ntiles) {
+OMG_DEV int live_prefix_v12(const GemmP& p, int lane, int bn, int& nlive) {
+  const bool in = lane < p.tile_groups;
+  const int c = in ? p.tiles_m * (p.tiles_n - dead_tiles_n(p, p.group_n_begin[in ? lane : 0], bn)) : 0;
+  int incl = c;
+#pragma unroll
+  for (int d = 1; d < 64; d <<= 1) {
+    const int up = __shfl_up(incl, d);
+    if (lane >= d) incl += up;
+  }
+  nlive = __builtin_amdgcn_readlane(incl, 63);
+  return in ? incl - c : 0x7fffffff;
+}
+template <bool LIVE = false>
+OMG_DEV TileV12 decode_tile_v12(const GemmP& p, int vb, int ntiles, int pre = 0) {
   int bid = vb;
   {
     const int q = ntiles >> 3, r = ntiles & 7, xcd = bid & 7, idx = bid >> 3;
     bid = (xcd < r ? xcd * (q + 1) : r * (q + 1) + (xcd - r) * q) + idx;
   }
-  const int tiles_per_group = p.tiles_m * p.tiles_n;
-  const int grp = bid / tiles_per_group;
-  const int t_in = bid - grp * tiles_per_group;
+  int grp, t_in, tiles_n = p.tiles_n, nd = 0;
+  if constexpr (LIVE) {
+    grp = __builtin_amdgcn_readfirstlane(__builtin_popcountll(__builtin_amdgcn_ballot_w64(pre <= bid)) - 1);
+    t_in = bid - __builtin_amdgcn_readlane(pre, grp);
+    nd = dead_tiles_n(p, p.group_n_begin[grp], 256);
+    tiles_n -= nd;
+  } else {
+    const int tiles_per_group = p.tiles_m * p.tiles_n;
+    grp = bid / tiles_per_group;
+    t_in = bid - grp * tiles_per_group;
+  }
   constexpr int G = 8;
-  const int per_group = G * p.tiles_n;
+  const int per_group = G * tiles_n;
   const int gid = t_in / per_group;
   const int first_m = gid * G;
   const int gsz = (p.tiles_m - first_m) < G ? (p.tiles_m - first_m) : G;
   const int r = t_in - gid * per_group;
   const int tm = first_m + (r % gsz);
-  const int tn = r / gsz;
+  const int tn = r / gsz + nd;
   const int m_base = (p.tile_groups > 1) ? grp * p.rows_per_group : 0;
   TileV12 t;
   t.m_end = (p.tile_groups > 1) ? m_base + p.rows_per_group : p.M;
@@ -63,18 +84,20 @@
   t.grp = grp;
   return t;
 }
-OMG_DEV int next_tile_v12(const GemmP& p, int vb, int step, int ntiles) {
+template <bool LIVE = false>
+OMG_DEV int next_tile_v12(const GemmP& p, int vb, int step, int ntiles, int pre = 0) {
   if (p.w_adapter_stride == 0 || p.group_adapter == nullptr) return vb;
   while (vb < ntiles) {
-    const TileV12 t = decode_tile_v12(p, vb, ntiles);
+    const TileV12 t = decode_tile_v12<LIVE>(p, vb, ntiles, pre);
     if (p.group_adapter[t.grp] >= 0) break;
     vb += step;
   }
   return vb;
 }
 
-template <typename T, bool CONV, int EF>
-__global__ __launch_bounds__(256, 1) void gemm_kernel_v12(GemmP p) {
+template <typename T, bool CONV, int EF, bool LIVE>
+OMG_DEV void gemm_v12_body(const GemmP& p) {
+  static_assert(!LIVE || (!CONV && EF != 2 && EF != 3), "the live walk serves the persistent Linear forms");
   constexpr int MT = 4, NT = 4;
   constexpr bool XE = true;
   constexpr int BM_ = MT * 64, BN_ = NT * 64, BKc = 64;
@@ -92,7 +115,9 @@
   const int tid = threadIdx.x;
   const int lane = tid & 63;
   const int w = __builtin_amdgcn_readfirstlane(tid >> 6);
-  const int ntiles = p.tile_groups * p.tiles_m * p.tiles_n;
+  int ntiles = p.tile_groups * p.tiles_m * p.tiles_n;
+  int pre = 0; (void)pre;
+  if constexpr (LIVE) pre = live_prefix_v12(p, lane, 256, ntiles);
   const int step = PERSIST ? (int)gridDim.x : ntiles;
   const int nk = (p.K + BKc - 1) / BKc;
 
@@ -113,8 +138,14 @@
   f32x16 acc[MT][NT];
   using V8 = typename Vec<T>::v8;
 
-  int vb = next_tile_v12(p, (int)blockIdx.x, step, ntiles);
+  int vb = next_tile_v12<LIVE>(p, (int)blockIdx.x, step, ntiles, pre);
   if (vb >= ntiles) return;
+  if constexpr (!CONV && EF == 2) {
+    if (p.group_n_begin != nullptr) {
+      const TileV12 t = decode_tile_v12(p, vb, ntiles);
+      if (t.n0 < dead_tiles_n(p, p.group_n_begin[t.grp], 256) * 256) return;
+    }
+  }
   int m0, n0, m_end;
 #define OMG_TILE_SCALARS(t_)                                                                               \
   do {                                                                                                     \
@@ -145,7 +176,7 @@
     voffW[i_] = (int)((long)gn_ * p.ldw * 2) + dchunk;                                                     \
   } while (0)
   {
-    const TileV12 t = decode_tile_v12(p, vb, ntiles);
+    const TileV12 t = decode_tile_v12<LIVE>(p, vb, ntiles, pre);
     OMG_TILE_SCALARS(t);
   }
 #pragma unroll
@@ -237,7 +268,7 @@
   do {                                                                                                     \
     if constexpr (PREFETCH) {       \
       if constexpr ((n_) == 0) {              \
-        const TileV12 t_ = decode_tile_v12(p, has_next ? vbn : vb, ntiles);                                \
+        const TileV12 t_ = decode_tile_v12<LIVE>(p, has_next ? vbn : vb, ntiles, pre);                     \
         OMG_TILE_SCALARS(t_);                                                                              \
       } else if constexpr ((n_) >= 1 && (n_) <= AB) {                                                      \
         OMG_ADDR_A((n_) >= 1 && (n_) <= AB ? (n_) - 1 : 0);                                                \
@@ -289,7 +320,7 @@
     sa_cur = 0; sw_cur = HALF; sa_nxt = 2 * HALF; sw_nxt = 3 * HALF; s_sp = 4 * HALF;
     { const unsigned tnxt = 1u; (void)tnxt; OMG_KS_PROLOGUE_5(); }
     e_m0 = m0; e_n0 = n0; e_mend = m_end;
-    if constexpr (PERSIST) { vbn = next_tile_v12(p, vb + step, step, ntiles); has_next = vbn < ntiles; }
+    if constexpr (PERSIST) { vbn = next_tile_v12<LIVE>(p, vb + step, step, ntiles, pre); has_next = vbn < ntiles; }
 
     int kt = 0;
 #define OMG_KS_VARS const unsigned tcur = 0u; const unsigned tnxt = 1u; (void)tnxt; (void)tcur
@@ -310,7 +341,7 @@
     first = false;
     { const int lane_n = fresh_lane(); OMG_LA_LW(lane_n); }
     if constexpr (!PREFETCH) {
-      const TileV12 t = decode_tile_v12(p, vb, ntiles);
+      const TileV12 t = decode_tile_v12<LIVE>(p, vb, ntiles, pre);
       OMG_TILE_SCALARS(t);
 #pragma unroll
       for (int i = 0; i < AB; ++i) OMG_ADDR_A(i);
@@ -340,14 +371,19 @@
 #undef OMG_ADDR_W
 #undef OMG_TILE_SCALARS
 }
-
 template <typename T, bool CONV, int EF>
+__global__ __launch_bounds__(256, 1) void gemm_kernel_v12(GemmP p) { gemm_v12_body<T, CONV, EF, false>(p); }
+template <typename T, int EF>
+__global__ __launch_bounds__(256, 1) void gemm_live_walk_v12(GemmP p) { gemm_v12_body<T, false, EF, true>(p); }
+
+template <typename T, bool CONV, int EF, bool LIVE = false>
 int launch_v12(GemmP p, hipStream_t s, int mrows) {
   constexpr int lds = 2 * (256 + 256) * 64 * 2 + 4 * 8192;
   static bool attr = false;
   if (!attr) {
     attr = true;
-    (void)hipFuncSetAttribute((const void*)gemm_kernel_v12<T, CONV, EF>, hipFuncAttributeMaxDynamicSharedMemorySize, lds);
+    if constexpr (LIVE) (void)hipFuncSetAttribute((const void*)gemm_live_walk_v12<T, EF>, hipFuncAttributeMaxDynamicSharedMemorySize, lds);
+    else (void)hipFuncSetAttribute((const void*)gemm_kernel_v12<T, CONV, EF>, hipFuncAttributeMaxDynamicSharedMemorySize, lds);
   }
   p.tiles_m = (mrows + 255) / 256;
   p.tiles_n = (p.N + 255) / 256;
@@ -360,13 +396,20 @@
     if (g_dbg & 0x10000) cus = 8;
     if (grid > cus && cus > 0) grid = cus;
   }
-  OMG_LAUNCH((gemm_kernel_v12<T, CONV, EF>), dim3(grid), dim3(256), lds, s, p);
+  if constexpr (LIVE) OMG_LAUNCH((gemm_live_walk_v12<T, EF>), dim3(grid), dim3(256), lds, s, p);
+  else OMG_LAUNCH((gemm_kernel_v12<T, CONV, EF>), dim3(grid), dim3(256), lds, s, p);
   return omg_check_launch("gemm_v12");
 }
 template <typename T, bool CONV>
 int launch_v12_form(const GemmP& p, hipStream_t s, int mrows) {
   const bool gb_rows = p.group_bias != nullptr && p.rows_per_group % 256 != 0;
   if (p.act == OMG_ACT_GEGLU) return launch_v12<T, CONV, 3>(p, s, mrows);
+  if constexpr (!CONV) {
+    if (p.group_n_begin != nullptr) {
+      if (gb_rows || p.act == OMG_ACT_SILU) return launch_v12<T, CONV, 4, true>(p, s, mrows);
+      if (p.residual == nullptr) return launch_v12<T, CONV, 1, true>(p, s, mrows);
+    }
+  }
   if (gb_rows || p.act == OMG_ACT_SILU) return launch_v12<T, CONV, 4>(p, s, mrows);
   if (p.residual != nullptr) return launch_v12<T, CONV, 2>(p, s, mrows);
   return launch_v12<T, CONV, 1>(p, s, mrows);
diff --git a/omg_amd/csrc/gemm_v13.h b/omg_amd/csrc/gemm_v13.h
--- a/omg_amd/csrc/gemm_v13.h
+++ b/omg_amd/csrc/gemm_v13.h
@@ -185,6 +185,9 @@
   const int m_end = (p.tile_groups > 1) ? m_base + p.rows_per_group : p.M;
   const int m0 = m_base + tm * BM_;
   const int n0 = tn * BN_;
+  if constexpr (!CONV) {
+    if (p.group_n_begin != nullptr && tn < dead_tiles_n(p, p.group_n_begin[grp], BN_)) return;
+  }
   int adapter = 0;
   if (p.group_adapter != nullptr) adapter = p.group_adapter[grp];
   if (p.w_adapter_stride != 0 && adapter < 0) return;
diff --git a/omg_amd/modules.py b/omg_amd/modules.py
--- a/omg_amd/modules.py
+++ b/omg_amd/modules.py
@@ -99,7 +99,7 @@
         return ops.LoraSpec(t, self.lora_up, st.group_adapter)
 
     def forward(self, x: torch.Tensor, scale=None, *, residual: Optional[torch.Tensor] = None, act: int = L.ACT_NONE,
-                group_bias: Optional[torch.Tensor] = None, groups: int = 1) -> torch.Tensor:
+                group_bias: Optional[torch.Tensor] = None, groups: int = 1, group_n_begin=None) -> torch.Tensor:
         if isinstance(x, ops.Mx8Tensor) or (self.mx8 and group_bias is None and self._mx8_ok()):
             if group_bias is not None or not self._mx8_ok():
                 raise L.OmgHipError("an MX-fp8 activation reached a Linear layer that cannot run in MX-fp8")
@@ -108,15 +108,20 @@
         x2 = x.reshape(-1, shp[-1])
         r2 = residual.reshape(-1, self.out_features) if residual is not None else None
         st = self.lora_state
+        n_samples = shp[0] if len(shp) == 3 else -1
         if st is not None and st.merged and self.w_slots is not None:
-            y = ops.gemm(x2, self.w_slots, bias=self.bias, residual=r2, act=act, groups=st.groups, w_group_adapter=st.group_adapter)
+            y = ops.gemm(x2, self.w_slots, bias=self.bias, residual=r2, act=act, groups=st.groups, w_group_adapter=st.group_adapter,
+                         group_n_begin=group_n_begin if st.groups == n_samples else None)
             return y.view(*shp[:-1], y.shape[-1])
         lora = self._lora(x2)
         if lora is not None:
             groups = self.lora_state.groups
             if x2.shape[0] % groups != 0:
                 raise L.OmgHipError("LoRA groups do not divide the row count")
-        y = ops.gemm(x2, self.weight, bias=self.bias, residual=r2, act=act, group_bias=group_bias, groups=groups, lora=lora)
+        elif group_n_begin is not None and group_bias is None and groups == 1:
+            groups = n_samples
+        y = ops.gemm(x2, self.weight, bias=self.bias, residual=r2, act=act, group_bias=group_bias, groups=groups, lora=lora,
+                     group_n_begin=group_n_begin if groups == n_samples else None)
         return y.view(*shp[:-1], y.shape[-1])
 
 
diff --git a/omg_amd/ops.py b/omg_amd/ops.py
--- a/omg_amd/ops.py
+++ b/omg_amd/ops.py
@@ -84,10 +84,21 @@
         self.a2, self.w2, self.group_adapter, self.a2_col_block = a2, w2, group_adapter, a2_col_block
 
 
+_TILE_N = {25: 256, 13: 256, 15: 256, 28: 320, 24: 320, 14: 128}
+
+
+def _dead_columns(rows_per_group: int, groups: int, N: int, n_begin: int) -> int:
+    if n_begin >= N:
+        return N
+    bn = _TILE_N.get(L.lib().omg_debug_choose_variant(rows_per_group, groups, N, 0), 128)
+    return max(n_begin, 0) // bn * bn
+
+
 def gemm(a: torch.Tensor, w: torch.Tensor, *, bias: Optional[torch.Tensor] = None,
          residual: Optional[torch.Tensor] = None, act: int = L.ACT_NONE, out: Optional[torch.Tensor] = None,
          out_scale: float = 1.0, group_bias: Optional[torch.Tensor] = None, groups: int = 1,
-         lora: Optional[LoraSpec] = None, w_group_adapter: Optional[torch.Tensor] = None) -> torch.Tensor:
+         lora: Optional[LoraSpec] = None, w_group_adapter: Optional[torch.Tensor] = None,
+         group_n_begin=None) -> torch.Tensor:
     _dev(a)
     M, K = a.shape
     assert a.stride(1) == 1
@@ -135,10 +146,15 @@
     args.act = act
     args.out_scale = out_scale
     args.C, args.ldc = out.data_ptr(), out.stride(0)
+    if group_n_begin is not None:
+        vec, host = group_n_begin
+        assert vec.dtype == torch.int32 and vec.numel() == groups == len(host) and vec.device == a.device
+        args.group_n_begin = vec.data_ptr()
     if _PROF is not None:
         t0 = _PROF.begin()
         L.check(L.lib().omg_gemm(C.byref(args), _stream()), "omg_gemm")
-        _PROF.end("gemm", 2.0 * M * N * (K + args.K2), t0, ("lin", M, N, K, args.K2, groups if adapter is not None else 1, act))
+        n_run = N if group_n_begin is None else N - sum(_dead_columns(M // groups, groups, N, nb) for nb in group_n_begin[1]) / groups
+        _PROF.end("gemm", 2.0 * M * n_run * (K + args.K2), t0, ("lin", M, N, K, args.K2, groups if adapter is not None else 1, act))
         return out
     L.check(L.lib().omg_gemm(C.byref(args), _stream()), "omg_gemm")
     return out
```
